# MachinaIO/mxx

Measured on AMD Instinct MI355X. Metric: dcrt_ring_ops_per_s, higher is better.
Workload: dtype u32

## Files before the change

include/gpupoly.h:

```cpp
#ifndef GPUPOLY_H
#define GPUPOLY_H

#include <stddef.h>
#include <stdint.h>

#ifdef __cplusplus
extern "C" {
#endif

typedef struct GpuContext GpuContext;
typedef struct GpuMatrix GpuMatrix;
typedef struct GpuEventSet GpuEventSet;
typedef struct GpuP1CovarianceCache GpuP1CovarianceCache;
typedef struct GpuComm GpuComm;

typedef struct GpuRngSeed {
    uint64_t words[4];
} GpuRngSeed;

#define GPU_POLY_FORMAT_COEFF 0
#define GPU_POLY_FORMAT_EVAL 1
#define GPU_MATRIX_DIST_UNIFORM 0
#define GPU_MATRIX_DIST_GAUSS 1
#define GPU_MATRIX_DIST_BIT 2
// ... 98 lines not shown
    const GpuMatrix *lhs;
    const GpuMatrix *rhs;
} GpuBatchOp;
int gpupoly_batch(const GpuBatchOp *ops, size_t count, uint32_t base_bits);
int gpupoly_matrix_mul_decompose_small(GpuMatrix *out, const GpuMatrix *lhs, const GpuMatrix *rhs, uint32_t base_bits);
int gpupoly_matrix_mul_tensor_identity(GpuMatrix *out, const GpuMatrix *lhs, const GpuMatrix *rhs, size_t identity_size);
int gpupoly_matrix_mul_tensor_identity_decompose(GpuMatrix *out, const GpuMatrix *lhs, const GpuMatrix *rhs,
                                                 size_t identity_size, uint32_t base_bits);
int gpupoly_matrix_mul_scalar_intt(GpuMatrix *out, const GpuMatrix *lhs, const GpuMatrix *scalar_1x1);
int gpupoly_matrix_transpose(GpuMatrix *out, const GpuMatrix *src);
int gpupoly_matrix_tensor(GpuMatrix *out, const GpuMatrix *lhs, const GpuMatrix *rhs);
int gpupoly_matrix_add_rows(GpuMatrix *out, size_t dst_row, const GpuMatrix *lhs, const GpuMatrix *rhs);
int gpupoly_matrix_ntt_add_rows(GpuMatrix *out, size_t dst_row, GpuMatrix *coeff, const GpuMatrix *addend,
                                int consume_coeff);
int gpupoly_matrix_row_view(GpuMatrix *m, size_t row, size_t rows, GpuMatrix **out_view);
int gpupoly_matrix_reshape_view(GpuMatrix *m, size_t rows, size_t cols, GpuMatrix **out_view);
int gpupoly_matrix_neg(GpuMatrix *out, const GpuMatrix *src);
int gpupoly_matrix_fill_zero(GpuMatrix *out);
int gpupoly_matrix_fill_identity(GpuMatrix *out, const GpuMatrix *scalar_1x1);
int gpupoly_matrix_sample_decomposed(GpuMatrix *out, int dist_type, double sigma, GpuRngSeed seed, uint32_t base_bits,
                                     int small);
int gpupoly_matrix_decompose_rows(const GpuMatrix *src, uint32_t base_bits, int small, size_t row_start, GpuMatrix *out);
int gpupoly_matrix_sample_decomposed_window(GpuMatrix *out, int dist_type, double sigma, GpuRngSeed seed,
                                            uint32_t base_bits, int small, size_t src_rows, size_t full_ncol,
                                            size_t col_offset, size_t row_start);
int gpupoly_timer_start(GpuContext *ctx);
int gpupoly_timer_stop(GpuContext *ctx, float *out_ms);
int gpupoly_timer_mark(GpuContext *ctx, uint32_t slot);
int gpupoly_timer_elapsed(GpuContext *ctx, uint32_t slot_begin, uint32_t slot_end, float *out_ms);
int gpupoly_matrix_device_ptr(const GpuMatrix *mat, void **out_ptr, size_t *out_bytes);
int gpupoly_matrix_layout(const GpuMatrix *mat, int *out);
int gpupoly_matrix_copy_to_context(GpuContext *dst_ctx, const GpuMatrix *src, GpuMatrix **out);
int gpupoly_context_device(const GpuContext *ctx, int *out_device);
int gpupoly_context_word_bytes(const GpuContext *ctx, int *out_bytes);
const char *gpupoly_context_last_kernel(const GpuContext *ctx);
int gpupoly_context_stream(const GpuContext *ctx, void **out_stream);
int gpupoly_comm_create(GpuContext *const *ctxs, size_t n, GpuComm **out_comm);
void gpupoly_comm_destroy(GpuComm *comm);
int gpupoly_comm_size(const GpuComm *comm, int *out_size);
const char *gpupoly_comm_backend(const GpuComm *comm);
int gpupoly_matrix_all_gather_columns(GpuComm *comm, const GpuMatrix *const *local_blocks, GpuMatrix *const *full);
int gpupoly_matrix_sample_distribution_segments(GpuMatrix *out, int dist_type, double sigma, const GpuRngSeed *seeds,
                                                const size_t *seg_cols, size_t nseg);
int gpupoly_matrix_sample_p1_full_cached_segments(const GpuP1CovarianceCache *cache, const GpuMatrix *tp2,
                                                  const GpuRngSeed *seeds, const size_t *seg_cols, size_t nseg,
                                                  GpuMatrix *out);
int gpupoly_matrix_gauss_samp_gq_arb_base_segments(GpuMatrix *src, uint32_t base_bits, double c, double dgg_stddev,
                                                   const GpuRngSeed *seeds, const size_t *seg_cols, size_t nseg,
                                                   GpuMatrix *out);
#define GPUPOLY_BLOCKS_STACKED 0
#define GPUPOLY_BLOCKS_COLUMNS 1
int gpupoly_matrix_sample_distribution_blocks(GpuMatrix *out, int dist_type, const GpuRngSeed *seeds, size_t nblk,
                                              int layout, const size_t *seg_cols);
#define GPUPOLY_HASH_KECCAK256 0
#define GPUPOLY_HASH_SHA3_256 1
#define GPUPOLY_TAGS_TABLE 0
#define GPUPOLY_TAGS_INDEXED_LE64 1
#define GPUPOLY_TAGS_INDEXED_DECIMAL 2
typedef struct GpuHashTags {
    int hash;
    int form;
    uint8_t key[32];
    const uint8_t *tags;
    const size_t *tag_offsets;
    size_t prefix_len;
    uint64_t first_index;
} GpuHashTags;
int gpupoly_hash_seeds(GpuContext *ctx, const GpuHashTags *tags, size_t ntags, GpuRngSeed *seeds_out);
int gpupoly_matrix_sample_hash_blocks(GpuMatrix *out, int dist_type, const GpuHashTags *tags, size_t nblk, int layout,
                                      const size_t *seg_cols);
int gpupoly_matrix_sample_gauss_blocks(GpuMatrix *out, double sigma, const GpuRngSeed *seeds, size_t nblk, int layout,
                                       const size_t *seg_cols);
int gpupoly_matrix_sample_hash_gauss_blocks(GpuMatrix *out, double sigma, const GpuHashTags *tags, size_t nblk, int layout,
                                            const size_t *seg_cols);
int gpupoly_matrix_concat_columns(GpuMatrix *out, const GpuMatrix *const *blocks, size_t n);
int gpupoly_matrix_split_columns(const GpuMatrix *src, GpuMatrix *const *blocks, size_t n);
int gpupoly_trapdoor_preimage_many(const GpuMatrix *re, const GpuP1CovarianceCache *cache, const GpuMatrix *public_matrix,
                                   uint32_t base_bits, const GpuMatrix *const *targets, size_t n, const GpuRngSeed *seeds,
                                   GpuMatrix *const *outs);
int gpupoly_trapdoor_preimage_keyed(const GpuMatrix *const *res, const GpuP1CovarianceCache *const *caches,
                                    const GpuMatrix *const *public_matrices, size_t nkeys, uint32_t base_bits,
                                    const uint32_t *key_of, const GpuMatrix *const *targets, size_t n,
                                    const GpuRngSeed *seeds, GpuMatrix *const *outs);
int gpupoly_matrix_sample_decomposed_blocks(GpuMatrix *out, int dist_type, const GpuRngSeed *seeds, size_t nblk,
                                            uint32_t base_bits, int small, size_t src_rows, size_t full_ncol,
                                            size_t col_offset);
int gpupoly_matrix_sample_hash_decomposed_blocks(GpuMatrix *out, int dist_type, const GpuHashTags *tags, size_t nblk,
                                                 uint32_t base_bits, int small, size_t src_rows, size_t full_ncol,
                                                 size_t col_offset);
int gpupoly_matrix_lut_targets(GpuMatrix *const *outs, size_t nrows_T, const GpuMatrix *w_identity, const GpuMatrix *w_gy,
                               const GpuMatrix *w_v, const GpuMatrix *w_vx, size_t col_start, uint32_t base_bits,
                               const uint64_t *y_words, size_t words_per_y, const uint64_t *idx, const GpuHashTags *tags);
int gpupoly_matrix_lut_targets_combine(GpuMatrix *const *outs, size_t nrows_T, const GpuMatrix *w_identity,
                                       const GpuMatrix *w_gy, const GpuMatrix *product, size_t col_start, uint32_t base_bits,
                                       const uint64_t *y_words, size_t words_per_y, const uint64_t *idx);
int gpupoly_matrix_scale_round(GpuMatrix *out, const GpuMatrix *in, uint64_t t, int round_half);
int gpupoly_matrix_crt_recompose_rounded(GpuMatrix *out, const GpuMatrix *const *terms, const int *signs,
                                         size_t terms_per_level, size_t num_slots);
int gpupoly_matrix_store_coeff_words(const GpuMatrix *mat, uint64_t *out, size_t words_per_coeff);
int gpupoly_matrix_load_coeff_words(GpuMatrix *mat, const uint64_t *words, size_t words_per_coeff, size_t coeffs_per_poly,
                                    int out_format);
int gpupoly_matrix_centered_max_abs(const GpuMatrix *mat, uint64_t *out, size_t words_per_value);
int gpupoly_matrix_extract_bits(const GpuMatrix *mat, const uint64_t *lo, const uint64_t *hi, size_t words_per_bound,
                                uint8_t *out, size_t bytes_per_poly);
int gpupoly_matrix_store_coeff_ints(const GpuMatrix *mat, void *out, int elem_bytes, int centred, size_t coeffs_per_poly,
                                    uint64_t *out_misfit_count, uint64_t *out_first_misfit);
int gpupoly_matrix_store_compact_bytes_many(GpuMatrix *const *mats, size_t n, uint8_t *payload_out, size_t payload_capacity,
                                            uint16_t *out_max_coeff_bits, uint16_t *out_bytes_per_coeff,
                                            size_t *out_payload_offsets, size_t *out_payload_lens, size_t *out_total_len);
int gpupoly_matrix_load_compact_bytes_many(GpuMatrix *const *mats, size_t n, const uint8_t *const *payloads,
                                           const size_t *payload_lens, const uint16_t *max_coeff_bits);
int gpupoly_matrix_fill_monomial(GpuMatrix *out, uint64_t shift, int format);
int gpupoly_matrix_mul_monomial(GpuMatrix *out, const GpuMatrix *in, uint64_t shift);
int gpupoly_matrix_monomial_sum(GpuMatrix *out, const GpuMatrix *addend, const GpuMatrix *const *mats,
                                const uint64_t *shifts, size_t n, int negate);
int gpupoly_matrix_mul_sum(GpuMatrix *out, size_t dst_col, size_t cols, const GpuMatrix *addend,
                           const GpuMatrix *const *lhss, const GpuMatrix *const *rhss, size_t n, int negate);
int gpupoly_matrix_mul_acc(GpuMatrix *out, const GpuMatrix *lhs, const GpuMatrix *rhs, int negate);
int gpupoly_matrix_mul_gadget(GpuMatrix *out, size_t dst_col, const GpuMatrix *lhs, const GpuMatrix *scalar_1x1,
                              size_t gadget_col, size_t cols, const GpuMatrix *addend, int negate, uint32_t base_bits,
                              int small);
int gpupoly_matrix_gadget_mul(GpuMatrix *out, const GpuMatrix *rhs, const GpuMatrix *addend, int negate,
                              uint32_t base_bits, int small);
int gpupoly_matrix_mul_decompose_gadget_scalar_many(GpuMatrix *const *outs, const GpuMatrix *const *lhss,
                                                    const GpuMatrix *const *addends, size_t n, const GpuMatrix *scalar_1x1,
                                                    int negate, uint32_t base_bits);
int gpupoly_matrix_mul_decompose_gadget_const_many(GpuMatrix *const *outs, const GpuMatrix *const *lhss,
                                                   const GpuMatrix *const *addends, size_t n, const uint64_t *const_words,
                                                   size_t words_per_const, int negate, uint32_t base_bits);
uint64_t gpupoly_launch_count(void);
int gpupoly_detmath_eval(GpuContext *ctx, int fn, const double *host_in, double *host_out, size_t n);
int gpupoly_device_can_access_peer(int device, int peer, int *out_can);
int gpupoly_marker_launch(GpuContext *ctx, uint32_t id);
int gpupoly_trace_begin(void);
const char *gpupoly_trace_end(void);
const char *gpupoly_version(void);
int gpupoly_reload_env(void);

#ifdef __cplusplus
}
#endif
#endif
```

mxx_amd/_ffi.py:

```python
from __future__ import annotations

import ctypes as C
import os

_HERE = os.path.dirname(os.path.abspath(__file__))
LIB_PATH = os.environ.get("MXX_GPUPOLY_LIB") or os.path.join(_HERE, "libgpupoly.so")

GPU_POLY_FORMAT_COEFF = 0
GPU_POLY_FORMAT_EVAL = 1
GPU_MATRIX_DIST_UNIFORM = 0
GPU_MATRIX_DIST_GAUSS = 1
GPU_MATRIX_DIST_BIT = 2
GPU_MATRIX_DIST_TERNARY = 3
GPUPOLY_BLOCKS_STACKED = 0
GPUPOLY_BLOCKS_COLUMNS = 1
GPUPOLY_HASH_KECCAK256 = 0
GPUPOLY_HASH_SHA3_256 = 1
GPUPOLY_TAGS_TABLE = 0
GPUPOLY_TAGS_INDEXED_LE64 = 1
GPUPOLY_TAGS_INDEXED_DECIMAL = 2


class GpuPolyError(RuntimeError):
    """Raised where the reference's Rust wrapper panics (`check_status`, gpu.rs:259-263)."""
# ... 54 lines not shown
    "gpu_matrix_add": (C.c_int, [_vp, _vp, _vp]),
    "gpu_matrix_sub": (C.c_int, [_vp, _vp, _vp]),
    "gpu_matrix_add_block": (C.c_int, [_vp, _vp, _sz, _sz, _sz, _sz, _sz, _sz]),
    "gpu_matrix_mul": (C.c_int, [_vp, _vp, _vp]),
    "gpu_matrix_mul_scalar": (C.c_int, [_vp, _vp, _vp]),
    "gpu_matrix_equal": (C.c_int, [_vp, _vp, C.POINTER(C.c_int)]),
    "gpu_matrix_ntt_all": (C.c_int, [_vp]),
    "gpu_matrix_intt_all": (C.c_int, [_vp]),
    "gpu_matrix_fill_gadget": (C.c_int, [_vp, C.c_uint32]),
    "gpu_matrix_fill_small_gadget": (C.c_int, [_vp, C.c_uint32]),
    "gpu_matrix_fill_small_decomposed_identity_chunk": (C.c_int, [_vp, _vp, _sz]),
    "gpu_matrix_decompose_base": (C.c_int, [_vp, C.c_uint32, _vp]),
    "gpu_matrix_decompose_base_small": (C.c_int, [_vp, C.c_uint32, _vp]),
    "gpu_matrix_sample_distribution": (C.c_int, [_vp, C.c_int, C.c_double, GpuRngSeed]),
    "gpu_matrix_sample_distribution_columns": (C.c_int, [_vp, C.c_int, C.c_double, GpuRngSeed, _sz, _sz]),
    "gpu_matrix_gauss_samp_gq_arb_base": (C.c_int, [_vp, C.c_uint32, C.c_double, C.c_double, GpuRngSeed, _vp]),
    "gpu_matrix_sample_p1_full": (C.c_int, [_vp, _vp, _vp, _vp, C.c_double, C.c_double, C.c_double, GpuRngSeed, _vp]),
    "gpu_matrix_create_p1_covariance_cache": (C.c_int, [_vp, _vp, _vp, C.c_double, C.c_double, C.c_double, C.POINTER(_vp)]),
    "gpu_matrix_destroy_p1_covariance_cache": (None, [_vp]),
    "gpu_matrix_sample_p1_full_cached": (C.c_int, [_vp, _vp, GpuRngSeed, _vp]),
    "gpu_matrix_load_rns_batch": (C.c_int, [_vp, _vp, _sz, C.c_int, C.POINTER(_vp)]),
    "gpu_matrix_store_rns_batch": (C.c_int, [_vp, _vp, _sz, C.c_int, C.POINTER(_vp)]),
    "gpu_matrix_store_const_coeff_batch": (C.c_int, [_vp, _vp, _sz, C.POINTER(_vp)]),
    "gpu_matrix_store_compact_bytes": (C.c_int, [_vp, _vp, _sz, C.POINTER(C.c_uint16), C.POINTER(C.c_uint16), C.POINTER(_sz)]),
    "gpu_matrix_load_compact_bytes": (C.c_int, [_vp, _vp, _sz, C.c_uint16]),
    "gpu_poly_store_compact_bytes": (C.c_int, [_vp, _vp, _sz, C.POINTER(C.c_uint16), C.POINTER(C.c_uint16), C.POINTER(_sz)]),
    "gpu_poly_load_compact_bytes": (C.c_int, [_vp, _vp, _sz, C.c_uint16]),
    "gpupoly_matrix_mul_decompose": (C.c_int, [_vp, _vp, _vp, C.c_uint32]),
    "gpupoly_matrix_mul_decompose_many": (C.c_int, [C.POINTER(C.c_void_p), C.POINTER(C.c_void_p), C.POINTER(C.c_void_p), C.POINTER(C.c_void_p), C.c_size_t, _vp, C.c_uint32]),
    "gpupoly_matrix_mul_decompose_pairs": (C.c_int, [C.POINTER(C.c_void_p), C.POINTER(C.c_void_p), C.POINTER(C.c_void_p), C.POINTER(C.c_void_p), C.POINTER(C.c_void_p), _sz, _sz, C.c_uint32, C.c_int]),
    "gpupoly_matrix_mul_batch":(C.c_int, [C.POINTER(C.c_void_p), C.POINTER(C.c_void_p), C.POINTER(C.c_void_p), C.c_size_t]),
    "gpupoly_batch": (C.c_int, [C.POINTER(GpuBatchOp), C.c_size_t, C.c_uint32]),
    "gpupoly_matrix_mul_decompose_small": (C.c_int, [_vp, _vp, _vp, C.c_uint32]),
    "gpupoly_matrix_mul_tensor_identity": (C.c_int, [_vp, _vp, _vp, C.c_size_t]),
    "gpupoly_matrix_mul_tensor_identity_decompose": (C.c_int, [_vp, _vp, _vp, C.c_size_t, C.c_uint32]),
    "gpupoly_matrix_mul_scalar_intt": (C.c_int, [_vp, _vp, _vp]),
    "gpupoly_matrix_transpose": (C.c_int, [_vp, _vp]),
    "gpupoly_matrix_tensor": (C.c_int, [_vp, _vp, _vp]),
    "gpupoly_matrix_add_rows": (C.c_int, [_vp, C.c_size_t, _vp, _vp]),
    "gpupoly_matrix_ntt_add_rows": (C.c_int, [_vp, C.c_size_t, _vp, _vp, C.c_int]),
    "gpupoly_matrix_row_view": (C.c_int, [_vp, C.c_size_t, C.c_size_t, C.POINTER(C.c_void_p)]),
    "gpupoly_matrix_reshape_view": (C.c_int, [_vp, C.c_size_t, C.c_size_t, C.POINTER(C.c_void_p)]),
    "gpupoly_matrix_neg": (C.c_int, [_vp, _vp]),
    "gpupoly_matrix_fill_zero": (C.c_int, [_vp]),
    "gpupoly_matrix_fill_identity": (C.c_int, [_vp, _vp]),
    "gpupoly_matrix_sample_decomposed": (C.c_int, [_vp, C.c_int, C.c_double, GpuRngSeed, C.c_uint32, C.c_int]),
    "gpupoly_matrix_decompose_rows": (C.c_int, [_vp, C.c_uint32, C.c_int, _sz, _vp]),
    "gpupoly_matrix_sample_decomposed_window": (C.c_int, [_vp, C.c_int, C.c_double, GpuRngSeed, C.c_uint32, C.c_int, _sz, _sz, _sz, _sz]),
    "gpupoly_timer_start": (C.c_int, [_vp]),
    "gpupoly_timer_stop": (C.c_int, [_vp, C.POINTER(C.c_float)]),
    "gpupoly_timer_mark": (C.c_int, [_vp, C.c_uint32]),
    "gpupoly_timer_elapsed": (C.c_int, [_vp, C.c_uint32, C.c_uint32, C.POINTER(C.c_float)]),
    "gpupoly_matrix_device_ptr": (C.c_int, [_vp, C.POINTER(_vp), C.POINTER(_sz)]),
    "gpupoly_matrix_layout": (C.c_int, [_vp, C.POINTER(C.c_int)]),
    "gpupoly_matrix_copy_to_context": (C.c_int, [_vp, _vp, C.POINTER(_vp)]),
    "gpupoly_context_device": (C.c_int, [_vp, C.POINTER(C.c_int)]),
    "gpupoly_context_word_bytes": (C.c_int, [_vp, C.POINTER(C.c_int)]),
    "gpupoly_context_last_kernel": (C.c_char_p, [_vp]),
    "gpupoly_context_stream": (C.c_int, [_vp, C.POINTER(C.c_void_p)]),
    "gpupoly_comm_create": (C.c_int, [C.POINTER(C.c_void_p), C.c_size_t, C.POINTER(_vp)]),
    "gpupoly_comm_destroy": (None, [_vp]),
    "gpupoly_comm_size": (C.c_int, [_vp, C.POINTER(C.c_int)]),
    "gpupoly_comm_backend": (C.c_char_p, [_vp]),
    "gpupoly_matrix_all_gather_columns": (C.c_int, [_vp, C.POINTER(C.c_void_p), C.POINTER(C.c_void_p)]),
    "gpupoly_matrix_sample_distribution_segments": (C.c_int, [_vp, C.c_int, C.c_double, C.POINTER(GpuRngSeed), C.POINTER(_sz), _sz]),
    "gpupoly_matrix_sample_distribution_blocks": (C.c_int, [_vp, C.c_int, C.POINTER(GpuRngSeed), _sz, C.c_int, C.POINTER(_sz)]),
    "gpupoly_hash_seeds": (C.c_int, [_vp, C.POINTER(GpuHashTags), _sz, C.POINTER(GpuRngSeed)]),
    "gpupoly_matrix_sample_hash_blocks": (C.c_int, [_vp, C.c_int, C.POINTER(GpuHashTags), _sz, C.c_int, C.POINTER(_sz)]),
    "gpupoly_matrix_sample_gauss_blocks": (C.c_int, [_vp, C.c_double, C.POINTER(GpuRngSeed), _sz, C.c_int, C.POINTER(_sz)]),
    "gpupoly_matrix_sample_hash_gauss_blocks": (C.c_int, [_vp, C.c_double, C.POINTER(GpuHashTags), _sz, C.c_int, C.POINTER(_sz)]),
    "gpupoly_matrix_sample_decomposed_blocks": (C.c_int, [_vp, C.c_int, C.POINTER(GpuRngSeed), _sz, C.c_uint32, C.c_int, _sz, _sz, _sz]),
    "gpupoly_matrix_sample_hash_decomposed_blocks": (C.c_int, [_vp, C.c_int, C.POINTER(GpuHashTags), _sz, C.c_uint32, C.c_int, _sz, _sz, _sz]),
    "gpupoly_matrix_lut_targets": (C.c_int, [C.POINTER(C.c_void_p), _sz, _vp, _vp, _vp, _vp, _sz, C.c_uint32, C.POINTER(C.c_uint64), _sz,
                                   C.POINTER(C.c_uint64), C.POINTER(GpuHashTags)]),
    "gpupoly_matrix_lut_targets_combine": (C.c_int, [C.POINTER(C.c_void_p), _sz, _vp, _vp, _vp, _sz, C.c_uint32, C.POINTER(C.c_uint64), _sz,
                                           C.POINTER(C.c_uint64)]),
    "gpupoly_matrix_sample_p1_full_cached_segments":(C.c_int, [_vp, _vp, C.POINTER(GpuRngSeed), C.POINTER(_sz), _sz, _vp]),
    "gpupoly_matrix_gauss_samp_gq_arb_base_segments": (C.c_int, [_vp, C.c_uint32, C.c_double, C.c_double, C.POINTER(GpuRngSeed), C.POINTER(_sz), _sz, _vp]),
    "gpupoly_matrix_concat_columns": (C.c_int, [_vp, C.POINTER(C.c_void_p), _sz]),
    "gpupoly_matrix_split_columns": (C.c_int, [_vp, C.POINTER(C.c_void_p), _sz]),
    "gpupoly_trapdoor_preimage_many": (C.c_int, [_vp, _vp, _vp, C.c_uint32, C.POINTER(C.c_void_p), _sz, C.POINTER(GpuRngSeed), C.POINTER(C.c_void_p)]),
    "gpupoly_trapdoor_preimage_keyed": (C.c_int, [C.POINTER(C.c_void_p), C.POINTER(C.c_void_p), C.POINTER(C.c_void_p), _sz, C.c_uint32,
                                        C.POINTER(C.c_uint32), C.POINTER(C.c_void_p), _sz, C.POINTER(GpuRngSeed), C.POINTER(C.c_void_p)]),
    "gpupoly_launch_count": (C.c_uint64, []),
    "gpupoly_matrix_scale_round": (C.c_int, [_vp, _vp, C.c_uint64, C.c_int]),
    "gpupoly_matrix_crt_recompose_rounded": (C.c_int, [_vp, C.POINTER(C.c_void_p), C.POINTER(C.c_int), _sz, _sz]),
    "gpupoly_matrix_store_coeff_words": (C.c_int, [_vp, C.POINTER(C.c_uint64), _sz]),
    "gpupoly_matrix_load_coeff_words": (C.c_int, [_vp, C.POINTER(C.c_uint64), _sz, _sz, C.c_int]),
    "gpupoly_matrix_centered_max_abs": (C.c_int, [_vp, C.POINTER(C.c_uint64), _sz]),
    "gpupoly_matrix_extract_bits": (C.c_int, [_vp, C.POINTER(C.c_uint64), C.POINTER(C.c_uint64), _sz, _u8p, _sz]),
    "gpupoly_matrix_store_coeff_ints": (C.c_int, [_vp, _vp, C.c_int, C.c_int, _sz, C.POINTER(C.c_uint64), C.POINTER(C.c_uint64)]),
    "gpupoly_matrix_fill_monomial": (C.c_int, [_vp, C.c_uint64, C.c_int]),
    "gpupoly_matrix_mul_monomial": (C.c_int, [_vp, _vp, C.c_uint64]),
    "gpupoly_matrix_monomial_sum": (C.c_int, [_vp, _vp, C.POINTER(C.c_void_p), C.POINTER(C.c_uint64), _sz, C.c_int]),
    "gpupoly_matrix_mul_sum": (C.c_int, [_vp, _sz, _sz, _vp, C.POINTER(C.c_void_p), C.POINTER(C.c_void_p), _sz, C.c_int]),
    "gpupoly_matrix_mul_acc": (C.c_int, [_vp, _vp, _vp, C.c_int]),
    "gpupoly_matrix_mul_gadget": (C.c_int, [_vp, _sz, _vp, _vp, _sz, _sz, _vp, C.c_int, C.c_uint32, C.c_int]),
    "gpupoly_matrix_gadget_mul": (C.c_int, [_vp, _vp, _vp, C.c_int, C.c_uint32, C.c_int]),
    "gpupoly_matrix_mul_decompose_gadget_scalar_many": (C.c_int, [C.POINTER(C.c_void_p), C.POINTER(C.c_void_p), C.POINTER(C.c_void_p), _sz, _vp, C.c_int, C.c_uint32]),
    "gpupoly_matrix_mul_decompose_gadget_const_many": (C.c_int, [C.POINTER(C.c_void_p), C.POINTER(C.c_void_p), C.POINTER(C.c_void_p), _sz, C.POINTER(C.c_uint64), _sz, C.c_int, C.c_uint32]),
    "gpupoly_matrix_store_compact_bytes_many": (C.c_int, [C.POINTER(C.c_void_p), _sz, _vp, _sz, C.POINTER(C.c_uint16), C.POINTER(C.c_uint16), C.POINTER(_sz), C.POINTER(_sz), C.POINTER(_sz)]),
    "gpupoly_matrix_load_compact_bytes_many": (C.c_int, [C.POINTER(C.c_void_p), _sz, C.POINTER(C.c_void_p), C.POINTER(_sz), C.POINTER(C.c_uint16)]),
    "gpupoly_detmath_eval": (C.c_int, [_vp, C.c_int, C.POINTER(C.c_double), C.POINTER(C.c_double), _sz]),
    "gpupoly_device_can_access_peer": (C.c_int, [C.c_int, C.c_int, C.POINTER(C.c_int)]),
    "gpupoly_marker_launch": (C.c_int, [_vp, C.c_uint32]),
    "gpupoly_trace_begin": (C.c_int, []),
    "gpupoly_trace_end": (C.c_char_p, []),
    "gpupoly_version": (C.c_char_p, []),
    "gpupoly_reload_env": (C.c_int, []),
}

_lib = None


def lib() -> C.CDLL:
    global _lib
    if _lib is None:
        if not os.path.exists(LIB_PATH):
            raise GpuPolyError(
                f"{LIB_PATH} is missing: build it with `python -c 'import __graft_entry__ as g; g.build()'` "
                "(or `make -C mxx_amd/csrc`). mxx_amd has no CPU fallback."
            )
        handle = C.CDLL(LIB_PATH)
        for name, (res, args) in SIGNATURES.items():
            fn = getattr(handle, name)
            fn.restype = res
            fn.argtypes = args
        _lib = handle
    return _lib


def last_error_string() -> str:
    msg = lib().gpu_last_error()
    return msg.decode("utf-8", "replace") if msg else "unknown GPU error"


def check_status(code: int, context: str) -> None:
    if code != 0:
        raise GpuPolyError(f"{context} failed: {last_error_string()}")


def reload_env() -> None:
    check_status(lib().gpupoly_reload_env(), "gpupoly_reload_env")


def trace_begin() -> None:
    check_status(lib().gpupoly_trace_begin(), "gpupoly_trace_begin")


def trace_end() -> list[dict]:
    text = lib().gpupoly_trace_end()
    if text is None:
        raise GpuPolyError(f"gpupoly_trace_end failed: {last_error_string()}")
    out = []
    for ln in text.decode().splitlines():
        name, blocks, threads, nbytes, ms = ln.split("\t")
        out.append({"kernel": name.strip("()"), "blocks": int(blocks), "threads": int(threads), "bytes": float(nbytes), "ms": float(ms)})
    return out


def gpu_device_sync() -> None:
    check_status(lib().gpu_device_synchronize(), "gpu_device_synchronize")


def detected_gpu_device_ids() -> list[int]:
    n = C.c_int(0)
# ... 28 lines not shown
```

mxx_amd/csrc/common.h:

```cpp
#pragma once

#include <hip/hip_runtime.h>

#include <atomic>
#include <cstddef>
#include <cstdint>
#include <cstdio>
#include <exception>
#include <map>
#include <unordered_map>
#include <mutex>
#include <string>
#include <vector>

#include "../../include/gpupoly.h"

constexpr size_t GPUPOLY_MAX_LIMBS = 64;

struct LimbConst {
    uint64_t q;
    uint64_t mu;
    uint64_t mu64;
    uint64_t n_inv;
    uint64_t n_inv_sh;
    uint64_t mu32;
    uint64_t inv_last_w;
    uint64_t inv_last_w_sh;
    uint32_t kbits;
    uint32_t lazy_terms;
};

struct EnvSwitches {
    int ntt_path = 0;
    int ntt14 = 0;
    bool decompose_fused = true;
    char matmul_path = 0;
    int matmul_tile = 0;
    bool gsamp_simple = false;
    bool gsamp_no_uni = false;
    bool p1_simple = false;
    int sampler_per_lane = 0;
    int sampler_fill_every = 0;
    bool ntt64_int = false;
    int ntt_phase = 0;
    bool serde_general = false;
    bool rng_compat = false;
    bool pack24 = true;
    int skinny24 = 0;
    int skinny24_shape = 0;
    size_t mul_decompose_many_budget = 0;
    size_t mul_decompose_pairs_budget = 0;
    size_t gadget_scalar_budget = 0;
    char mul_sum_path = 0;
    size_t crt_recompose_chunk_bytes = size_t(256) << 20;
    void load();
};

struct GpuContext {
    EnvSwitches env;
    int device = 0;
    std::vector<int> gpu_ids;
    uint32_t logN = 0;
    int N = 0;
    int level = 0;
    uint32_t dnum = 0;
    int limb_count = 0;
    bool wide = false;
    int word_bytes = 4;
    uint32_t crt_bits = 0;
    std::vector<uint64_t> moduli;
    hipStream_t stream = nullptr;
    LimbConst *d_limbs = nullptr;
    LimbConst *d_limbs_r = nullptr;
    void *d_tw_fwd = nullptr;
    void *d_tw_fwd_sh = nullptr;
    void *d_tw_inv = nullptr;
    void *d_tw_inv_sh = nullptr;
    void *d_tw2_fwd = nullptr;
    void *d_tw2_inv = nullptr;
    bool lazy_ok = false;
    bool tight_ok = false;
    void *d_tw2s_inv = nullptr;
    bool signed_ok = false;
    void *d_twf_fwd = nullptr, *d_twf_inv = nullptr;
    void *d_flimbs = nullptr;
    bool f64_ok = false;
    uint64_t *d_garner = nullptr;
    std::vector<uint64_t> garner_inv;
    std::vector<LimbConst> limbs;
    hipEvent_t timer_start = nullptr, timer_stop = nullptr;
    std::vector<hipEvent_t> marks;
    std::mutex mutex;
    bool pool_ok = false;
    std::mutex alloc_mutex;
    std::multimap<size_t, void *> free_blocks;
    std::unordered_map<void *, size_t> live_blocks;
    size_t cached_bytes = 0, cache_limit = 0;
    std::atomic<const char *> last_kernel{""};
    bool pack24_ok = false;
    std::mutex layout_mutex;
    std::map<uint32_t, void *> gadget_weights;
    std::map<std::vector<uint64_t>, void *> gadget_const_tables;
};

struct LayoutTag {
    std::atomic<int> v{GPU_MATRIX_LAYOUT_WORDS};
    LayoutTag() = default;
    LayoutTag(const LayoutTag &o) : v(o.v.load(std::memory_order_acquire)) {}
    LayoutTag &operator=(const LayoutTag &o) {
        v.store(o.v.load(std::memory_order_acquire), std::memory_order_release);
        return *this;
    }
};

struct GpuMatrix {
    GpuContext *ctx = nullptr;
    int level = 0;
    size_t rows = 0, cols = 0;
    int format = GPU_POLY_FORMAT_EVAL;
    void *storage = nullptr;
    size_t bytes = 0;
    LayoutTag layout;
    bool borrowed = false;
    GpuMatrix *parent = nullptr;
    int views = 0;
};

struct GpuEventSet {
    std::vector<hipEvent_t> events;
    int device = 0;
    void *staging = nullptr;
    GpuContext *ctx = nullptr;
    void *dev_staging = nullptr;
};

struct GpuP1CovarianceCache {
    GpuContext *ctx = nullptr;
    int level = 0;
    size_t d = 0, m = 0, n = 0;
    double sigma = 0, s = 0, dgg_stddev = 0;
    double *sqrt_var = nullptr;
    double *update_coeff = nullptr;
    void *karney_div = nullptr;
};

struct P1KeyEntry {
    const double *sqrt_var;
    const double *update_coeff;
    const void *karney_div;
};

static inline dim3 item_grid(size_t items, unsigned threads) {
    const size_t blocks = (items + threads - 1) / threads;
    const size_t max_x = (static_cast<size_t>(1) << 31) / threads;
// ... 79 lines not shown

inline size_t matrix_polys(const GpuMatrix *m) { return m->rows * m->cols; }
inline size_t matrix_limbs(const GpuMatrix *m) { return static_cast<size_t>(m->level) + 1; }
inline size_t matrix_words(const GpuMatrix *m) { return matrix_polys(m) * matrix_limbs(m) * static_cast<size_t>(m->ctx->N); }

void *words_ptr(const GpuMatrix *m);
const void *packed24_ptr(const GpuMatrix *m, bool *packed);
inline size_t packed24_bytes(const GpuMatrix *m) { return m->bytes / 4 * 3; }
inline bool storage_overlaps(const GpuMatrix *x, const GpuMatrix *y) {
    if (x == y) return true;
    if (!x->storage || !y->storage || x->bytes == 0 || y->bytes == 0) return false;
    const size_t xb = x->layout.v.load(std::memory_order_acquire) == GPU_MATRIX_LAYOUT_PACKED24 ? packed24_bytes(x) : x->bytes;
    const size_t yb = y->layout.v.load(std::memory_order_acquire) == GPU_MATRIX_LAYOUT_PACKED24 ? packed24_bytes(y) : y->bytes;
    const char *xs = static_cast<const char *>(x->storage), *ys = static_cast<const char *>(y->storage);
    return xs < ys + yb && ys < xs + xb;
}
inline bool same_block(const GpuMatrix *x, const GpuMatrix *y) {
    return x == y || (x->storage == y->storage && x->bytes == y->bytes);
}
inline bool partial_overlap(const GpuMatrix *out, const GpuMatrix *operand) {
    return storage_overlaps(out, operand) && !same_block(out, operand);
}
inline bool row_block_overlaps(const GpuMatrix *m, size_t row, size_t rows, const GpuMatrix *y) {
    if (m->layout.v.load(std::memory_order_acquire) == GPU_MATRIX_LAYOUT_PACKED24) return rows && m->cols && storage_overlaps(m, y);
    if (!m->storage) return false;
    const size_t poly_bytes = matrix_limbs(m) * static_cast<size_t>(m->ctx->N) * m->ctx->word_bytes;
    GpuMatrix block;
    block.storage = static_cast<char *>(m->storage) + row * m->cols * poly_bytes;
    block.bytes = rows * m->cols * poly_bytes;
    return storage_overlaps(&block, y);
}
bool pack24_eligible(const GpuMatrix *m);
int pack24_store(GpuMatrix *m, bool ntt);

int sample_impl(GpuMatrix *out, int dist, double sigma, GpuRngSeed seed, size_t full_ncol, size_t col_offset, bool keep_coeff,
                size_t row_offset = 0, uint32_t tower_first = 0, uint32_t tower_count = 0);

struct RngBlockWindow {
    size_t cols, full_ncol, col_offset;
};
int sample_blocks_impl(const char *entry, bool hashed, GpuMatrix *out, int dist_type, const GpuRngSeed *seeds, const GpuHashTags *tags,
                       size_t nblk, int layout, const size_t *seg_cols, const RngBlockWindow *win, const double *sigma = nullptr);
int sample_decomposed_blocks_impl(const char *entry, bool hashed, GpuMatrix *out, int dist_type, const GpuRngSeed *seeds,
                                  const GpuHashTags *tags, size_t nblk, uint32_t base_bits, int small, size_t src_rows, size_t full_ncol,
                                  size_t col_offset);

int hash_tags_check(const char *entry, const GpuHashTags *tags, size_t ntags, size_t *table_bytes);
size_t hash_tags_staged_words(const GpuHashTags *tags, size_t ntags, size_t table_bytes);
void hash_tags_stage(const GpuHashTags *tags, size_t ntags, size_t table_bytes, uint64_t *staging);
int launch_hash_seeds(GpuContext *ctx, GpuRngSeed *d_seeds, const GpuHashTags *tags, size_t ntags, const uint64_t *d_staged);

int ctx_activate(const GpuContext *ctx);
bool ctx_is_registered(const GpuContext *ctx);
int ctx_alloc(GpuContext *ctx, size_t bytes, void **out);
void ctx_free(GpuContext *ctx, void *ptr);
struct CtxBlock {
    GpuContext *ctx;
    void *ptr = nullptr;
    explicit CtxBlock(GpuContext *c) : ctx(c) {}
    CtxBlock(const CtxBlock &) = delete;
    CtxBlock &operator=(const CtxBlock &) = delete;
    ~CtxBlock() {
        if (ptr) ctx_free(ctx, ptr);
    }
    int alloc(size_t bytes) { return ctx_alloc(ctx, bytes, &ptr); }
    void *release() {
        void *p = ptr;
        ptr = nullptr;
        return p;
    }
};
int matrix_check_same_shape(const GpuMatrix *a, const GpuMatrix *b, const char *who);
int coeff_domain_source(const GpuMatrix *mat, CtxBlock &scratch, const void **src);

int launch_ntt(GpuContext *ctx, void *data, size_t vectors, int limbs_per_poly, bool inverse);
int launch_ntt_lds_u32(GpuContext *ctx, uint32_t *data, size_t vectors, uint32_t L, bool inverse);
int launch_ntt_digits_u32(GpuContext *ctx, uint32_t *out, const uint32_t *coeff, size_t out_vectors, uint32_t L,
                          uint32_t src_cols, uint32_t towers, uint32_t dpt, uint32_t base_bits, size_t k, uint32_t td0 = 0);
int launch_ntt_lds_u64(GpuContext *ctx, uint64_t *data, size_t vectors, uint32_t L, bool inverse);
int launch_ntt_digits_u64(GpuContext *ctx, uint64_t *out, const uint64_t *coeff, size_t out_vectors, uint32_t L,
                          uint32_t src_cols, uint32_t towers, uint32_t dpt, uint32_t base_bits, size_t k, uint32_t td0 = 0);
int launch_intt_oop_u32(GpuContext *ctx, uint32_t *out, const uint32_t *in, size_t vectors, uint32_t L);
int launch_ntt_add_u32(GpuContext *ctx, uint32_t *out, const uint32_t *src, const uint32_t *add, size_t vectors, uint32_t L);
int launch_mul_intt_u32(GpuContext *ctx, uint32_t *out, const uint32_t *in, const uint32_t *w, size_t vectors, uint32_t L);
int launch_matmul(GpuMatrix *out, const GpuMatrix *lhs, const GpuMatrix *rhs);
int launch_ntt_fwd_pack24_u32(GpuContext *ctx, uint32_t *out, const uint32_t *in, size_t vectors, uint32_t L);
int launch_matmul_skinny24(GpuMatrix *out, const GpuMatrix *lhs, const GpuMatrix *rhs, bool small_grid);
int skinny24_parse_shape(const char *s);
int launch_matmul_dma_u32(GpuMatrix *out, const GpuMatrix *lhs, const GpuMatrix *rhs);
int launch_matmul_dma32_u32(GpuMatrix *out, const GpuMatrix *lhs, const GpuMatrix *rhs);
int launch_matmul_mfma_u32(GpuMatrix *out, const GpuMatrix *lhs, const GpuMatrix *rhs);
int launch_copy_block(GpuMatrix *out, const GpuMatrix *src, size_t dst_row, size_t dst_col, size_t src_row,
                      size_t src_col, size_t rows, size_t cols, bool add);
int sample_p1_keyed_segments(const GpuP1CovarianceCache *cache, const P1KeyEntry *d_keys, const GpuMatrix *tp2,
                             const GpuRngSeed *seeds, const size_t *seg_cols, size_t nseg, GpuMatrix *out);
int launch_scatter_i64(GpuMatrix *out, const int64_t *vals);
```

mxx_amd/csrc/ntt14.h:

```cpp
#pragma once

#include "ntt_lds.h"

namespace ntt14 {
constexpr int LOGN = 14;
constexpr uint32_t N = 1u << LOGN;
constexpr uint32_t T = 512;
constexpr int R0 = 32;
constexpr uint32_t BLK = 512;
constexpr uint32_t BLK_PAD = BLK + 64;
constexpr uint32_t GROUP_WORDS = 8 * BLK_PAD;

__device__ __forceinline__ uint32_t pad64(uint32_t pos) { return pos + ((pos >> 5) << 2); }

__device__ __forceinline__ void wave_sync() {
    __builtin_amdgcn_fence(__ATOMIC_ACQ_REL, "wavefront");
    __builtin_amdgcn_wave_barrier();
}

#ifdef GPUPOLY_PHASE_TIMING
#define NTT14_PHASE(bit) ((phase & (bit)) != 0)
#else
#define NTT14_PHASE(bit) false
#endif
// ... 115 lines not shown
                        if (t[0] == static_cast<W>(0xdeadbeefu) && t[VN - 1] == static_cast<W>(0x12345u)) dstc[0] = t[0];
                    } else if constexpr (NTS) __builtin_nontemporal_store(t, reinterpret_cast<wx *>(dstc));
                    else *reinterpret_cast<wx *>(dstc) = t;
                }
                continue;
            }
            W *dst = g + B * BLK + 8 * lane;
#pragma unroll
            for (int m = 0; m < 8; m += VN) {
                typedef W wx __attribute__((ext_vector_type(VN)));
                wx t;
#pragma unroll
                for (int e = 0; e < VN; ++e) t[e] = v[m + e];
                if constexpr (PK) {
                    store_packed4<NTS>(reinterpret_cast<uint32_t *>(g), B * BLK + 8 * lane + m, t[0], t[1], t[2], t[3]);
                    continue;
                }
                if constexpr (ADD) {
                    const wx a = __builtin_nontemporal_load(reinterpret_cast<const wx *>(addv + B * BLK + 8 * lane + m));
#pragma unroll
                    for (int e = 0; e < VN; ++e) t[e] = csub<W>(t[e] + a[e], q);
                }
                if (NTT14_PHASE(4)) {
                    if (t[0] == static_cast<W>(0xdeadbeefu) && t[VN - 1] == static_cast<W>(0x12345u)) dst[m] = t[0];
                } else if constexpr (NTS) __builtin_nontemporal_store(t, reinterpret_cast<wx *>(dst + m));
                else *reinterpret_cast<wx *>(dst + m) = t;
            }
        }
    }
}

template <typename W, bool NT = false>
struct LoadVector {
    const W *g;
    __device__ __forceinline__ W operator()(uint32_t e) const { return nt_load<NT, W>(g + e); }
};

template <typename W, bool TIGHT = false, bool NT = false>
__global__ void __launch_bounds__(512, 8 / (sizeof(W) / 4))
    fwd_kernel(W *__restrict__ data, const TwPair<W> *__restrict__ tw_all, const LimbConst *__restrict__ limbs,
               uint32_t L, uint32_t phase = 0) {
    const uint32_t limb = blockIdx.x;
    const size_t vec = (static_cast<size_t>(blockIdx.z) * gridDim.y + blockIdx.y) * L + limb;
    const LimbConst lc = limbs[limb];
    W *g = data + vec * N;
#ifdef GPUPOLY_PHASE_TIMING
    if (phase & 64) {
        fwd_body<W, TIGHT, NT, LoadVector<W, NT>, false, NT, true>(g, LoadVector<W, NT>{g}, tw_all, lc, limb, nullptr, phase);
    } else if (phase & 8) {
        if (phase & 16) fwd_body<W, TIGHT, false, LoadVector<W, NT>, false, true>(g, LoadVector<W, NT>{g}, tw_all, lc, limb, nullptr, phase);
        else fwd_body<W, TIGHT, NT, LoadVector<W, NT>, false, true>(g, LoadVector<W, NT>{g}, tw_all, lc, limb, nullptr, phase);
    } else if (phase & 16) {
        fwd_body<W, TIGHT, false>(g, LoadVector<W, NT>{g}, tw_all, lc, limb, nullptr, phase);
    } else {
        fwd_body<W, TIGHT, NT>(g, LoadVector<W, NT>{g}, tw_all, lc, limb, nullptr, phase);
    }
#else
    (void)phase;
    fwd_body<W, TIGHT, NT, LoadVector<W, NT>, false, NT>(g, LoadVector<W, NT>{g}, tw_all, lc, limb);
#endif
}

template <bool NT = false>
__global__ void __launch_bounds__(512, 8)
    fwd_pack24_kernel(uint32_t *__restrict__ out, const uint32_t *__restrict__ in, const TwPair<uint32_t> *__restrict__ tw_all,
                      const LimbConst *__restrict__ limbs, uint32_t L) {
    const uint32_t limb = blockIdx.x;
    const size_t vec = (static_cast<size_t>(blockIdx.z) * gridDim.y + blockIdx.y) * L + limb;
    const LimbConst lc = limbs[limb];
    fwd_body<uint32_t, false, NT, LoadVector<uint32_t, NT>, false, NT, false, true>(
        out + vec * (N / 4 * 3), LoadVector<uint32_t, NT>{in + vec * N}, tw_all, lc, limb);
}

template <typename W, bool TIGHT = false>
__global__ void __launch_bounds__(512, 8 / (sizeof(W) / 4))
    fwd_add_kernel(W *__restrict__ out, const W *__restrict__ src, const W *__restrict__ add,
                   const TwPair<W> *__restrict__ tw_all, const LimbConst *__restrict__ limbs, uint32_t L) {
    const uint32_t limb = blockIdx.x;
    const size_t vec = (static_cast<size_t>(blockIdx.z) * gridDim.y + blockIdx.y) * L + limb;
    const LimbConst lc = limbs[limb];
    fwd_body<W, TIGHT, true, LoadVector<W, true>, true, true>(out + vec * N, LoadVector<W, true>{src + vec * N}, tw_all, lc, limb, add + vec * N);
}

template <typename W, bool REDUCE>
struct LoadDigit {
    const W *src;
    uint32_t shift;
    W mask, q;
    __device__ __forceinline__ W operator()(uint32_t e) const {
        const W digit = (src[e] >> shift) & mask;
        if constexpr (REDUCE) return digit >= q ? digit % q : digit;
        else return digit;
    }
};

template <typename W, bool REDUCE, bool TIGHT = false, bool NTS = false>
__global__ void __launch_bounds__(512, 8 / (sizeof(W) / 4))
    fwd_digits_kernel(W *__restrict__ out, const W *__restrict__ coeff, const TwPair<W> *__restrict__ tw_all,
                      const LimbConst *__restrict__ limbs, uint32_t L, uint32_t src_cols, uint32_t towers, uint32_t dpt,
                      uint32_t base_bits, uint32_t k, uint32_t td0) {
    const uint32_t rest = blockIdx.x >> 3, col_hi = rest / L, limb = rest - col_hi * L;
    const uint32_t col = col_hi * 8u + (blockIdx.x & 7u);
    if (col >= src_cols) return;
    const uint32_t td = blockIdx.y + td0;
    const size_t r = blockIdx.z;
    const uint32_t t = td / dpt, d = td - t * dpt;
    const size_t vec = ((r * k + blockIdx.y) * src_cols + col) * L + limb;
    const LimbConst lc = limbs[limb];
    const uint32_t src_bits = limbs[t].kbits, shift = d * base_bits;
    LoadDigit<W, REDUCE> load;
    load.src = coeff + ((r * src_cols + col) * L + t) * N;
    load.shift = shift < 8 * sizeof(W) ? shift : 0;
    load.mask = 0;
    if (shift < src_bits && shift < 8 * sizeof(W)) {
        const uint32_t rem = src_bits - shift;
        const uint32_t db = base_bits < rem ? base_bits : rem;
        load.mask = db >= 8 * sizeof(W) ? static_cast<W>(~static_cast<W>(0)) : static_cast<W>((static_cast<W>(1) << db) - 1);
    }
    load.q = static_cast<W>(lc.q);
    (void)towers;
    fwd_body<W, TIGHT, NTS, LoadDigit<W, REDUCE>, false, NTS>(out + vec * N, load, tw_all, lc, limb);
}

template <typename W, bool SGN, bool MULW = false, int CAP = 31, int WPS = ((SGN && !MULW) ? 8 : 6), bool NT = false>
__global__ void __launch_bounds__(512, WPS / (sizeof(W) / 4))
    inv_kernel(W *__restrict__ data, const TwPair<W> *__restrict__ tw_all, const LimbConst *__restrict__ limbs,
               uint32_t L, const W *in = nullptr, const W *__restrict__ mulw = nullptr) {
    extern __shared__ __attribute__((aligned(16))) unsigned char smem[];
    W *xs = reinterpret_cast<W *>(smem);
    typedef typename std::conditional<sizeof(W) == 4, uint4, ulonglong2>::type V16;
    constexpr int VN = 16 / sizeof(W);
    const uint32_t tid = threadIdx.x, lane = tid & 63u;
    const uint32_t wave = __builtin_amdgcn_readfirstlane(tid >> 6);
    const uint32_t limb = blockIdx.x;
    const size_t vec = (static_cast<size_t>(blockIdx.z) * gridDim.y + blockIdx.y) * L + limb;
    const LimbConst lc = limbs[limb];
    const W q = static_cast<W>(lc.q);
    const W muw = static_cast<W>(sizeof(W) == 4 ? lc.mu32 : lc.mu64);
    const TwPair<W> *tw = tw_all + static_cast<size_t>(limb) * N;
    W *g = data + vec * N;
    const W *gin = (!MULW && in) ? in + vec * N : g;

    V16 dnext[8 / VN], wnext[8 / VN];
    const W *src0 = (MULW ? in + vec * N : g) + wave * BLK + 8 * lane;
    const W *wsrc0 = MULW ? mulw + static_cast<size_t>(limb) * N + wave * BLK + 8 * lane : nullptr;
    if constexpr (MULW) {
#pragma unroll
        for (int m = 0; m < 8 / VN; ++m) {
            dnext[m] = *reinterpret_cast<const V16 *>(src0 + m * VN);
            wnext[m] = *reinterpret_cast<const V16 *>(wsrc0 + m * VN);
        }
    }

    W h[R0];
#pragma unroll
    for (int grp = 0; grp < 4; ++grp) {
        W *x = xs + (grp & 1) * GROUP_WORDS;
        W *xb = x + wave * BLK_PAD;
        const uint32_t B = 8u * grp + wave;
        W v[8];
        {
            if constexpr (MULW) {
                static_assert(sizeof(W) == 4, "the fused product is a 32-bit Montgomery product");
                W wv[8];
#pragma unroll
                for (int m = 0; m < 8 / VN; ++m) {
// ... 73 lines not shown
```

mxx_amd/csrc/ntt_lds_u32.hip:

```cpp
#include "ntt_rings.h"

using W = uint32_t;

int launch_ntt_lds_u32(GpuContext *ctx, uint32_t *data, size_t vectors, uint32_t L, bool inverse) {
    return launch_ntt_lds<W>(ctx, data, vectors, L, inverse);
}

template __global__ void ntt14::inv_kernel<W, true, false, 31, 8, true>(W *, const TwPair<W> *, const LimbConst *, uint32_t, const W *,
                                                                        const W *);

template <typename R, bool TIGHT>
static int launch_lazy_mulw(GpuContext *ctx, W *out, const W *in, const W *w, size_t vectors, uint32_t L) {
    const size_t lds = R::template lds<W>();
    if (lds > kLdsLimitBytes) return -1;
    if (int rc = lds_opt_in<ntt_inv_lazy_kernel<W, R::LOGN, R::LOGR, R::WPE, 0, TIGHT, false, true>>(ctx, lds)) return rc;
    MXX_LAUNCH((ntt_inv_lazy_kernel<W, R::LOGN, R::LOGR, R::WPE, 0, TIGHT, false, true>), dim3(static_cast<unsigned>(vectors)), R::block(),
               lds, ctx->stream, out, tw_inv<W>(ctx), ctx->d_limbs_r, L, in, w);
    HIP_TRY(hipGetLastError());
    return 0;
}

template <typename R, bool TIGHT>
static int launch_split_mulw(GpuContext *ctx, W *out, const W *in, const W *w, size_t vectors, uint32_t L) {
    const size_t lds = R::template lds<W>();
    if (lds > kLdsLimitBytes || !R::fits(vectors)) return -1;
    if (int rc = lds_opt_in<ntt_inv_lazy_kernel<W, R::LOGN, R::LOGR, R::WPE, R::PRE, TIGHT, false, true>>(ctx, lds)) return rc;
    const uint32_t logN = R::RING;
    MXX_LAUNCH((ntt_inv_lazy_kernel<W, R::LOGN, R::LOGR, R::WPE, R::PRE, TIGHT, false, true>), R::sub_grid(vectors), R::block(), lds,
               ctx->stream, out, tw_inv<W>(ctx), ctx->d_limbs, L, in, w);
    MXX_LAUNCH((ntt_inv_tail_kernel<W, R::PRE, TIGHT>), dim3(static_cast<unsigned>(vectors * R::set_blocks)), dim3(256), 0, ctx->stream, out,
               tw_inv<W>(ctx), ctx->d_limbs_r, L, logN);
    HIP_TRY(hipGetLastError());
    return 0;
}

int launch_mul_intt_u32(GpuContext *ctx, uint32_t *out, const uint32_t *in, const uint32_t *w, size_t vectors, uint32_t L) {
    if (!(ctx->lazy_ok || ctx->tight_ok) || !ctx->d_limbs_r || ctx->env.ntt_path > 1 || vectors > 0x7fffffffull) return -1;
    MXX_TRACE_BYTES(2.0 * vectors * ctx->N * sizeof(W));
    dim3 grid;
    if (ntt14_grouped(ctx, vectors, L, false, true, grid)) {
        const dim3 block(ntt14::T);
        const size_t lds = ntt14::lds_bytes(sizeof(W));
        if (ntt14_signed(ctx))
            MXX_LAUNCH((ntt14::inv_kernel<W, true, true>), grid, block, lds, ctx->stream, out,
                       static_cast<const TwPair<W> *>(ctx->d_tw2s_inv), ctx->d_limbs_r, L, in, w);
        else
            MXX_LAUNCH((ntt14::inv_kernel<W, false, true>), grid, block, lds, ctx->stream, out, tw_inv<W>(ctx), ctx->d_limbs_r, L, in, w);
        HIP_TRY(hipGetLastError());
        return 0;
    }
    return by_width_class<W>(ctx, [&](auto tight) {
        constexpr bool TIGHT = decltype(tight)::value;
        return visit_ring<W>(ctx->logN, [&](auto ring) {
            using R = decltype(ring);
            if constexpr (R::PRE > 0) return launch_split_mulw<R, TIGHT>(ctx, out, in, w, vectors, L);
            else return launch_lazy_mulw<R, TIGHT>(ctx, out, in, w, vectors, L);
        });
    });
}

int launch_intt_oop_u32(GpuContext *ctx, uint32_t *out, const uint32_t *in, size_t vectors, uint32_t L) {
    dim3 grid;
    if (vectors == 0 || !ntt14_grouped(ctx, vectors, L, true, true, grid)) return -1;
    MXX_TRACE_BYTES(2.0 * vectors * ntt14::N * sizeof(W));
    return launch_ntt_lds<W>(ctx, out, vectors, L, true, in);
}

int launch_ntt_fwd_pack24_u32(GpuContext *ctx, uint32_t *out, const uint32_t *in, size_t vectors, uint32_t L) {
    dim3 grid;
    if (vectors == 0 || !ntt14_grouped(ctx, vectors, L, false, false, grid)) return -1;
    const bool nt = (vectors << 14) * sizeof(W) >= (size_t(1) << 30);
    MXX_TRACE_BYTES(1.75 * vectors * ntt14::N * sizeof(W));
    return bool_dispatch(nt, [&](auto NT) {
        MXX_LAUNCH((ntt14::fwd_pack24_kernel<NT()>), grid, dim3(ntt14::T), ntt14::lds_bytes(sizeof(W)), ctx->stream, out, in, tw_fwd<W>(ctx),
                   ctx->d_limbs, L);
        HIP_TRY(hipGetLastError());
        return 0;
    });
}

int launch_ntt_add_u32(GpuContext *ctx, uint32_t *out, const uint32_t *src, const uint32_t *add, size_t vectors, uint32_t L) {
    dim3 grid;
    if (!ntt14_grouped(ctx, vectors, L, true, true, grid)) return -1;
    MXX_TRACE_BYTES(3.0 * vectors * ntt14::N * sizeof(W));
    return bool_dispatch(!ctx->lazy_ok, [&](auto TIGHT) {
        MXX_LAUNCH((ntt14::fwd_add_kernel<W, TIGHT()>), grid, dim3(ntt14::T), ntt14::lds_bytes(sizeof(W)), ctx->stream, out, src, add,
                   tw_fwd<W>(ctx), ctx->d_limbs, L);
        HIP_TRY(hipGetLastError());
        return 0;
    });
}

int launch_ntt_digits_u32(GpuContext *ctx, uint32_t *out, const uint32_t *coeff, size_t out_vectors, uint32_t L,
                          uint32_t src_cols, uint32_t towers, uint32_t dpt, uint32_t base_bits, size_t k, uint32_t td0) {
    DigitLaunch<W> d{out, coeff, L, src_cols, towers, dpt, base_bits, 0, td0};
    if (!ntt14_switches(ctx, true, true) || !d.plan(ctx, out_vectors, k)) return -1;
    MXX_TRACE_BYTES((static_cast<double>(d.src_rows) * src_cols * L + static_cast<double>(out_vectors)) * ctx->N * sizeof(W));
    if (ctx->logN != 14) return launch_ntt_digits<W>(ctx, d);
    const dim3 grid(8u * L * ((src_cols + 7u) / 8u), d.k, static_cast<unsigned>(d.src_rows));
    return bool_dispatch(d.reduce, !ctx->lazy_ok, d.nts, [&](auto RED, auto TIGHT, auto NTS) {
        MXX_LAUNCH((ntt14::fwd_digits_kernel<W, RED(), TIGHT(), NTS()>), grid, dim3(ntt14::T), ntt14::lds_bytes(sizeof(W)), ctx->stream, out,
                   coeff, tw_fwd<W>(ctx), ctx->d_limbs, L, src_cols, towers, dpt, base_bits, d.k, td0);
        HIP_TRY(hipGetLastError());
        return 0;
    });
}
```

mxx_amd/csrc/preimage.hip:

```cpp
#include "matmul_tile.h"
#include "rng.h"

#include <algorithm>
#include <cmath>
#include <string>
#include <vector>

namespace {

constexpr size_t kGroupMax = RNG_MAX_SEGMENTS;
constexpr size_t kGroupBytes = size_t(1) << 30;

struct RequestTable {
    uint32_t count;
    uint32_t start[kGroupMax + 1];
    uint32_t pad_start[kGroupMax];
    void *ptr[kGroupMax];
};

__device__ __forceinline__ uint32_t request_of(const RequestTable &t, uint32_t col) {
    uint32_t lo = 0, hi = t.count;
    while (hi - lo > 1) {
        const uint32_t mid = (lo + hi) >> 1;
        if (col >= t.start[mid]) lo = mid;
// ... 125 lines not shown
    const uint32_t ct = blockIdx.y / row_tiles, rt = blockIdx.y - ct * row_tiles;
    const uint32_t i = (blockIdx.x * blockDim.x + threadIdx.x) * SV;
    if (i >= N) return;
    uint32_t lo = 0, hi = keys.count;
    while (hi - lo > 1) {
        const uint32_t mid = (lo + hi) >> 1;
        if (ct >= keys.tile_start[mid]) lo = mid;
        else hi = mid;
    }
    const uint32_t r0 = rt * TR, c0 = keys.col_start[lo] + (ct - keys.tile_start[lo]) * TC, cend = keys.col_start[lo + 1];
    const LimbConst lc = limbs[limb];
    const W q = static_cast<W>(lc.q);
    typedef typename TileTypes<W, SV>::VT VT;
    typedef typename TileTypes<W, SV>::wxs wxs;
    typedef typename TileTypes<W, SV>::D D;

    const size_t poly = static_cast<size_t>(L) * N;
    const size_t in_poly = static_cast<size_t>(limb) * N + i;
    const W *a_ptr[TR];
#pragma unroll
    for (int r = 0; r < TR; ++r)
        a_ptr[r] = static_cast<const W *>(keys.lhs[lo]) + static_cast<size_t>(min(r0 + r, rows - 1)) * inner * poly + in_poly;
    size_t b_off[TC];
#pragma unroll
    for (int c = 0; c < TC; ++c) b_off[c] = static_cast<size_t>(min(c0 + c, cend - 1)) * poly + in_poly;
    const size_t strideBk = static_cast<size_t>(cols) * poly;

    D acc[TR][TC][SV];
    MXX_TILE_CLEAR(acc);
    const uint32_t lazy = lc.lazy_terms;
    uint32_t pending = 0;
#define MXX_TILE_A(r, k) (a_ptr[r] + (k) * poly)
#define MXX_TILE_B(c, k) (B + b_off[c] + (k) * strideBk)
#include "matmul_tile_loop.inc"
#pragma unroll
    for (int r = 0; r < TR; ++r) {
        if (r0 + r >= rows) continue;
#pragma unroll
        for (int c = 0; c < TC; ++c) {
            if (c0 + c >= cend) continue;
            W o[SV];
#pragma unroll
            for (int s = 0; s < SV; ++s) o[s] = tile_reduce<W>(acc[r][c][s], q, lc);
            *reinterpret_cast<VT *>(C + (static_cast<size_t>(r0 + r) * cols + c0 + c) * poly + in_poly) = *reinterpret_cast<const VT *>(o);
        }
    }
}

struct KeyRuns {
    size_t count = 0;
    uint32_t start[kGroupMax + 1];
    uint32_t pad_start[kGroupMax + 1];
    const GpuMatrix *re[kGroupMax], *a[kGroupMax];
};

static uint64_t keyed_col_tiles(const uint32_t *col_start, size_t runs, uint32_t tc) {
    uint64_t tiles = 0;
    for (size_t k = 0; k < runs; ++k) tiles += (col_start[k + 1] - col_start[k] + tc - 1) / tc;
    return tiles;
}

static bool keyed_grid_fits(const GpuContext *ctx, size_t rows, const uint32_t *col_start, size_t runs, size_t L) {
    const TileShape t = stacked_tile(ctx, rows, col_start[runs], L);
    return (rows + t.tr - 1) / t.tr * keyed_col_tiles(col_start, runs, t.tc) <= 65535;
}

template <typename W, int TR, int TC, int SV>
static int launch_keyed_cfg(GpuContext *ctx, GpuMatrix *out, const GpuMatrix *const *lhs, const uint32_t *col_start, size_t runs,
                            const GpuMatrix *rhs) {
    const uint32_t rows = static_cast<uint32_t>(out->rows), inner = static_cast<uint32_t>(rhs->rows),
                   cols = static_cast<uint32_t>(rhs->cols), L = static_cast<uint32_t>(matrix_limbs(out));
    KeyedLhs keys{};
    keys.count = static_cast<uint32_t>(runs);
    uint32_t tiles = 0;
    double lhs_bytes = 0.0;
    for (size_t k = 0; k < runs; ++k) {
        keys.col_start[k] = col_start[k];
        keys.tile_start[k] = tiles;
        keys.lhs[k] = words_ptr(lhs[k]);
        tiles += (col_start[k + 1] - col_start[k] + TC - 1) / TC;
        lhs_bytes += static_cast<double>(lhs[k]->bytes);
    }
    for (size_t k = runs; k <= kGroupMax; ++k) {
        keys.col_start[k] = cols;
        keys.tile_start[k] = tiles;
    }
    TileGrid g = tile_grid<TR, TC, SV>(ctx, rows, cols, L, rhs->bytes);
    g.grid.y = g.row_tiles * tiles;
    if (g.grid.y > 65535) return set_error("gpupoly_trapdoor_preimage_keyed: matrix too large");
    static const std::string name = std::string("matmul_keyed_kernel<") + (sizeof(W) == 4 ? "u32," : "u64,") + std::to_string(TR) + "," +
                                    std::to_string(TC) + "," + std::to_string(SV) + "> (a left operand per column run, few rows)";
    ctx->last_kernel = name.c_str();
    MXX_TRACE_BYTES(lhs_bytes + static_cast<double>(rhs->bytes) + static_cast<double>(out->bytes));
    MXX_LAUNCH((matmul_keyed_kernel<W, TR, TC, SV>), g.grid, dim3(g.threads), 0, ctx->stream, keys, static_cast<W *>(words_ptr(out)),
               static_cast<const W *>(words_ptr(rhs)), ctx->d_limbs, rows, inner, cols, L, static_cast<uint32_t>(ctx->N), g.row_tiles);
    HIP_TRY(hipGetLastError());
    return 0;
}

static int launch_matmul_keyed(GpuContext *ctx, GpuMatrix *out, const GpuMatrix *const *lhs, const uint32_t *col_start, size_t runs,
                               const GpuMatrix *rhs) {
    const int rc = dispatch_stacked_tile(ctx, stacked_tile(ctx, out->rows, rhs->cols, matrix_limbs(out)), [&](auto cfg) {
        typedef decltype(cfg) T;
        return launch_keyed_cfg<typename T::W, T::TR, T::TC, T::SV>(ctx, out, lhs, col_start, runs, rhs);
    });
    if (rc == 0) out->format = GPU_POLY_FORMAT_EVAL;
    return rc;
}

struct TempMatrix {
    GpuMatrix *m = nullptr;
    TempMatrix() = default;
    TempMatrix(const TempMatrix &) = delete;
    TempMatrix &operator=(const TempMatrix &) = delete;
    ~TempMatrix() { release(); }
    int make(GpuContext *ctx, int level, size_t rows, size_t cols) {
        return gpu_matrix_create(ctx, level, rows, cols, GPU_POLY_FORMAT_EVAL, &m);
    }
    void release() {
        gpu_matrix_destroy(m);
        m = nullptr;
    }
};

static GpuMatrix row_block(const GpuMatrix *m, size_t row, size_t rows) {
    const size_t poly_bytes = matrix_limbs(m) * static_cast<size_t>(m->ctx->N) * m->ctx->word_bytes;
    char *base = static_cast<char *>(words_ptr(m));
    GpuMatrix v = *m;
    v.rows = rows;
    v.storage = rows && m->cols ? base + row * m->cols * poly_bytes : nullptr;
    v.bytes = rows * m->cols * poly_bytes;
    v.borrowed = true;
    return v;
}

static bool words_overlap(const GpuMatrix *a, const GpuMatrix *b) { return a->bytes && b->bytes && storage_overlaps(a, b); }

static int fail(const std::string &msg) { return set_error("gpupoly_trapdoor_preimage_many: " + msg); }

struct PreimageCall {
    GpuContext *ctx;
    const GpuMatrix *re, *a;
    const GpuP1CovarianceCache *cache;
    uint32_t base_bits;
    double sigma_large;
    size_t d, dk;
    const char *entry = "gpupoly_trapdoor_preimage_many";
};

struct KeyedGroup {
    KeyRuns runs;
    const P1KeyEntry *d_keys;
};

static int preimage_group(const PreimageCall &call, const GpuMatrix *const *targets, const GpuRngSeed *seeds,
                          GpuMatrix *const *outs, const std::vector<size_t> &group, const KeyedGroup *keyed = nullptr) {
    GpuContext *ctx = call.ctx;
    const int level = call.re->level;
    const size_t top = 2 * call.d, ng = group.size();
    std::vector<size_t> cols(ng), pads(ng);
    std::vector<GpuRngSeed> seed_p2(ng), seed_p1(ng), seed_z(ng);
    RequestTable gather{}, scatter{};
    gather.count = scatter.count = static_cast<uint32_t>(ng);
    size_t at = 0, pad_at = 0;
    for (size_t g = 0; g < ng; ++g) {
        const size_t j = group[g];
        cols[g] = targets[j]->cols;
        pads[g] = (cols[g] + call.d - 1) / call.d * call.d;
        seed_p2[g] = seeds[3 * j];
        seed_p1[g] = seeds[3 * j + 1];
        seed_z[g] = seeds[3 * j + 2];
        gather.start[g] = scatter.start[g] = static_cast<uint32_t>(at);
        gather.pad_start[g] = scatter.pad_start[g] = static_cast<uint32_t>(pad_at);
        gather.ptr[g] = words_ptr(targets[j]);
        scatter.ptr[g] = words_ptr(outs[j]);
        at += cols[g];
        pad_at += pads[g];
    }
    if (pad_at >> 32) return set_error(std::string(call.entry) + ": a group of requests wider than 2^32 columns");
    for (size_t g = ng; g <= kGroupMax; ++g) gather.start[g] = scatter.start[g] = static_cast<uint32_t>(at);
    for (size_t g = ng; g < kGroupMax; ++g) {
        gather.pad_start[g] = scatter.pad_start[g] = static_cast<uint32_t>(pad_at);
        gather.ptr[g] = scatter.ptr[g] = nullptr;
    }
    TempMatrix p, tp2, ap, perturbed, z, rez;
    int rc = p.make(ctx, level, top + call.dk, pad_at);
    if (rc) return rc;
    GpuMatrix p1 = row_block(p.m, 0, top), p2 = row_block(p.m, top, call.dk);
    rc = gpupoly_matrix_sample_distribution_segments(&p2, GPU_MATRIX_DIST_GAUSS, call.sigma_large, seed_p2.data(), pads.data(), ng);
    if (rc) return rc;
    if ((rc = tp2.make(ctx, level, top, pad_at))) return rc;
    rc = keyed ? launch_matmul_keyed(ctx, tp2.m, keyed->runs.re, keyed->runs.pad_start, keyed->runs.count, &p2)
               : gpu_matrix_mul(tp2.m, call.re, &p2);
    if (rc || (rc = gpu_matrix_intt_all(tp2.m))) return rc;
    rc = keyed ? sample_p1_keyed_segments(call.cache, keyed->d_keys, tp2.m, seed_p1.data(), pads.data(), ng, &p1)
               : gpupoly_matrix_sample_p1_full_cached_segments(call.cache, tp2.m, seed_p1.data(), pads.data(), ng, &p1);
    if (rc) return rc;
    tp2.release();
    p.m->format = GPU_POLY_FORMAT_EVAL;
    if ((rc = ap.make(ctx, level, call.d, pad_at))) return rc;
    rc = keyed ? launch_matmul_keyed(ctx, ap.m, keyed->runs.a, keyed->runs.pad_start, keyed->runs.count, p.m) : gpu_matrix_mul(ap.m, call.a, p.m);
    if (rc) return rc;
    if ((rc = perturbed.make(ctx, level, call.d, at))) return rc;
    rc = ctx->wide ? launch_gather_sub<uint64_t>(ctx, perturbed.m, ap.m, gather) : launch_gather_sub<uint32_t>(ctx, perturbed.m, ap.m, gather);
    if (rc) return rc;
    ap.release();
    if ((rc = z.make(ctx, level, call.dk, at))) return rc;
    rc = gpupoly_matrix_gauss_samp_gq_arb_base_segments(perturbed.m, call.base_bits, call.cache->sigma, call.cache->dgg_stddev,
                                                        seed_z.data(), cols.data(), ng, z.m);
    if (rc) return rc;
    perturbed.release();
    if ((rc = rez.make(ctx, level, top, at))) return rc;
    rc = keyed ? launch_matmul_keyed(ctx, rez.m, keyed->runs.re, keyed->runs.start, keyed->runs.count, z.m) : gpu_matrix_mul(rez.m, call.re, z.m);
    if (rc) return rc;
    return ctx->wide ? launch_scatter<uint64_t>(ctx, scatter, p.m, rez.m, z.m) : launch_scatter<uint32_t>(ctx, scatter, p.m, rez.m, z.m);
}

}

extern "C" int gpupoly_trapdoor_preimage_many(const GpuMatrix *re, const GpuP1CovarianceCache *cache,
                                              const GpuMatrix *public_matrix, uint32_t base_bits,
                                              const GpuMatrix *const *targets, size_t n, const GpuRngSeed *seeds,
                                              GpuMatrix *const *outs) {
    ABI_GUARD_BEGIN
    if (!re || !cache || !public_matrix) return fail("null trapdoor, covariance cache or public matrix");
    if (n == 0) return 0;
    if (!targets || !seeds || !outs) return fail("null targets, seeds or outputs");
    GpuContext *ctx = re->ctx;
    const int level = re->level;
    if (cache->ctx != ctx || public_matrix->ctx != ctx) return fail("context mismatch");
    if (cache->level != level || public_matrix->level != level) return fail("level mismatch");
    if (base_bits == 0 || base_bits >= 63) return fail("invalid base_bits");
    const size_t d = public_matrix->rows, L = matrix_limbs(re);
    const uint32_t dpt = (ctx->crt_bits + base_bits - 1) / base_bits;
    const size_t top = 2 * d, dk = d * dpt * L;
    if (d == 0 || re->rows != top || re->cols != dk || public_matrix->cols != top + dk || cache->d != d || cache->m != top)
        return fail("shape mismatch: needs [R; E] 2d x dk, A d x (2d + dk) and a covariance cache of dimension d");
    if (re->format != GPU_POLY_FORMAT_EVAL || public_matrix->format != GPU_POLY_FORMAT_EVAL)
        return fail("[R; E] and the public matrix must be in EVAL form");
    for (size_t j = 0; j < n; ++j) {
        const GpuMatrix *t = targets[j], *o = outs[j];
        if (!t || !o) return fail("null target or output " + std::to_string(j));
        if (t->ctx != ctx || o->ctx != ctx) return fail("context mismatch in request " + std::to_string(j));
        if (t->level != level || o->level != level) return fail("level mismatch in request " + std::to_string(j));
        if (t->rows != d) return fail("target " + std::to_string(j) + " must have d rows");
        if (o->rows != top + dk || o->cols != t->cols)
            return fail("output " + std::to_string(j) + " must be (2d + dk) x its target's columns");
        if (t->format != GPU_POLY_FORMAT_EVAL) return fail("target " + std::to_string(j) + " must be in EVAL form");
        if (t->cols >> 31) return fail("target " + std::to_string(j) + " too wide");
    }
    for (size_t j = 0; j < n; ++j) {
        const GpuMatrix *o = outs[j];
        bool alias = words_overlap(o, re) || words_overlap(o, public_matrix);
        for (size_t i = 0; i < n && !alias; ++i) alias = words_overlap(o, targets[i]) || (i != j && words_overlap(o, outs[i]));
        if (alias) return fail("output " + std::to_string(j) + " aliases an input or another output");
    }
    if ((static_cast<size_t>(ctx->N) >> 1) % SAMPLER_THREADS)
        return fail("unsupported: ring dimension not a multiple of 128 (segmented samplers)");
    if (cache->m > 8) return fail("unsupported: trapdoor dimension above 4 (no p1 lane kernel)");
    if (ctx->env.p1_simple) return fail("unsupported under MXX_HIP_P1=simple (the p1 lane kernel is switched off)");
    if (dpt > 4) return fail("unsupported: more than four digits per tower (G-sampler lane kernel)");
    if (ctx->env.rng_compat) return fail("unsupported under MXX_HIP_RNG_COMPAT=reference");
    const double sigma_large = std::sqrt(cache->s * cache->s - cache->sigma * cache->sigma);
    if (!(sigma_large > 0.0) || !(cache->sigma > 0.0)) return fail("invalid Gaussian widths in the covariance cache");
    if (ctx_activate(ctx)) return 1;
    const PreimageCall call{ctx, re, public_matrix, cache, base_bits, sigma_large, d, dk};
    const size_t poly_bytes = L * static_cast<size_t>(ctx->N) * ctx->word_bytes;
    std::vector<size_t> group;
    size_t group_bytes = 0;
    for (size_t j = 0; j < n; ++j) {
        if (targets[j]->cols == 0) continue;
        const size_t bytes = dk * ((targets[j]->cols + d - 1) / d * d) * poly_bytes;
        if (!group.empty() && (group.size() == kGroupMax || group_bytes + bytes > kGroupBytes)) {
            const int rc = preimage_group(call, targets, seeds, outs, group);
            if (rc) return rc;
            group.clear();
            group_bytes = 0;
        }
        group.push_back(j);
        group_bytes += bytes;
    }
    if (!group.empty()) {
        const int rc = preimage_group(call, targets, seeds, outs, group);
        if (rc) return rc;
    }
    for (size_t j = 0; j < n; ++j) outs[j]->format = GPU_POLY_FORMAT_EVAL;
    return 0;
    ABI_GUARD_END
}

extern "C" int gpupoly_trapdoor_preimage_keyed(const GpuMatrix *const *res, const GpuP1CovarianceCache *const *caches,
                                               const GpuMatrix *const *public_matrices, size_t nkeys, uint32_t base_bits,
                                               const uint32_t *key_of, const GpuMatrix *const *targets, size_t n,
                                               const GpuRngSeed *seeds, GpuMatrix *const *outs) {
    ABI_GUARD_BEGIN
    static const char *const who = "gpupoly_trapdoor_preimage_keyed";
    auto refuse = [&](const std::string &what) { return set_error(std::string(who) + ": " + what); };
    if (nkeys > 0 && (!res || !caches || !public_matrices)) return refuse("null array of trapdoors, covariance caches or public matrices");
    if (n > 0 && (!key_of || !targets || !seeds || !outs)) return refuse("null key_of, targets, seeds or outputs");
    if (nkeys == 0 && n > 0) return refuse("requests without keys");
    if (base_bits == 0 || base_bits >= 63) return refuse("invalid base_bits");
    for (size_t k = 0; k < nkeys; ++k)
        if (!res[k] || !caches[k] || !public_matrices[k])
            return refuse("null trapdoor, covariance cache or public matrix in key " + std::to_string(k));
    if (nkeys == 0) return 0;
    GpuContext *ctx = res[0]->ctx;
    const int level = res[0]->level;
    const size_t d = public_matrices[0]->rows, L = matrix_limbs(res[0]);
    const uint32_t dpt = (ctx->crt_bits + base_bits - 1) / base_bits;
    const size_t top = 2 * d, dk = d * dpt * L;
    for (size_t k = 0; k < nkeys; ++k) {
        const GpuMatrix *re = res[k], *a = public_matrices[k];
        const GpuP1CovarianceCache *cache = caches[k];
        const std::string at = " in key " + std::to_string(k);
        if (re->ctx != ctx || cache->ctx != ctx || a->ctx != ctx) return refuse("context mismatch" + at);
        if (re->level != level || cache->level != level || a->level != level) return refuse("level mismatch" + at);
        if (a->rows != d) return refuse("keys of different trapdoor dimension d" + at);
        if (d == 0 || re->rows != top || re->cols != dk || a->cols != top + dk || cache->d != d || cache->m != top)
            return refuse("shape mismatch" + at + ": needs [R; E] 2d x dk, A d x (2d + dk) and a covariance cache of dimension d");
        if (re->format != GPU_POLY_FORMAT_EVAL || a->format != GPU_POLY_FORMAT_EVAL)
            return refuse("[R; E] and the public matrix must be in EVAL form" + at);
    }
    for (size_t j = 0; j < n; ++j) {
        const GpuMatrix *t = targets[j], *o = outs[j];
        const std::string js = std::to_string(j);
        if (key_of[j] >= nkeys) return refuse("key_of[" + js + "] out of range");
        if (!t || !o) return refuse("null target or output " + js);
        if (t->ctx != ctx || o->ctx != ctx) return refuse("context mismatch in request " + js);
        if (t->level != level || o->level != level) return refuse("level mismatch in request " + js);
    }
    for (size_t j = 0; j < n; ++j) {
        const GpuMatrix *o = outs[j];
        bool alias = false;
        for (size_t k = 0; k < nkeys && !alias; ++k) alias = words_overlap(o, res[k]) || words_overlap(o, public_matrices[k]);
        for (size_t i = 0; i < n && !alias; ++i) alias = words_overlap(o, targets[i]) || (i != j && words_overlap(o, outs[i]));
        if (alias) return refuse("output " + std::to_string(j) + " aliases a key's [R; E] or A, a target or another output");
    }
    for (size_t j = 0; j < n; ++j) {
        const GpuMatrix *t = targets[j], *o = outs[j];
        const std::string js = std::to_string(j);
        if (t->rows != d) return refuse("target " + js + " must have d rows");
        if (o->rows != top + dk || o->cols != t->cols) return refuse("output " + js + " must be (2d + dk) x its target's columns");
        if (t->format != GPU_POLY_FORMAT_EVAL) return refuse("target " + js + " must be in EVAL form");
        if (t->cols >> 31) return refuse("target " + js + " too wide");
    }
    if ((static_cast<size_t>(ctx->N) >> 1) % SAMPLER_THREADS)
        return refuse("unsupported: ring dimension not a multiple of 128 (segmented samplers)");
    if (top > 8) return refuse("unsupported: trapdoor dimension above 4 (no p1 lane kernel)");
    if (ctx->env.p1_simple) return refuse("unsupported under MXX_HIP_P1=simple (the p1 lane kernel is switched off)");
    if (dpt > 4) return refuse("unsupported: more than four digits per tower (G-sampler lane kernel)");
    if (ctx->env.rng_compat) return refuse("unsupported under MXX_HIP_RNG_COMPAT=reference");
    for (size_t k = 1; k < nkeys; ++k)
        if (caches[k]->sigma != caches[0]->sigma || caches[k]->s != caches[0]->s || caches[k]->dgg_stddev != caches[0]->dgg_stddev)
            return refuse("unsupported: the covariance caches of key 0 and key " + std::to_string(k) + " carry different widths");
    const GpuP1CovarianceCache *cache0 = caches[0];
    const double sigma_large = std::sqrt(cache0->s * cache0->s - cache0->sigma * cache0->sigma);
    if (!(sigma_large > 0.0) || !(cache0->sigma > 0.0)) return refuse("invalid Gaussian widths in the covariance caches");
    std::vector<size_t> order;
    for (size_t j = 0; j < n; ++j)
        if (targets[j]->cols) order.push_back(j);
    std::stable_sort(order.begin(), order.end(), [&](size_t x, size_t y) { return key_of[x] < key_of[y]; });
    const size_t poly_bytes = L * static_cast<size_t>(ctx->N) * ctx->word_bytes;
    std::vector<std::vector<size_t>> groups;
    size_t group_bytes = 0;
    for (size_t j : order) {
        const size_t bytes = dk * ((targets[j]->cols + d - 1) / d * d) * poly_bytes;
        if (groups.empty() || groups.back().size() == kGroupMax || group_bytes + bytes > kGroupBytes) {
            groups.emplace_back();
            group_bytes = 0;
// ... 51 lines not shown
```

mxx_amd/csrc/rng.h:

```cpp
#pragma once

#include <hip/hip_runtime.h>
#include <stdint.h>
#include <type_traits>
#include <cstdlib>

#include "detmath.h"

struct ChaChaRng {
    uint32_t state[16];
    uint32_t *ring;
    uint32_t ring_stride;
    uint32_t head;
    uint32_t tail;
};

#define RNG_RING_SLOTS 32
#ifndef RNG_DRAW_BITS
#define RNG_DRAW_BITS 16
#endif
#define RNG_DRAW_LOG (RNG_DRAW_BITS == 16 ? 1 : 2)
#define RNG_DRAW_MASK ((1u << RNG_DRAW_BITS) - 1u)
#define RNG_BLOCK_DRAWS (512u / RNG_DRAW_BITS)
#define RNG_U64_DRAWS (64 / RNG_DRAW_BITS)
// ... 436 lines not shown
    return (hi == 0 && lo == 0) ? 1 : lo;
}

template <typename RNG>
__device__ __forceinline__ void karney_heavy(KarneyFsm &f, RNG &rng) {
    if (f.st == KS_SIGN && rng_avail(rng) >= 1 + RNG_U64_DRAWS) {
        uint32_t w1;
        uint64_t w2;
        rng_next16_u64(rng, w1, w2);
        const bool neg = (w1 & 1u) == 0;
        const double di0 = f.stddev * static_cast<double>(f.k) + (neg ? -f.mean : f.mean);
        const double ci0 = ceil(di0);
        const double x0 = (ci0 - di0) / f.stddev;
        uint64_t j = w2 - __umul64hi(w2, f.magic) * f.cs;
        while (j >= f.cs) j -= f.cs;
        const double x = x0 + static_cast<double>(static_cast<int64_t>(j)) / f.stddev;
        if (!(x < 1.0) || (x == 0.0 && neg && f.k == 0)) {
            const int32_t it = f.iter + 1;
            f.iter = it;
            f.k = 0;
            f.in_p = false;
            karney_open_h(f);
            if (it >= (1 << 16)) f.st = KS_FALLBACK;
        } else {
            f.b_left = f.k + 1;
            f.x = x;
            f.xt_hi = karney_ticks_hi(x);
            f.bt_hi = karney_ticks_hi(karney_b1_threshold(f.k, x));
            f.T_hi = f.xt_hi;
            f.cnt = 0;
            f.T_own_cnt = f.zz_own_cnt = KARNEY_NO_OWN;
            const int64_t mag = static_cast<int64_t>(ci0) + static_cast<int64_t>(j);
            f.result = neg ? -mag : mag;
            f.st = KS_B;
        }
    } else if (f.st == KS_TIE && rng_avail(rng) >= 2 * ((KARNEY_LO_BITS + RNG_DRAW_BITS - 1) / RNG_DRAW_BITS)) {
        const bool is_b = f.tie_st == KS_B, odd = (f.cnt & 1u) != 0;
        uint64_t tlo;
        if (!is_b) {
            if (f.cnt == 0) tlo = 0;
            else if (f.T_own_cnt == f.cnt) tlo = f.T_lo;
            else tlo = karney_draw_lo(rng, f.T_hi);
        } else if (odd) {
            tlo = karney_ticks(karney_b1_threshold(f.k, f.x)) & KARNEY_LO_MASK;
        } else {
            if (f.cnt == 0) tlo = karney_ticks(f.x) & KARNEY_LO_MASK;
            else if (f.zz_own_cnt == f.cnt - 2) tlo = f.zz_lo;
            else tlo = karney_draw_lo(rng, f.T_hi);
        }
        const uint64_t ulo = karney_draw_lo(rng, f.tie_h);
        f.st = static_cast<int32_t>(f.tie_st);
        karney_advance<true>(f, ulo < tlo, f.tie_h, ulo);
    } else if (f.st == KS_FALLBACK && rng_avail(rng) >= 2 * RNG_U64_DRAWS) {
        f.result = static_cast<int64_t>(llround(f.mean + f.stddev * rng_standard_normal(rng)));
        f.st = KS_DONE;
    }
}

static __device__ int64_t sample_integer_karney(ChaChaRng &rng, double mean, double stddev) {
    KarneyFsm f;
    karney_reset(f);
    karney_begin(f, mean, stddev, karney_divisor(stddev));
    for (uint32_t step = 0; f.st != KS_DONE; ++step) {
        if ((step & 7) == 0) rng_fill_lane(rng);
        karney_heavy(f, rng);
        karney_light(f, rng);
    }
    return f.result;
}

#ifndef SAMPLER_PER_LANE_CAP
#define SAMPLER_PER_LANE_CAP 8
#endif
constexpr uint32_t kSamplerPerLaneCap = SAMPLER_PER_LANE_CAP;
#ifndef GAUSS_GROUP_LOG
#define GAUSS_GROUP_LOG 1
#endif
#ifndef SAMPLER_THREADS
#define SAMPLER_THREADS 64
#endif
#define RNG_MAX_SEGMENTS 64
struct RngSegments {
    uint32_t count;
    uint32_t start[RNG_MAX_SEGMENTS + 1];
    ChaChaKey key[RNG_MAX_SEGMENTS];
};
struct NoSegments {};
template <bool SEG>
using SegArg = typename std::conditional<SEG, RngSegments, NoSegments>::type;

#if defined(__HIPCC__)
__device__ __forceinline__ uint32_t rng_segment_of(const RngSegments &s, uint32_t col) {
    uint32_t lo = 0, hi = s.count;
    while (hi - lo > 1) {
        const uint32_t mid = (lo + hi) >> 1;
        if (col >= s.start[mid]) lo = mid;
        else hi = mid;
    }
    return lo;
}
#endif

static inline bool rng_segments_build(RngSegments &out, const GpuRngSeed *seeds, const size_t *seg_cols, size_t nseg,
                                      uint64_t domain_tag, size_t total_cols) {
    if (nseg == 0 || nseg > RNG_MAX_SEGMENTS || !seeds || !seg_cols) return false;
    size_t at = 0;
    out.count = static_cast<uint32_t>(nseg);
    for (size_t j = 0; j < nseg; ++j) {
        if (seg_cols[j] == 0 || at + seg_cols[j] > 0xffffffffull) return false;
        out.start[j] = static_cast<uint32_t>(at);
        out.key[j] = chacha_subkey(seeds[j], 0, domain_tag);
        at += seg_cols[j];
    }
    for (size_t j = nseg; j <= RNG_MAX_SEGMENTS; ++j) out.start[j] = static_cast<uint32_t>(at);
    for (size_t j = nseg; j < RNG_MAX_SEGMENTS; ++j) out.key[j] = ChaChaKey{};
    return at == total_cols;
}

struct RngBlockTable {
    const ChaChaKey *keys;
    const uint64_t *starts;
    uint64_t cols;
    uint32_t nblk, keys_per_block;
    uint64_t win_cols = 0, full_ncol = 0, col_offset = 0;
};
struct RngBlockRef {
    uint32_t blk;
    uint64_t local;
};

#if defined(__HIPCC__)
__device__ __forceinline__ RngBlockRef rng_block_of(const RngBlockTable &t, uint64_t p) {
    const uint64_t row = p / t.cols, col = p - row * t.cols;
    RngBlockRef r;
    if (t.win_cols) {
        const uint64_t blk = col / t.win_cols;
        r.blk = static_cast<uint32_t>(blk);
        r.local = row * t.full_ncol + t.col_offset + (col - blk * t.win_cols);
        return r;
    }
    if (!t.starts) {
        r.blk = static_cast<uint32_t>(row);
        r.local = col;
        return r;
    }
    uint32_t lo = 0, hi = t.nblk;
    while (hi - lo > 1) {
        const uint32_t mid = (lo + hi) >> 1;
        if (col >= t.starts[mid]) lo = mid;
        else hi = mid;
    }
    const uint64_t first = t.starts[lo];
    r.blk = lo;
    r.local = row * (t.starts[lo + 1] - first) + (col - first);
    return r;
}
#endif

struct GpuContext;
void launch_gauss_blocks(GpuContext *ctx, int64_t *stage, size_t polys, const RngBlockTable &table, double sigma);

static inline uint32_t sampler_per_lane(size_t total, const void *kernel, int device, int forced) {
    if (forced >= 1) return static_cast<uint32_t>(forced);
    int blocks_per_cu = 0, cus = 0;
    if (hipOccupancyMaxActiveBlocksPerMultiprocessor(&blocks_per_cu, kernel, SAMPLER_THREADS, 0) != hipSuccess || blocks_per_cu < 1)
        blocks_per_cu = 2;
    if (hipDeviceGetAttribute(&cus, hipDeviceAttributeMultiprocessorCount, device) != hipSuccess || cus < 1) cus = 256;
    const size_t lanes = static_cast<size_t>(blocks_per_cu) * cus * SAMPLER_THREADS;
    const size_t per = (total + lanes - 1) / lanes;
    return static_cast<uint32_t>(per < 1 ? 1 : (per > kSamplerPerLaneCap ? kSamplerPerLaneCap : per));
}
```

mxx_amd/csrc/runtime.hip:

```cpp
#include "common.h"

#include <algorithm>
#include <cstdlib>
#include <iterator>
#include <map>
#include <cstring>
#include <dlfcn.h>

typedef unsigned __int128 u128h;

static thread_local std::string g_last_error;

int set_error(const char *msg) {
    g_last_error = msg ? msg : "unknown error";
    return 1;
}
int set_error(const std::string &msg) {
    g_last_error = msg;
    return 1;
}
int set_error(hipError_t err, const char *what) {
    g_last_error = std::string(what ? what : "hip call") + ": " + hipGetErrorString(err);
    (void)hipGetLastError();
    return 1;
// ... 217 lines not shown
void EnvSwitches::load() {
    *this = EnvSwitches();
    if (const char *e = std::getenv("MXX_HIP_NTT_PATH")) {
        if (e[0] == 'l') ntt_path = 1;
        else if (e[0] == 'g' && e[1] == 'e') ntt_path = 2;
        else if (e[0] == 'g' && e[1] == 'l') ntt_path = 3;
    }
    if (const char *e = std::getenv("MXX_HIP_NTT14")) ntt14 = e[0] == 'w' ? 1 : (e[0] == 'u' ? 2 : 0);
    if (const char *e = std::getenv("MXX_HIP_DECOMPOSE_FUSED")) decompose_fused = e[0] != '0';
    if (const char *e = std::getenv("MXX_HIP_MATMUL_PATH")) matmul_path = e[0];
    if (const char *e = std::getenv("MXX_HIP_MATMUL_TILE")) {
        if (e[0] && e[1] && e[2]) matmul_tile = ((e[0] - '0') * 100 + (e[1] - '0') * 10 + (e[2] - '0')) * 2 + (e[3] == 'p');
    }
    if (const char *e = std::getenv("MXX_HIP_GSAMP")) {
        gsamp_simple = e[0] == 's';
        gsamp_no_uni = e[0] == 'n';
    }
    if (const char *e = std::getenv("MXX_HIP_P1")) p1_simple = e[0] == 's';
    if (const char *e = std::getenv("MXX_HIP_NTT64")) ntt64_int = e[0] == 'i';
    if (const char *e = std::getenv("MXX_HIP_RNG_COMPAT")) rng_compat = e[0] == 'r';
    if (const char *e = std::getenv("MXX_HIP_SERDE")) serde_general = e[0] == 'g';
    if (const char *e = std::getenv("MXX_HIP_PACK24")) pack24 = !(std::strcmp(e, "0") == 0 || std::strcmp(e, "off") == 0);
    if (const char *e = std::getenv("MXX_HIP_SKINNY24")) {
        if (std::strcmp(e, "0") == 0) skinny24 = 1;
        else if (std::strncmp(e, "force", 5) == 0 && (e[5] == 0 || e[5] == ':')) {
            skinny24 = 2;
            if (e[5] == ':') skinny24_shape = skinny24_parse_shape(e + 6) ? skinny24_parse_shape(e + 6) : -1;
        }
    }
    if (const char *e = std::getenv("MXX_HIP_MUL_DECOMPOSE_MANY_BUDGET")) mul_decompose_many_budget = static_cast<size_t>(std::strtoull(e, nullptr, 10));
    if (const char *e = std::getenv("MXX_HIP_MUL_DECOMPOSE_PAIRS_BUDGET")) mul_decompose_pairs_budget = static_cast<size_t>(std::strtoull(e, nullptr, 10));
    if (const char *e = std::getenv("MXX_HIP_GADGET_SCALAR_BUDGET")) gadget_scalar_budget = static_cast<size_t>(std::strtoull(e, nullptr, 10));
    if (const char *e = std::getenv("MXX_HIP_CRT_RECOMPOSE_CHUNK_BYTES")) {
        const size_t v = static_cast<size_t>(std::strtoull(e, nullptr, 10));
        if (v >= 1) crt_recompose_chunk_bytes = v;
    }
    if (const char *e = std::getenv("MXX_HIP_MUL_SUM_PATH")) mul_sum_path = (e[0] == 't' || e[0] == 's') ? e[0] : 0;
    if (const char *e = std::getenv("MXX_HIP_SAMPLER_PER_LANE")) {
        const int v = std::atoi(e);
        if (v >= 1 && v <= 4096) sampler_per_lane = v;
    }
    if (const char *e = std::getenv("MXX_HIP_NTT_PHASE")) {
        const int v = std::atoi(e);
        if (v >= 0 && v <= 127) ntt_phase = v;
    }
    if (const char *e = std::getenv("MXX_HIP_SAMPLER_FILL_EVERY")) {
        const int v = std::atoi(e);
        if (v >= 1 && v <= 8) sampler_fill_every = v;
    }
}

static std::mutex g_registry_mutex;
static std::vector<GpuContext *> g_contexts;
bool ctx_is_registered(const GpuContext *ctx) {
    std::lock_guard<std::mutex> lk(g_registry_mutex);
    return std::find(g_contexts.begin(), g_contexts.end(), ctx) != g_contexts.end();
}

extern "C" int gpupoly_reload_env(void) {
    std::lock_guard<std::mutex> lk(g_registry_mutex);
    for (GpuContext *c : g_contexts) c->env.load();
    return 0;
}

int ctx_activate(const GpuContext *ctx) {
    HIP_TRY(hipSetDevice(ctx->device));
    return 0;
}

static size_t round_block(size_t bytes) {
    const size_t gran = bytes >= (size_t(1) << 20) ? (size_t(1) << 20) : 4096;
    return (bytes + gran - 1) / gran * gran;
}

static void cache_trim(GpuContext *ctx, size_t limit) {
    while (ctx->cached_bytes > limit && !ctx->free_blocks.empty()) {
        auto it = std::prev(ctx->free_blocks.end());
        (void)hipFree(it->second);
        ctx->cached_bytes -= it->first;
        ctx->free_blocks.erase(it);
    }
}

int ctx_alloc(GpuContext *ctx, size_t bytes, void **out) {
    *out = nullptr;
    if (bytes == 0) return 0;
    const size_t want = round_block(bytes);
    std::lock_guard<std::mutex> lk(ctx->alloc_mutex);
    auto it = ctx->free_blocks.lower_bound(want);
    if (it != ctx->free_blocks.end() && it->first <= want + want / 4) {
        *out = it->second;
        ctx->live_blocks[*out] = it->first;
        ctx->cached_bytes -= it->first;
        ctx->free_blocks.erase(it);
        return 0;
    }
    hipError_t e = hipMalloc(out, want);
    if (e != hipSuccess) {
        (void)hipGetLastError();
        cache_trim(ctx, 0);
        e = hipMalloc(out, want);
    }
    if (e != hipSuccess) {
        (void)hipGetLastError();
        {
            std::lock_guard<std::mutex> reg(g_registry_mutex);
            for (GpuContext *other : g_contexts) {
                if (other == ctx || other->device != ctx->device) continue;
                if (!other->alloc_mutex.try_lock()) continue;
                cache_trim(other, 0);
                other->alloc_mutex.unlock();
            }
        }
        e = hipMalloc(out, want);
        if (e != hipSuccess) {
            *out = nullptr;
            return set_error(e, "hipMalloc");
        }
    }
    ctx->live_blocks[*out] = want;
    return 0;
}

void ctx_free(GpuContext *ctx, void *ptr) {
    if (!ptr) return;
    std::lock_guard<std::mutex> lk(ctx->alloc_mutex);
    auto it = ctx->live_blocks.find(ptr);
    if (it == ctx->live_blocks.end()) {
        (void)hipFree(ptr);
        return;
    }
    const size_t size = it->second;
    ctx->live_blocks.erase(it);
    if (!ctx->pool_ok) {
        (void)hipFree(ptr);
        return;
    }
    ctx->free_blocks.emplace(size, ptr);
    ctx->cached_bytes += size;
    cache_trim(ctx, ctx->cache_limit);
}

template <typename W>
static int upload_tables(GpuContext *ctx, const std::vector<std::vector<uint64_t>> &fwd,
                         const std::vector<std::vector<uint64_t>> &inv) {
    const size_t N = ctx->N, L = ctx->limb_count;
    const unsigned shift = sizeof(W) * 8;
    std::vector<W> h_f(L * N), h_fs(L * N), h_i(L * N), h_is(L * N);
    for (size_t l = 0; l < L; ++l) {
        uint64_t q = ctx->moduli[l];
        for (size_t j = 0; j < N; ++j) {
            h_f[l * N + j] = (W)fwd[l][j];
            h_fs[l * N + j] = (W)(((u128h)fwd[l][j] << shift) / q);
            h_i[l * N + j] = (W)inv[l][j];
            h_is[l * N + j] = (W)(((u128h)inv[l][j] << shift) / q);
        }
    }
    size_t bytes = L * N * sizeof(W);
    HIP_TRY(hipMalloc(&ctx->d_tw_fwd, bytes));
    HIP_TRY(hipMalloc(&ctx->d_tw_fwd_sh, bytes));
    HIP_TRY(hipMalloc(&ctx->d_tw_inv, bytes));
    HIP_TRY(hipMalloc(&ctx->d_tw_inv_sh, bytes));
    HIP_TRY(hipMemcpy(ctx->d_tw_fwd, h_f.data(), bytes, hipMemcpyHostToDevice));
    HIP_TRY(hipMemcpy(ctx->d_tw_fwd_sh, h_fs.data(), bytes, hipMemcpyHostToDevice));
    HIP_TRY(hipMemcpy(ctx->d_tw_inv, h_i.data(), bytes, hipMemcpyHostToDevice));
    HIP_TRY(hipMemcpy(ctx->d_tw_inv_sh, h_is.data(), bytes, hipMemcpyHostToDevice));
    std::vector<W> h_pf(2 * L * N), h_pi(2 * L * N);
    for (size_t i = 0; i < L * N; ++i) {
        h_pf[2 * i] = static_cast<W>(0) - h_f[i];
        h_pf[2 * i + 1] = h_fs[i];
        h_pi[2 * i] = h_i[i];
        h_pi[2 * i + 1] = h_is[i];
    }
    HIP_TRY(hipMalloc(&ctx->d_tw2_fwd, 2 * bytes));
    HIP_TRY(hipMalloc(&ctx->d_tw2_inv, 2 * bytes));
    HIP_TRY(hipMemcpy(ctx->d_tw2_fwd, h_pf.data(), 2 * bytes, hipMemcpyHostToDevice));
    HIP_TRY(hipMemcpy(ctx->d_tw2_inv, h_pi.data(), 2 * bytes, hipMemcpyHostToDevice));
    if (sizeof(W) == 8 && ctx->crt_bits <= 51 && N >= 2) {
        struct HostTwF { double w, wi; };
        struct HostF64Limb { double q, qinv; HostTwF n_inv, last_w; };
        std::vector<HostTwF> tf(L * N), ti(L * N);
        std::vector<HostF64Limb> fl(L);
        for (size_t l = 0; l < L; ++l) {
            const double qd = static_cast<double>(ctx->moduli[l]);
            for (size_t j = 0; j < N; ++j) {
                tf[l * N + j] = {static_cast<double>(fwd[l][j]), static_cast<double>(fwd[l][j]) / qd};
                ti[l * N + j] = {static_cast<double>(inv[l][j]), static_cast<double>(inv[l][j]) / qd};
            }
            const LimbConst &lc = ctx->limbs[l];
            fl[l] = {qd, 1.0 / qd, {static_cast<double>(lc.n_inv), static_cast<double>(lc.n_inv) / qd},
                     {static_cast<double>(lc.inv_last_w), static_cast<double>(lc.inv_last_w) / qd}};
        }
        HIP_TRY(hipMalloc(&ctx->d_twf_fwd, sizeof(HostTwF) * L * N));
        HIP_TRY(hipMalloc(&ctx->d_twf_inv, sizeof(HostTwF) * L * N));
        HIP_TRY(hipMalloc(&ctx->d_flimbs, sizeof(HostF64Limb) * L));
        HIP_TRY(hipMemcpy(ctx->d_twf_fwd, tf.data(), sizeof(HostTwF) * L * N, hipMemcpyHostToDevice));
        HIP_TRY(hipMemcpy(ctx->d_twf_inv, ti.data(), sizeof(HostTwF) * L * N, hipMemcpyHostToDevice));
        HIP_TRY(hipMemcpy(ctx->d_flimbs, fl.data(), sizeof(HostF64Limb) * L, hipMemcpyHostToDevice));
        ctx->f64_ok = true;
    }
    if (ctx->signed_ok && sizeof(W) == 4) {
        auto signed_pair = [](uint64_t w, uint64_t q, W *dst) {
            const int64_t c = w > q / 2 ? static_cast<int64_t>(w) - static_cast<int64_t>(q) : static_cast<int64_t>(w);
            __int128 num = static_cast<__int128>(c) << 32;
            __int128 fl = num / static_cast<__int128>(q);
            if (num % static_cast<__int128>(q) < 0) fl -= 1;
            dst[0] = static_cast<W>(static_cast<uint32_t>(static_cast<int32_t>(c)));
            dst[1] = static_cast<W>(static_cast<uint32_t>(static_cast<int32_t>(fl)));
        };
        for (size_t l = 0; l < L; ++l)
            for (size_t j = 0; j < N; ++j) signed_pair(inv[l][j], ctx->moduli[l], &h_pi[2 * (l * N + j)]);
        HIP_TRY(hipMalloc(&ctx->d_tw2s_inv, 2 * bytes));
        HIP_TRY(hipMemcpy(ctx->d_tw2s_inv, h_pi.data(), 2 * bytes, hipMemcpyHostToDevice));
    }
    return 0;
}

static void context_release(GpuContext *ctx) {
    if (!ctx) return;
    {
        std::lock_guard<std::mutex> reg(g_registry_mutex);
        g_contexts.erase(std::remove(g_contexts.begin(), g_contexts.end(), ctx), g_contexts.end());
    }
    (void)hipSetDevice(ctx->device);
    if (ctx->stream) (void)hipStreamSynchronize(ctx->stream);
    for (auto &kv : ctx->free_blocks) (void)hipFree(kv.second);
    for (auto &kv : ctx->live_blocks) (void)hipFree(kv.first);
    if (ctx->d_limbs) (void)hipFree(ctx->d_limbs);
    if (ctx->d_limbs_r) (void)hipFree(ctx->d_limbs_r);
    if (ctx->d_twf_fwd) (void)hipFree(ctx->d_twf_fwd);
    if (ctx->d_twf_inv) (void)hipFree(ctx->d_twf_inv);
    if (ctx->d_flimbs) (void)hipFree(ctx->d_flimbs);
    if (ctx->d_tw_fwd) (void)hipFree(ctx->d_tw_fwd);
    if (ctx->d_tw_fwd_sh) (void)hipFree(ctx->d_tw_fwd_sh);
    if (ctx->d_tw_inv) (void)hipFree(ctx->d_tw_inv);
    if (ctx->d_tw_inv_sh) (void)hipFree(ctx->d_tw_inv_sh);
    if (ctx->d_garner) (void)hipFree(ctx->d_garner);
    if (ctx->d_tw2_fwd) (void)hipFree(ctx->d_tw2_fwd);
    if (ctx->d_tw2_inv) (void)hipFree(ctx->d_tw2_inv);
    if (ctx->d_tw2s_inv) (void)hipFree(ctx->d_tw2s_inv);
    for (auto &kv : ctx->gadget_weights) (void)hipFree(kv.second);
    for (auto &kv : ctx->gadget_const_tables) (void)hipFree(kv.second);
    if (ctx->timer_start) (void)hipEventDestroy(ctx->timer_start);
    if (ctx->timer_stop) (void)hipEventDestroy(ctx->timer_stop);
    for (hipEvent_t ev : ctx->marks)
        if (ev) (void)hipEventDestroy(ev);
    if (ctx->stream) (void)hipStreamDestroy(ctx->stream);
    delete ctx;
}

extern "C" int gpu_context_create(uint32_t logN, uint32_t L, uint32_t dnum, const uint64_t *moduli,
                                  size_t moduli_len, const int *gpu_ids, size_t gpu_ids_len, GpuContext **out_ctx) {
    ABI_GUARD_BEGIN
    if (!out_ctx) return set_error("gpu_context_create: null out_ctx");
    *out_ctx = nullptr;
    if (!moduli || moduli_len == 0) return set_error("gpu_context_create: empty moduli");
    if (moduli_len != static_cast<size_t>(L) + 1) return set_error("gpu_context_create: moduli_len must equal L+1");
    if (moduli_len > GPUPOLY_MAX_LIMBS) return set_error("gpu_context_create: too many limbs");
    if (!gpu_ids || gpu_ids_len == 0) return set_error("gpu_context_create: empty gpu_ids");
    if (logN < 1 || logN > 17) return set_error("gpu_context_create: logN out of range [1,17]");
    int dev_count = 0;
    HIP_TRY(hipGetDeviceCount(&dev_count));
    for (size_t i = 0; i < gpu_ids_len; ++i) {
        if (gpu_ids[i] < 0 || gpu_ids[i] >= dev_count) return set_error("gpu_context_create: invalid gpu id");
        for (size_t j = 0; j < i; ++j)
            if (gpu_ids[j] == gpu_ids[i]) return set_error("gpu_context_create: duplicate gpu id");
    }
    const uint64_t N = 1ull << logN;
    bool wide = false;
    for (size_t i = 0; i < moduli_len; ++i) {
        uint64_t q = moduli[i];
        if (q < 3 || (q - 1) % (2 * N) != 0) return set_error("gpu_context_create: modulus must be = 1 (mod 2N)");
        if (!h_is_prime(q)) return set_error("gpu_context_create: modulus is not prime");
        if (q >> 62) return set_error("gpu_context_create: modulus must be < 2^62");
        if (q >> 31) wide = true;
        for (size_t j = 0; j < i; ++j)
            if (moduli[j] == q) return set_error("gpu_context_create: duplicate modulus");
    }

    GpuContext *ctx = new GpuContext();
    ctx->device = gpu_ids[0];
    ctx->gpu_ids.assign(gpu_ids, gpu_ids + gpu_ids_len);
    ctx->logN = logN;
    ctx->N = static_cast<int>(N);
    ctx->level = static_cast<int>(L);
    ctx->dnum = dnum;
    ctx->limb_count = static_cast<int>(moduli_len);
    ctx->wide = wide;
    ctx->word_bytes = wide ? 8 : 4;
    ctx->moduli.assign(moduli, moduli + moduli_len);

    hipError_t e = hipSetDevice(ctx->device);
    if (e != hipSuccess) { delete ctx; return set_error(e, "hipSetDevice"); }
    e = hipStreamCreateWithFlags(&ctx->stream, hipStreamNonBlocking);
    if (e != hipSuccess) { delete ctx; return set_error(e, "hipStreamCreate"); }

    ctx->env.load();
    {
        ctx->pool_ok = true;
        size_t free_b = 0, total_b = 0;
        ctx->cache_limit = size_t(64) << 30;
        if (hipMemGetInfo(&free_b, &total_b) == hipSuccess && free_b) ctx->cache_limit = free_b / 2;
        else (void)hipGetLastError();
        const char *env = std::getenv("MXX_HIP_MEMPOOL_RELEASE_THRESHOLD_BYTES");
        if (!env) env = std::getenv("MXX_CUDA_MEMPOOL_RELEASE_THRESHOLD_BYTES");
        if (env && *env) ctx->cache_limit = std::strtoull(env, nullptr, 10);
        const char *nopool = std::getenv("MXX_HIP_DISABLE_MEMPOOL");
        if (nopool && *nopool == '1') ctx->pool_ok = false;
    }

    std::vector<std::vector<uint64_t>> fwd(moduli_len), inv(moduli_len);
    ctx->limbs.resize(moduli_len);
    uint32_t crt_bits = 0;
    for (size_t l = 0; l < moduli_len; ++l) {
        uint64_t q = moduli[l];
        uint64_t psi = h_min_primitive_root(q, 2 * N);
        uint64_t ipsi = h_invmod_prime(psi, q);
        fwd[l].resize(N);
        inv[l].resize(N);
        uint64_t p = 1, ip = 1;
        for (uint64_t i = 0; i < N; ++i) {
            uint32_t r = h_bitrev(static_cast<uint32_t>(i), logN);
            fwd[l][r] = p;
            inv[l][r] = ip;
            p = h_mulmod(p, psi, q);
            ip = h_mulmod(ip, ipsi, q);
        }
        LimbConst &lc = ctx->limbs[l];
        lc.q = q;
        lc.kbits = h_bits(q);
        crt_bits = std::max(crt_bits, lc.kbits);
        lc.mu = static_cast<uint64_t>((((u128h)1) << (2 * lc.kbits)) / q);
        lc.mu64 = static_cast<uint64_t>((((u128h)1) << 64) / q);
        lc.n_inv = h_invmod_prime(N % q, q);
        lc.n_inv_sh = static_cast<uint64_t>(((u128h)lc.n_inv << (wide ? 64 : 32)) / q);
        lc.mu32 = (((uint64_t)1) << 32) / q;
        lc.inv_last_w = h_mulmod(inv[l][1 % N], lc.n_inv, q);
        lc.inv_last_w_sh = static_cast<uint64_t>(((u128h)lc.inv_last_w << (wide ? 64 : 32)) / q);
        if (!wide) {
            u128h q2 = (u128h)(q - 1) * (q - 1);
            u128h terms = ((((u128h)1) << 64) - q) / q2;
            lc.lazy_terms = terms > (1u << 20) ? (1u << 20) : static_cast<uint32_t>(terms);
        } else {
            u128h q2 = (u128h)(q - 1) * (q - 1);
            u128h terms = (~(u128h)0 - q) / q2;
            lc.lazy_terms = terms > (1u << 20) ? (1u << 20) : static_cast<uint32_t>(terms);
        }
    }
    ctx->crt_bits = crt_bits;
    ctx->lazy_ok = crt_bits + 7 <= (wide ? 64u : 32u);
    ctx->tight_ok = !wide && !ctx->lazy_ok && crt_bits + 4 <= 32u;
    ctx->signed_ok = !wide && crt_bits <= 24;
    ctx->pack24_ok = !wide && crt_bits <= 24 && ctx->N % 4 == 0;

    ctx->garner_inv.assign(moduli_len * moduli_len, 0);
    for (size_t i = 0; i < moduli_len; ++i)
        for (size_t j = 0; j < i; ++j)
            ctx->garner_inv[i * moduli_len + j] = h_invmod_prime(moduli[j] % moduli[i], moduli[i]);

    int rc = 0;
    e = hipMalloc(&ctx->d_limbs, sizeof(LimbConst) * moduli_len);
    if (e == hipSuccess)
        e = hipMemcpy(ctx->d_limbs, ctx->limbs.data(), sizeof(LimbConst) * moduli_len, hipMemcpyHostToDevice);
    if (e == hipSuccess) e = hipMalloc(&ctx->d_garner, sizeof(uint64_t) * moduli_len * moduli_len);
    if (e == hipSuccess)
        e = hipMemcpy(ctx->d_garner, ctx->garner_inv.data(), sizeof(uint64_t) * moduli_len * moduli_len,
                      hipMemcpyHostToDevice);
    if (e == hipSuccess && !wide) {
        std::vector<LimbConst> lr = ctx->limbs;
        for (LimbConst &c : lr) {
            const uint64_t r = (1ull << 32) % c.q;
            c.n_inv = h_mulmod(c.n_inv, r, c.q);
            c.n_inv_sh = static_cast<uint64_t>(((u128h)c.n_inv << 32) / c.q);
            c.inv_last_w = h_mulmod(c.inv_last_w, r, c.q);
            c.inv_last_w_sh = static_cast<uint64_t>(((u128h)c.inv_last_w << 32) / c.q);
        }
        e = hipMalloc(&ctx->d_limbs_r, sizeof(LimbConst) * moduli_len);
        if (e == hipSuccess) e = hipMemcpy(ctx->d_limbs_r, lr.data(), sizeof(LimbConst) * moduli_len, hipMemcpyHostToDevice);
    }
    if (e != hipSuccess) rc = set_error(e, "context constant upload");
    if (!rc) rc = wide ? upload_tables<uint64_t>(ctx, fwd, inv) : upload_tables<uint32_t>(ctx, fwd, inv);
    if (!rc) {
        e = hipEventCreate(&ctx->timer_start);
        if (e == hipSuccess) e = hipEventCreate(&ctx->timer_stop);
        if (e != hipSuccess) rc = set_error(e, "hipEventCreate");
    }
    if (rc) {
        std::string keep = g_last_error;
        context_release(ctx);
        g_last_error = keep;
        return rc;
    }
    {
        std::lock_guard<std::mutex> reg(g_registry_mutex);
        g_contexts.push_back(ctx);
    }
    *out_ctx = ctx;
    return 0;
    ABI_GUARD_END
}

extern "C" void gpu_context_destroy(GpuContext *ctx) { context_release(ctx); }

extern "C" int gpu_context_get_N(const GpuContext *ctx, int *out_N) {
    if (!ctx || !out_N) return set_error("gpu_context_get_N: null argument");
    *out_N = ctx->N;
    return 0;
}

extern "C" int gpupoly_context_device(const GpuContext *ctx, int *out_device) {
    if (!ctx || !out_device) return set_error("gpupoly_context_device: null argument");
    *out_device = ctx->device;
    return 0;
}

extern "C" int gpupoly_context_stream(const GpuContext *ctx, void **out_stream) {
    if (!ctx || !out_stream) return set_error("gpupoly_context_stream: null argument");
    *out_stream = static_cast<void *>(ctx->stream);
    return 0;
}

extern "C" const char *gpupoly_context_last_kernel(const GpuContext *ctx) { return ctx ? ctx->last_kernel.load() : ""; }

extern "C" int gpupoly_context_word_bytes(const GpuContext *ctx, int *out_bytes) {
    if (!ctx || !out_bytes) return set_error("gpupoly_context_word_bytes: null argument");
    *out_bytes = ctx->word_bytes;
    return 0;
}

extern "C" int gpu_event_set_wait(GpuEventSet *events) {
    ABI_GUARD_BEGIN
    if (!events) return 0;
    HIP_TRY(hipSetDevice(events->device));
    for (hipEvent_t ev : events->events) HIP_TRY(hipEventSynchronize(ev));
    return 0;
    ABI_GUARD_END
}

extern "C" void gpu_event_set_destroy(GpuEventSet *events) {
    if (!events) return;
    (void)hipSetDevice(events->device);
    for (hipEvent_t ev : events->events) {
        (void)hipEventSynchronize(ev);
        (void)hipEventDestroy(ev);
    }
    if (events->staging) (void)hipHostFree(events->staging);
    if (events->dev_staging && events->ctx) ctx_free(events->ctx, events->dev_staging);
    delete events;
}

extern "C" int gpu_device_count(int *out_count) {
    ABI_GUARD_BEGIN
    if (!out_count) return set_error("gpu_device_count: null out_count");
    int n = 0;
    hipError_t e = hipGetDeviceCount(&n);
    if (e != hipSuccess) {
        *out_count = 0;
        return set_error(e, "hipGetDeviceCount");
    }
    *out_count = n;
    return 0;
    ABI_GUARD_END
}

extern "C" int gpu_device_mem_info(int device, size_t *out_free, size_t *out_total) {
    ABI_GUARD_BEGIN
    if (!out_free || !out_total) return set_error("gpu_device_mem_info: null output");
    int prev = 0;
    HIP_TRY(hipGetDevice(&prev));
    HIP_TRY(hipSetDevice(device));
    hipError_t e = hipMemGetInfo(out_free, out_total);
    (void)hipSetDevice(prev);
    if (e != hipSuccess) return set_error(e, "hipMemGetInfo");
    return 0;
    ABI_GUARD_END
}

extern "C" int gpupoly_device_can_access_peer(int device, int peer, int *out_can) {
    ABI_GUARD_BEGIN
    if (!out_can) return set_error("gpupoly_device_can_access_peer: null output");
    *out_can = 0;
    if (device == peer) {
        *out_can = 1;
        return 0;
    }
    HIP_TRY(hipDeviceCanAccessPeer(out_can, device, peer));
    return 0;
    ABI_GUARD_END
}

extern "C" int gpu_device_synchronize(void) {
    ABI_GUARD_BEGIN
    int n = 0;
    HIP_TRY(hipGetDeviceCount(&n));
    int prev = 0;
    HIP_TRY(hipGetDevice(&prev));
    for (int d = 0; d < n; ++d) {
        HIP_TRY(hipSetDevice(d));
        HIP_TRY(hipDeviceSynchronize());
    }
    HIP_TRY(hipSetDevice(prev));
// ... 74 lines not shown
```

mxx_amd/csrc/trapdoor.hip:

```cpp
#include "common.h"
#include "modarith.h"
#include "rng.h"

#include <algorithm>
#include <cstdlib>

static constexpr uint64_t kTagGadget = 0x6761646765746731ull;
static constexpr uint64_t kTagP1 = 0x7065727475726231ull;
static constexpr int kGaussMaxDigits = 64;

__host__ __device__ __forceinline__ uint64_t gadget_stream0(uint32_t i, uint32_t t) {
    return ((static_cast<uint64_t>(i) + 1) << 8) | (static_cast<uint64_t>(t) + 1);
}

template <typename W, int MAXD>
__global__ void __launch_bounds__(128) gauss_samp_gq_kernel(W *__restrict__ out, const W *__restrict__ src,
                                     const LimbConst *__restrict__ limbs, size_t src_polys, uint32_t src_cols,
                                     uint32_t L, uint32_t N, uint32_t dpt, uint32_t base_bits, double c, size_t k,
                                     GpuRngSeed seed) {
    __shared__ uint32_t ring[128 * RNG_RING_SLOTS];
    const size_t idx = item_index();
    const size_t total = src_polys * L * N;
    if (idx >= total) return;
    const uint32_t i = static_cast<uint32_t>(idx % N);
// ... 80 lines not shown
    for (int d = 0; d < MAXD; ++d) {
        if (d < last) z[d] = sample_integer_karney(rng, -a[d], sigma);
        else z[d] = z_last;
    }

    const size_t r = p / src_cols, col = p - r * src_cols;
    int64_t z_prev = 0;
#pragma unroll
    for (int d = 0; d < MAXD; ++d) {
        if (d < (int)dpt) {
            int64_t digit;
            if (dpt == 1) digit = static_cast<int64_t>(base) * z[0] + m_digits[0] * z[0] + v_digits[0];
            else if (d == 0) digit = static_cast<int64_t>(base) * z[0] + m_digits[0] * z_last + v_digits[0];
            else if (d < last) digit = static_cast<int64_t>(base) * z[d] - z_prev + m_digits[d] * z_last + v_digits[d];
            else digit = m_digits[d] * z_last - z_prev + v_digits[d];
            z_prev = z[d];
            const size_t orow = r * k + static_cast<size_t>(t) * dpt + d;
            const size_t opoly = orow * src_cols + col;
            for (uint32_t l = 0; l < L; ++l)
                out[(opoly * L + l) * N + i] = signed_to_residue_mu<W>(digit, limbs[l].q, limbs[l].mu64);
        }
    }
}

struct GqTower {
    double c_last, sd;
    KarneyDivisor div;
    double cvec[4];
};

__global__ void gq_tower_kernel(GqTower *__restrict__ towers, const LimbConst *__restrict__ limbs, uint32_t L,
                                uint32_t dpt, uint32_t base_bits, double c) {
    const uint32_t t = blockIdx.x * blockDim.x + threadIdx.x;
    if (t >= L) return;
    const uint64_t base = 1ull << base_bits;
    const double base_f = static_cast<double>(base);
    const double sigma = c / (base_f + 1.0);
    const uint64_t qt = limbs[t].q;
    double c_last = 0.0;
    GqTower g;
    for (uint32_t d = 0; d < 4; ++d) g.cvec[d] = 0.0;
    for (uint32_t d = 0; d < dpt; ++d) {
        c_last = (c_last + static_cast<double>(static_cast<int64_t>((qt >> (base_bits * d)) & (base - 1)))) / base_f;
        if (d < 4) g.cvec[d] = c_last;
    }
    g.c_last = c_last;
    g.sd = sigma / c_last;
    g.div = karney_divisor(g.sd);
    towers[t] = g;
}

struct GqPertConsts {
    double ld[4], hn[4];
};

static inline GqPertConsts gq_pert_consts(uint32_t dpt, uint32_t base_bits) {
    GqPertConsts k{};
    const double base_f = static_cast<double>(1ull << base_bits), kf = static_cast<double>(dpt);
    for (uint32_t d = 0; d < 4 && d < dpt; ++d) {
        k.ld[d] = d == 0 ? sqrt(base_f * (1.0 + 1.0 / kf) + 1.0) : sqrt(base_f * (1.0 + 1.0 / (kf - static_cast<double>(d))));
        k.hn[d] = sqrt(base_f * (1.0 - 1.0 / (kf - static_cast<double>(d))));
    }
    return k;
}

template <typename W, int MAXD, bool SEG = false>
__global__ void __launch_bounds__(256) gauss_samp_prep_kernel(double *__restrict__ a_out, uint64_t *__restrict__ left_out,
                                       const W *__restrict__ src, const LimbConst *__restrict__ limbs,
                                       ChaChaKey key, size_t total, uint32_t L, uint32_t logN,
                                       uint32_t dpt, uint32_t base_bits, double c, GqPertConsts pc,
                                       uint32_t src_cols, SegArg<SEG> segs) {
    static_assert(MAXD <= 4, "GqPertConsts holds four digits");
    const size_t idx = item_index();
    if (idx >= total) return;
    const uint32_t i = static_cast<uint32_t>(idx & ((1u << logN) - 1));
    const uint32_t pt = static_cast<uint32_t>(idx >> logN);
    uint32_t p = pt / L;
    const uint32_t t = pt - p * L;
    if constexpr (SEG) {
        const uint32_t p_u = static_cast<uint32_t>(__builtin_amdgcn_readfirstlane(p));
        const uint32_t row = p_u / src_cols, col = p_u - row * src_cols;
        const uint32_t j = rng_segment_of(segs, col);
        key = segs.key[j];
        p = row * (segs.start[j + 1] - segs.start[j]) + (col - segs.start[j]);
    }
    const uint64_t qt = limbs[t].q;
    uint64_t value = static_cast<uint64_t>(src[idx]);
    if (value >= qt) value %= qt;
    const uint64_t base = 1ull << base_bits;
    const double base_f = static_cast<double>(base);
    const double sigma = c / (base_f + 1.0);

    uint64_t w[8];
    chacha_block_words(key, gadget_stream0(i, t), static_cast<uint64_t>(p) + 1, 0, w);
    double zf[MAXD];
#pragma unroll
    for (int d = 0; d < MAXD; ++d)
        zf[d] = d < (int)dpt ? sigma * (sqrt(-2.0 * det_log(u64_to_open01(w[2 * d]))) * det_cos2pi(u64_to_open01(w[2 * d + 1]))) : 0.0;
#pragma unroll
    for (int j = 0; j < 8; ++j)
        if (j >= 2 * (int)dpt) left_out[static_cast<size_t>(j - 2 * (int)dpt) * total + idx] = w[j];
    double prev_a = 0.0;
#pragma unroll
    for (int d = 0; d < MAXD; ++d) {
        if (d < (int)dpt) {
            double pd;
            if (d + 1 < (int)dpt) pd = pc.ld[d] * zf[d] + pc.hn[d] * zf[d + 1 < MAXD ? d + 1 : d];
            else pd = (d == 0 ? 0.0 : pc.hn[d - 1 < 0 ? 0 : d - 1]) * zf[d];
            const double vd = static_cast<double>(static_cast<int64_t>((value >> (base_bits * d)) & (base - 1)));
            const double ad = (prev_a + vd - pd) / base_f;
            prev_a = ad;
            a_out[static_cast<size_t>(d) * total + idx] = ad;
        }
    }
}

template <typename W, int MAXD, int SV, bool UNI = false, bool SEG = false>
__global__ void __launch_bounds__(SAMPLER_THREADS, 4) gauss_samp_lanes_kernel(int64_t *__restrict__ stage,
                                        const LimbConst *__restrict__ limbs, ChaChaKey key,
                                        const GqTower *__restrict__ towers, const double *__restrict__ a_in,
                                        const uint64_t *__restrict__ left_in, size_t total, uint32_t src_cols,
                                        uint32_t L, uint32_t logN, uint32_t dpt, uint32_t base_bits, double c,
                                        KarneyDivisor div_sigma, uint32_t per_lane, uint32_t fill_every,
                                        SegArg<SEG> segs) {
    static_assert(!SEG || UNI, "segments need a wave's chunk inside one polynomial");
    __shared__ uint32_t ring[SAMPLER_THREADS * RNG_RING_SLOTS];
    const uint64_t base = 1ull << base_bits;
    const double base_f = static_cast<double>(base);
    const double sigma = c / (base_f + 1.0);
    const int last = static_cast<int>(dpt) - 1;
    const uint32_t nleft = 8 - 2 * dpt;
    WaveChunk chunk = wave_chunk(total, per_lane);
    const uint32_t pt_u = static_cast<uint32_t>(__builtin_amdgcn_readfirstlane(static_cast<uint32_t>(chunk.base >> logN)));
    uint32_t p_u = pt_u / L;
    const uint32_t t_u = pt_u - p_u * L;
    const GqTower tw_u = towers[UNI ? t_u : 0];
    if constexpr (SEG) {
        const uint32_t row = p_u / src_cols, col = p_u - row * src_cols;
        const uint32_t j = rng_segment_of(segs, col);
        key = segs.key[j];
        p_u = row * (segs.start[j + 1] - segs.start[j]) + (col - segs.start[j]);
    }

    ChaChaRng rng;
    rng_init_keyed(rng, ring, key, 0, 0, SAMPLER_THREADS);
    KarneyFsm f;
    karney_reset(f);
    bool fin = true, have = false;
    uint32_t ph = 0;
    size_t idx = 0;
    uint32_t tower = 0;
    double a[MAXD];
    int64_t z[MAXD];
    int64_t z_last = 0;
#pragma unroll
    for (int d = 0; d < MAXD; ++d) { a[d] = 0.0; z[d] = 0; }

    auto integer_ready = [&]() {
        if (f.st == KS_DONE && !fin) {
            if (ph == 0) {
                z_last = f.result;
                const double zl = static_cast<double>(z_last);
#pragma unroll
                for (int d = 0; d < MAXD; ++d)
                    if (d < (int)dpt) a[d] += zl * (UNI ? tw_u.cvec[d] : towers[tower].cvec[d]);
            } else {
#pragma unroll
                for (int d = 0; d < MAXD; ++d)
                    if (d == (int)ph - 1) z[d] = f.result;
            }
            ++ph;
            if (ph == dpt) {
                fin = true;
            } else {
                double an = 0.0;
#pragma unroll
                for (int d = 0; d < MAXD; ++d)
                    if (d == (int)ph - 1) an = a[d];
                karney_begin(f, -an, sigma, div_sigma);
            }
        }
    };
    auto element_done = [&]() {
        const bool take = f.st == KS_DONE && fin;
        if (take && have) {
#pragma unroll
            for (int d = 0; d < MAXD; ++d) {
                if (d < (int)dpt) {
                    stage[idx * dpt + d] = d < last ? z[d] : z_last;
                }
            }
        }
        const uint32_t e = wave_take(chunk, take);
        if (take) {
            have = e < chunk.len;
            if (have) {
                idx = chunk.base + e;
                const uint32_t i = static_cast<uint32_t>(idx & ((1u << logN) - 1));
                uint32_t p, t;
                if constexpr (UNI) {
                    p = p_u;
                    t = t_u;
                } else {
                    const uint32_t pt = static_cast<uint32_t>(idx >> logN);
                    p = pt / L;
                    t = pt - p * L;
                }
                tower = t;
                rng_reopen(rng, gadget_stream0(i, t), static_cast<uint64_t>(p) + 1, 1);
                const uint32_t slot0 = (rng.tail >> RNG_DRAW_LOG) & (RNG_RING_SLOTS - 1);
                for (uint32_t w = 0; w < nleft; ++w) {
                    const uint64_t lw = left_in[static_cast<size_t>(w) * total + idx];
                    rng.ring[(slot0 + 4 * dpt + 2 * w) * rng.ring_stride] = static_cast<uint32_t>(lw);
                    rng.ring[(slot0 + 4 * dpt + 2 * w + 1) * rng.ring_stride] = static_cast<uint32_t>(lw >> 32);
                }
                rng.head = rng.tail + 2 * RNG_U64_DRAWS * dpt;
                rng.tail += RNG_BLOCK_DRAWS;
                double a_last = 0.0;
#pragma unroll
                for (int d = 0; d < MAXD; ++d) {
                    if (d < (int)dpt) {
                        a[d] = a_in[static_cast<size_t>(d) * total + idx];
                        a_last = a[d];
                    }
// ... 145 lines not shown
    MXX_TRACE_BYTES(static_cast<double>(total) * (sizeof(W) + static_cast<double>(dpt) * L * sizeof(W)));
#define LAUNCH_GS(MAXD)                                                                                        \
    MXX_LAUNCH((gauss_samp_gq_kernel<W, MAXD>), dim3(blocks), dim3(128), 0, ctx->stream, out, src,      \
                       ctx->d_limbs, polys, src_cols, L, N, dpt, base_bits, c, k, seed)
    if (dpt <= 2) LAUNCH_GS(2);
    else if (dpt <= 4) LAUNCH_GS(4);
    else if (dpt <= 8) LAUNCH_GS(8);
    else if (dpt <= 20) LAUNCH_GS(20);
    else LAUNCH_GS(64);
#undef LAUNCH_GS
    HIP_TRY(hipGetLastError());
    return 0;
}

static int gauss_samp_impl(GpuMatrix *src, uint32_t base_bits, double c, GpuRngSeed seed, GpuMatrix *out, const RngSegments *segs);

extern "C" int gpu_matrix_gauss_samp_gq_arb_base(GpuMatrix *src, uint32_t base_bits, double c, double dgg_stddev,
                                                 GpuRngSeed seed, GpuMatrix *out) {
    ABI_GUARD_BEGIN
    (void)dgg_stddev;
    return gauss_samp_impl(src, base_bits, c, seed, out, nullptr);
    ABI_GUARD_END
}

extern "C" int gpupoly_matrix_gauss_samp_gq_arb_base_segments(GpuMatrix *src, uint32_t base_bits, double c, double dgg_stddev,
                                                              const GpuRngSeed *seeds, const size_t *seg_cols, size_t nseg,
                                                              GpuMatrix *out) {
    ABI_GUARD_BEGIN
    (void)dgg_stddev;
    if (!src || !out) return set_error("invalid gpupoly_matrix_gauss_samp_gq_arb_base_segments arguments");
    if (static_cast<size_t>(src->ctx->N) % SAMPLER_THREADS)
        return set_error("gpupoly_matrix_gauss_samp_gq_arb_base_segments: unsupported: ring too small for a wave per polynomial chunk");
    RngSegments segs;
    if (!rng_segments_build(segs, seeds, seg_cols, nseg, kTagGadget, src->cols))
        return set_error("gpupoly_matrix_gauss_samp_gq_arb_base_segments: segments must be 1..64, non-empty and cover the source's columns");
    return gauss_samp_impl(src, base_bits, c, GpuRngSeed{}, out, &segs);
    ABI_GUARD_END
}

static int gauss_samp_impl(GpuMatrix *src, uint32_t base_bits, double c, GpuRngSeed seed, GpuMatrix *out, const RngSegments *segs) {
    {
    if (!src || !out) return set_error("invalid gpu_matrix_gauss_samp_gq_arb_base arguments");
    if (base_bits == 0 || base_bits >= 63) return set_error("invalid base_bits in gpu_matrix_gauss_samp_gq_arb_base");
    if (!(c > 0.0)) return set_error("c must be positive in gpu_matrix_gauss_samp_gq_arb_base");
    if (src->ctx != out->ctx || src->level != out->level)
        return set_error("context mismatch in gpu_matrix_gauss_samp_gq_arb_base");
    GpuContext *ctx = src->ctx;
    const int requested = out->format;
    const size_t L = matrix_limbs(src);
    const uint32_t dpt = (ctx->crt_bits + base_bits - 1) / base_bits;
    if (dpt == 0 || dpt > kGaussMaxDigits)
        return set_error("invalid digits_per_tower in gpu_matrix_gauss_samp_gq_arb_base");
    const size_t k = static_cast<size_t>(dpt) * L;
    if (out->rows != src->rows * k || out->cols != src->cols)
        return set_error("output size mismatch in gpu_matrix_gauss_samp_gq_arb_base");
    if (storage_overlaps(src, out)) return set_error("gpu_matrix_gauss_samp_gq_arb_base: output must not alias the source");
    const size_t polys = matrix_polys(src);
    if (polys == 0) {
        out->format = GPU_POLY_FORMAT_EVAL;
        return 0;
    }
    if (ctx_activate(ctx)) return 1;
    if (src->format == GPU_POLY_FORMAT_EVAL) {
        int rc = gpu_matrix_intt_all(src);
        if (rc) return rc;
    }
    int rc = ctx->wide ? launch_gauss_samp<uint64_t>(ctx, static_cast<uint64_t *>(words_ptr(out)),
                                                     static_cast<const uint64_t *>(words_ptr(src)), polys,
                                                     (uint32_t)src->cols, (uint32_t)L, dpt, base_bits, c, k, seed, segs)
                       : launch_gauss_samp<uint32_t>(ctx, static_cast<uint32_t *>(words_ptr(out)),
                                                     static_cast<const uint32_t *>(words_ptr(src)), polys,
                                                     (uint32_t)src->cols, (uint32_t)L, dpt, base_bits, c, k, seed, segs);
    if (rc) return rc;
    out->format = GPU_POLY_FORMAT_COEFF;
    if (requested == GPU_POLY_FORMAT_EVAL) {
        rc = launch_ntt(ctx, words_ptr(out), matrix_polys(out) * L, static_cast<int>(L), false);
        if (rc) return rc;
        out->format = GPU_POLY_FORMAT_EVAL;
    }
    return 0;
    }
}

struct P1KeyedSegments {
    RngSegments segs;
    const P1KeyEntry *keys;
};
template <typename W>
__global__ void p1_covariance_kernel(const W *__restrict__ a_mat, const W *__restrict__ b_mat,
                                     const W *__restrict__ d_mat, uint32_t d, uint32_t L, uint32_t N, uint64_t q0,
                                     double sigma, double s, double dgg_stddev, double *__restrict__ cov_ws,
                                     double *__restrict__ sqrt_var_out, double *__restrict__ update_out) {
    const uint32_t i = blockIdx.x * blockDim.x + threadIdx.x;
    if (i >= N) return;
    const uint32_t m = 2 * d;
    double *cov = cov_ws + static_cast<size_t>(i) * m * m;
    double *sqrt_var = sqrt_var_out + static_cast<size_t>(i) * m;
    double *upd = update_out + static_cast<size_t>(i) * m * m;
    const double sigma2 = sigma * sigma, s2 = s * s, fallback = dgg_stddev * dgg_stddev, eps = 1e-9;
    for (uint32_t r = 0; r < d; ++r)
        for (uint32_t c = 0; c < d; ++c) {
            const size_t rc = (static_cast<size_t>(r) * d + c) * L * N + i;
            const size_t cr = (static_cast<size_t>(c) * d + r) * L * N + i;
            const double a_rc = static_cast<double>(centered_residue(a_mat[rc], q0));
            const double d_rc = static_cast<double>(centered_residue(d_mat[rc], q0));
            const double b_rc = static_cast<double>(centered_residue(b_mat[rc], q0));
            const double b_cr = static_cast<double>(centered_residue(b_mat[cr], q0));
            cov[r * m + c] = -sigma2 * a_rc + (r == c ? s2 : 0.0);
            cov[(r + d) * m + (c + d)] = -sigma2 * d_rc + (r == c ? s2 : 0.0);
            cov[r * m + (c + d)] = -sigma2 * b_rc;
            cov[(r + d) * m + c] = -sigma2 * b_cr;
        }
    for (int t = static_cast<int>(m) - 1; t >= 0; --t) {
        double var = cov[t * m + t];
        if (!(var > eps)) var = fallback;
        sqrt_var[t] = sqrt(var);
        for (int r = 0; r < t; ++r) upd[t * m + r] = cov[r * m + t] / var;
        if (t == 0) break;
        for (int r = 0; r < t; ++r) {
            const double cr = upd[t * m + r];
            for (int c = 0; c <= r; ++c) {
                const double colc = upd[t * m + c] * var;
                const double v = cov[r * m + c] - cr * colc;
                cov[r * m + c] = v;
                cov[c * m + r] = v;
            }
        }
    }
}

template <typename W, int MAXM>
__global__ void __launch_bounds__(128) p1_sample_kernel(W *__restrict__ out, const W *__restrict__ tp2,
                                 const LimbConst *__restrict__ limbs, const double *__restrict__ sqrt_var_base,
                                 const double *__restrict__ update_base, uint32_t m, uint32_t cols, uint32_t L,
                                 uint32_t N, uint64_t q0, double c_scale, GpuRngSeed seed,
                                 double *__restrict__ mean_ws) {
    __shared__ uint32_t ring[128 * RNG_RING_SLOTS];
    const size_t idx = item_index();
    if (idx >= static_cast<size_t>(cols) * N) return;
    const uint32_t col = static_cast<uint32_t>(idx / N);
    const uint32_t i = static_cast<uint32_t>(idx - static_cast<size_t>(col) * N);
    const double *sqrt_var = sqrt_var_base + static_cast<size_t>(i) * m;
    const double *upd = update_base + static_cast<size_t>(i) * m * m;
    ChaChaRng rng;
    rng_init(rng, ring, seed, static_cast<uint64_t>(col) + 1, static_cast<uint64_t>(i) + 1, 0, kTagP1);

    if constexpr (MAXM > 0) {
        double mean[MAXM];
#pragma unroll
        for (int r = 0; r < MAXM; ++r)
            mean[r] = r < (int)m ? c_scale * static_cast<double>(centered_residue(
                                                 tp2[((static_cast<size_t>(r) * cols + col) * L) * N + i], q0))
                                 : 0.0;
#pragma unroll
        for (int t = MAXM - 1; t >= 0; --t) {
            if (t >= (int)m) continue;
            const double mu = mean[t];
            const int64_t z = sample_integer_karney(rng, mu, sqrt_var[t]);
            for (uint32_t l = 0; l < L; ++l)
                out[((static_cast<size_t>(t) * cols + col) * L + l) * N + i] =
                    signed_to_residue_mu<W>(z, limbs[l].q, limbs[l].mu64);
            const double delta = static_cast<double>(z) - mu;
#pragma unroll
            for (int r = 0; r < MAXM; ++r)
                if (r < t) mean[r] += upd[t * m + r] * delta;
        }
    } else {
        double *mean = mean_ws + idx * m;
        for (uint32_t r = 0; r < m; ++r)
            mean[r] = c_scale * static_cast<double>(centered_residue(
                                    tp2[((static_cast<size_t>(r) * cols + col) * L) * N + i], q0));
        for (int t = static_cast<int>(m) - 1; t >= 0; --t) {
            const double mu = mean[t];
            const int64_t z = sample_integer_karney(rng, mu, sqrt_var[t]);
            for (uint32_t l = 0; l < L; ++l)
                out[((static_cast<size_t>(t) * cols + col) * L + l) * N + i] =
                    signed_to_residue_mu<W>(z, limbs[l].q, limbs[l].mu64);
            const double delta = static_cast<double>(z) - mu;
            for (int r = 0; r < t; ++r) mean[r] += upd[t * m + r] * delta;
        }
    }
}

__global__ void p1_divisor_kernel(KarneyDivisor *__restrict__ div, const double *__restrict__ sqrt_var, size_t count) {
    const size_t idx = item_index();
    if (idx < count) div[idx] = karney_divisor(sqrt_var[idx]);
}

template <bool SEG, bool KEYED>
using P1SegArg = typename std::conditional<KEYED, P1KeyedSegments, SegArg<SEG>>::type;
template <typename T>
__device__ __forceinline__ const T *wave_uniform_ptr(const void *p) {
    const uint64_t v = reinterpret_cast<uint64_t>(p);
    const uint32_t lo = __builtin_amdgcn_readfirstlane(static_cast<uint32_t>(v));
    const uint32_t hi = __builtin_amdgcn_readfirstlane(static_cast<uint32_t>(v >> 32));
    return reinterpret_cast<const T *>((static_cast<uint64_t>(hi) << 32) | lo);
}
template <typename W, int MAXM, int SV, bool SEG = false, bool KEYED = false>
__global__ void __launch_bounds__(SAMPLER_THREADS) p1_sample_lanes_kernel(int64_t *__restrict__ stage, const W *__restrict__ tp2,
                                       const double *__restrict__ sqrt_var_base, const double *__restrict__ update_base,
                                       const KarneyDivisor *__restrict__ div_base, uint32_t m, uint32_t cols, uint32_t L,
                                       uint32_t logN, uint64_t q0, double c_scale, ChaChaKey key, size_t total,
                                       uint32_t per_lane, uint32_t fill_every, P1SegArg<SEG, KEYED> segs) {
    static_assert(SEG || !KEYED, "the keyed form is a form of the segment path");
    __shared__ uint32_t ring[SAMPLER_THREADS * RNG_RING_SLOTS];
    WaveChunk chunk = wave_chunk(total, per_lane);
    uint32_t seg_col0 = 0;
    if constexpr (KEYED) {
        const uint32_t col_u = static_cast<uint32_t>(__builtin_amdgcn_readfirstlane(static_cast<uint32_t>(chunk.base >> logN)));
        const uint32_t j = rng_segment_of(segs.segs, col_u < cols ? col_u : cols - 1);
        key = segs.segs.key[j];
        seg_col0 = segs.segs.start[j];
        const P1KeyEntry e = segs.keys[j];
        sqrt_var_base = wave_uniform_ptr<double>(e.sqrt_var);
        update_base = wave_uniform_ptr<double>(e.update_coeff);
        div_base = wave_uniform_ptr<KarneyDivisor>(e.karney_div);
    } else if constexpr (SEG) {
        const uint32_t col_u = static_cast<uint32_t>(__builtin_amdgcn_readfirstlane(static_cast<uint32_t>(chunk.base >> logN)));
        const uint32_t j = rng_segment_of(segs, col_u < cols ? col_u : cols - 1);
        key = segs.key[j];
        seg_col0 = segs.start[j];
    }
    ChaChaRng rng;
    rng_init_keyed(rng, ring, key, 0, 0, SAMPLER_THREADS);
    KarneyFsm f;
    karney_reset(f);
    bool fin = true, have = false;
    uint32_t t = 0, col = 0, i = 0;
    double mean[MAXM], mu = 0.0;
#pragma unroll
    for (int r = 0; r < MAXM; ++r) mean[r] = 0.0;

    auto integer_ready = [&]() {
        if (f.st == KS_DONE && !fin) {
            const int64_t z = f.result;
            stage[((static_cast<size_t>(t) * cols + col) << logN) + i] = z;
            const double delta = static_cast<double>(z) - mu;
            const double *upd = update_base + (static_cast<size_t>(i) * m + t) * m;
#pragma unroll
            for (int r = 0; r < MAXM; ++r)
                if (r < (int)t) mean[r] += upd[r] * delta;
            if (t == 0) {
                fin = true;
            } else {
                --t;
#pragma unroll
                for (int r = 0; r < MAXM; ++r)
                    if (r == (int)t) mu = mean[r];
                const size_t sv = static_cast<size_t>(i) * m + t;
                karney_begin(f, mu, sqrt_var_base[sv], div_base[sv]);
            }
        }
    };
    auto element_done = [&]() {
        const bool take = f.st == KS_DONE && fin;
        const uint32_t e = wave_take(chunk, take);
        if (take) {
            have = e < chunk.len;
            if (have) {
                const size_t idx = chunk.base + e;
                col = static_cast<uint32_t>(idx >> logN);
                i = static_cast<uint32_t>(idx & ((1u << logN) - 1));
                const W *row = tp2 + ((static_cast<size_t>(col) * L) << logN) + i;
#pragma unroll
                for (int r = 0; r < MAXM; ++r)
                    if (r < (int)m) {
                        mean[r] = c_scale * static_cast<double>(centered_residue(*row, q0));
                        row += (static_cast<size_t>(cols) * L) << logN;
                    }
                rng_reopen(rng, static_cast<uint64_t>(col - seg_col0) + 1, static_cast<uint64_t>(i) + 1);
                t = m - 1;
#pragma unroll
                for (int r = 0; r < MAXM; ++r)
                    if (r == (int)t) mu = mean[r];
                fin = false;
                const size_t sv = static_cast<size_t>(i) * m + t;
                karney_begin(f, mu, sqrt_var_base[sv], div_base[sv]);
            } else {
                f.st = KS_IDLE;
            }
        }
    };
    for (uint32_t step = 0;; ++step) {
        integer_ready();
        element_done();
        if (__all(f.st == KS_IDLE)) break;
        rng_fill_wave(rng, f.st != KS_IDLE, step % fill_every == 0, 16, karney_urgent(SV));
        karney_heavy(f, rng);
#pragma unroll
        for (int s4 = 0; s4 < KARNEY_SUPERSTEP / SV; ++s4) karney_light(f, rng);
#pragma unroll
        for (int sv = 1; sv < SV; ++sv) {
            integer_ready();
            karney_heavy(f, rng);
#pragma unroll
            for (int s4 = 0; s4 < KARNEY_SUPERSTEP / SV; ++s4) karney_light(f, rng);
        }
    }
}

static int check_p1_inputs(const GpuMatrix *a, const GpuMatrix *b, const GpuMatrix *d, double sigma, double s,
                           double dgg_stddev, const char *who) {
    if (!a || !b || !d) return set_error(std::string("invalid ") + who + " arguments");
    if (!(sigma > 0.0) || !(s > sigma)) return set_error(std::string("invalid sigma/s in ") + who);
// ... 167 lines not shown
    MXX_LAUNCH((p1_sample_lanes_kernel<WT, MAXM, SV, SEG>), dim3(lblocks), dim3(SAMPLER_THREADS), 0, ctx->stream, \
               static_cast<int64_t *>(stage), static_cast<const WT *>(words_ptr(tp2)), cache->sqrt_var,                \
               cache->update_coeff, static_cast<const KarneyDivisor *>(cache->karney_div), (uint32_t)m,           \
               (uint32_t)cols, L, ctx->logN, ctx->moduli[0], c_scale, key, total, per_lane,                       \
               static_cast<uint32_t>(ctx->env.sampler_fill_every ? ctx->env.sampler_fill_every : 2), SEGARG)
#define LAUNCH_P1KEYED(WT, MAXM, SV)  \
    MXX_LAUNCH((p1_sample_lanes_kernel<WT, MAXM, SV, true, true>), dim3(lblocks), dim3(SAMPLER_THREADS), 0, ctx->stream, \
               static_cast<int64_t *>(stage), static_cast<const WT *>(words_ptr(tp2)), static_cast<const double *>(nullptr), \
               static_cast<const double *>(nullptr), static_cast<const KarneyDivisor *>(nullptr), (uint32_t)m,   \
               (uint32_t)cols, L, ctx->logN, ctx->moduli[0], c_scale, key, total, per_lane,                       \
               static_cast<uint32_t>(ctx->env.sampler_fill_every ? ctx->env.sampler_fill_every : 2), keyed_segs)
#define LAUNCH_P1L(WT, MAXM)                                                                                      \
    do {                                                                                                          \
        uint32_t per_lane =                                                                                       \
            sampler_per_lane(total, reinterpret_cast<const void *>(p1_sample_lanes_kernel<WT, MAXM, KARNEY_SERVICES>), ctx->device, ctx->env.sampler_per_lane); \
        if (segs)         \
            while ((static_cast<size_t>(N) / SAMPLER_THREADS) % per_lane) --per_lane;                             \
        const unsigned lblocks = static_cast<unsigned>((total + SAMPLER_THREADS * per_lane - 1) / (SAMPLER_THREADS * per_lane)); \
        if (segs && d_keys) {                                                                                     \
            const P1KeyedSegments keyed_segs{*segs, d_keys};                                                      \
            if (per_lane == 1) LAUNCH_P1KEYED(WT, MAXM, 1);                                                       \
            else LAUNCH_P1KEYED(WT, MAXM, KARNEY_SERVICES);                                                       \
        } else if (segs) {                                                                                        \
            if (per_lane == 1) LAUNCH_P1K(WT, MAXM, 1, true, *segs);                                              \
            else LAUNCH_P1K(WT, MAXM, KARNEY_SERVICES, true, *segs);                                              \
        } else if (per_lane == 1) {                                                                               \
            LAUNCH_P1K(WT, MAXM, 1, false, NoSegments{});                                                         \
        } else {                                                                                                  \
            LAUNCH_P1K(WT, MAXM, KARNEY_SERVICES, false, NoSegments{});                                           \
        }                                                                                                         \
    } while (0)
        if (ctx->wide) {
            if (m <= 2) LAUNCH_P1L(uint64_t, 2);
            else if (m <= 4) LAUNCH_P1L(uint64_t, 4);
            else LAUNCH_P1L(uint64_t, 8);
        } else {
            if (m <= 2) LAUNCH_P1L(uint32_t, 2);
            else if (m <= 4) LAUNCH_P1L(uint32_t, 4);
            else LAUNCH_P1L(uint32_t, 8);
        }
#undef LAUNCH_P1L
#undef LAUNCH_P1KEYED
#undef LAUNCH_P1K
        const hipError_t le = hipGetLastError();
        int lrc = le == hipSuccess ? launch_scatter_i64(out, static_cast<const int64_t *>(stage)) : 0;
        ctx_free(ctx, stage);
        if (le != hipSuccess) return set_error(le, "p1_sample_lanes_kernel");
        if (lrc) return lrc;
        lrc = launch_ntt(ctx, words_ptr(out), matrix_polys(out) * L, static_cast<int>(L), false);
        if (lrc) return lrc;
        out->format = GPU_POLY_FORMAT_EVAL;
        return 0;
    }
    const dim3 blocks = item_grid(total, 128);
    void *mean_ws = nullptr;
    if (m > 8 && ctx_alloc(ctx, total * m * sizeof(double), &mean_ws)) return 1;
#define LAUNCH_P1(WT, MAXM)                                                                                       \
    MXX_LAUNCH((p1_sample_kernel<WT, MAXM>), dim3(blocks), dim3(128), 0, ctx->stream,                      \
                       static_cast<WT *>(words_ptr(out)), static_cast<const WT *>(words_ptr(tp2)), ctx->d_limbs,             \
                       cache->sqrt_var, cache->update_coeff, (uint32_t)m, (uint32_t)cols, L, N, ctx->moduli[0],    \
                       c_scale, seed, static_cast<double *>(mean_ws))
    if (ctx->wide) {
        if (m <= 2) LAUNCH_P1(uint64_t, 2);
        else if (m <= 4) LAUNCH_P1(uint64_t, 4);
        else if (m <= 8) LAUNCH_P1(uint64_t, 8);
        else LAUNCH_P1(uint64_t, 0);
    } else {
        if (m <= 2) LAUNCH_P1(uint32_t, 2);
        else if (m <= 4) LAUNCH_P1(uint32_t, 4);
        else if (m <= 8) LAUNCH_P1(uint32_t, 8);
        else LAUNCH_P1(uint32_t, 0);
    }
#undef LAUNCH_P1
    hipError_t e = hipGetLastError();
    if (mean_ws) ctx_free(ctx, mean_ws);
    if (e != hipSuccess) return set_error(e, "p1_sample_kernel");
    int rc = launch_ntt(ctx, words_ptr(out), matrix_polys(out) * L, static_cast<int>(L), false);
    if (rc) return rc;
    out->format = GPU_POLY_FORMAT_EVAL;
    return 0;
    }
}

extern "C" int gpu_matrix_sample_p1_full(const GpuMatrix *a_mat, const GpuMatrix *b_mat, const GpuMatrix *d_mat,
                                         const GpuMatrix *tp2, double sigma, double s, double dgg_stddev,
                                         GpuRngSeed seed, GpuMatrix *out) {
    ABI_GUARD_BEGIN
    if (out && ((tp2 && storage_overlaps(tp2, out)) || (a_mat && storage_overlaps(a_mat, out)) ||
                (b_mat && storage_overlaps(b_mat, out)) || (d_mat && storage_overlaps(d_mat, out))))
        return set_error("gpu_matrix_sample_p1_full: output must not alias an input");
    GpuP1CovarianceCache *cache = nullptr;
    int rc = gpu_matrix_create_p1_covariance_cache(a_mat, b_mat, d_mat, sigma, s, dgg_stddev, &cache);
    if (rc) return rc;
    rc = gpu_matrix_sample_p1_full_cached(cache, tp2, seed, out);
    gpu_matrix_destroy_p1_covariance_cache(cache);
    return rc;
    ABI_GUARD_END
}
```

mxx_amd/trapdoor.py:

```python
from __future__ import annotations

import math
import threading
import weakref

from .matrix import GpuDCRTPolyMatrix
from .sampler import DistType, GpuDCRTPolyUniformSampler, random_gpu_rng_seed, sample_gpu_matrix_with_seed

SPECTRAL_CONSTANT = 1.8


def preimage_c(base: int, sigma: float) -> float:
    return (base + 1.0) * sigma


def preimage_smoothing_parameter(base: int, sigma: float, d: int, n: int, k: int) -> float:
    return SPECTRAL_CONSTANT * (base + 1.0) * sigma * sigma * (math.sqrt(d * n * k) + math.sqrt(2 * n) + 4.7)


def p1_covariance_parameters(params, d: int, dgg_stddev: float):
    base = 1 << params.base_bits()
    n, k = params.ring_dimension(), params.modulus_digits()
    return preimage_c(base, dgg_stddev), preimage_smoothing_parameter(base, dgg_stddev, d, n, k), dgg_stddev

# ... 71 lines not shown
    def clear_public_matrix_cache(self) -> None:
        with self._p1_lock:
            self._stacked = None
            self._replicas = {}

    def replica_for(self, params, public_matrix: GpuDCRTPolyMatrix):
        key = params.ctx_raw().value
        with self._p1_lock:
            hit = self._replicas.get(key)
            if hit is not None and hit[2]() is public_matrix and hit[3] == public_matrix.content_version():
                return hit[0], hit[1]
        td, a = self.to_params(params), public_matrix.to_params(params)
        with self._p1_lock:
            self._replicas[key] = (td, a, weakref.ref(public_matrix), public_matrix.content_version())
        return td, a

    def to_params(self, params) -> "GpuDCRTTrapdoor":
        return GpuDCRTTrapdoor(self.r.to_params(params), self.e.to_params(params))

    def to_compact_bytes(self) -> bytes:
        out = b""
        for m in (self.r, self.e):
            b = m.to_compact_bytes()
            out += len(b).to_bytes(8, "little") + b
        return out

    @classmethod
    def from_compact_bytes(cls, params, data: bytes):
        mats, off = [], 0
        for _ in range(2):
            if off + 8 > len(data):
                return None
            ln = int.from_bytes(data[off : off + 8], "little")
            off += 8
            if off + ln > len(data):
                return None
            mats.append(GpuDCRTPolyMatrix.from_compact_bytes(params, data[off : off + ln]))
            off += ln
        if off != len(data):
            return None
        return cls(mats[0], mats[1])

    def __eq__(self, other):
        return isinstance(other, GpuDCRTTrapdoor) and self.r == other.r and self.e == other.e

    __hash__ = None


WORKER_DNUM = 0x5700
_worker_params_cache: dict = {}
_worker_params_lock = threading.Lock()


def preimage_workers() -> int:
    import os

    try:
        return max(1, min(8, int(os.environ.get("MXX_PREIMAGE_WORKERS", "4"))))
    except ValueError:
        return 4


def worker_params(params, k: int):
    from .params import GpuDCRTPolyParams

    key = (params.ctx_raw().value, k)
    with _worker_params_lock:
        for dead in [kk for kk, (owner, _) in _worker_params_cache.items() if owner() is None]:
            del _worker_params_cache[dead]
        hit = _worker_params_cache.get(key)
        if hit is not None and hit[0]() is params.ctx():
            return hit[1]
        pw = GpuDCRTPolyParams(params.ring_dimension(), params.moduli(), params.base_bits(), gpu_ids=params.gpu_ids(), dnum=WORKER_DNUM + k)
        _worker_params_cache[key] = (weakref.ref(params.ctx()), pw)
        return pw


TRAFFIC_BOUND_BYTES = 32 << 20


def _traffic_bound(params, polys: int) -> bool:
    word = 4 if max(params.moduli()) < (1 << 31) else 8
    return polys * params.crt_depth() * params.ring_dimension() * word >= TRAFFIC_BOUND_BYTES


class GpuDCRTPolyTrapdoorSampler:
    def __init__(self, params, sigma: float):
        self.sigma = float(sigma)
        self.base = 1 << params.base_bits()
        self.c = preimage_c(self.base, self.sigma)

    @staticmethod
    def trapdoor_to_bytes(trapdoor: "GpuDCRTTrapdoor") -> bytes:
        return trapdoor.to_compact_bytes()

    @staticmethod
    def trapdoor_from_bytes(params, data: bytes):
        return GpuDCRTTrapdoor.from_compact_bytes(params, data)

    def trapdoor(self, params, size: int):
        u = GpuDCRTPolyUniformSampler()
        td = GpuDCRTTrapdoor.new(params, size, self.sigma)
        a_bar = u.sample_uniform(params, size, size, DistType.FinRingDist())
        g = GpuDCRTPolyMatrix.gadget_matrix(params, size)
        a0 = a_bar.concat_columns([GpuDCRTPolyMatrix.identity(params, size)])
        a1 = g - (a_bar * td.r + td.e)
        return td, a0.concat_columns([a1])

    def _sample_pert(self, params, td: GpuDCRTTrapdoor, s, c, dgg_stddev, sigma_large, total_ncol):
        return self._sample_pert_parts(params, td, s, c, dgg_stddev, sigma_large, total_ncol)[:2]

    def sample_pert_square_mat_gpu_native_parts(self, params, td, s, c, dgg_stddev, sigma_large, total_ncol):
        return GpuPerturbationSamples(*self._sample_pert(params, td, s, c, dgg_stddev, sigma_large, total_ncol))

    def sample_pert_square_mat_gpu_native(self, params, td, s, c, dgg_stddev, sigma_large, total_ncol):
        p1, p2 = self._sample_pert(params, td, s, c, dgg_stddev, sigma_large, total_ncol)
        assert p1.col_size() >= total_ncol and p2.col_size() >= total_ncol, "p1 / p2 must include the target columns"
        p_hat = GpuDCRTPolyMatrix(params, p1.row_size() + p2.row_size(), total_ncol, p1.level, p1.is_ntt)
        p_hat.copy_block_from(p1, 0, 0, 0, 0, p1.row_size(), total_ncol)
        p_hat.copy_block_from(p2, p1.row_size(), 0, 0, 0, p2.row_size(), total_ncol)
        return p_hat

    @staticmethod
    def _draw_seeds():
        return random_gpu_rng_seed(), random_gpu_rng_seed(), random_gpu_rng_seed()

    def _sample_pert_parts(self, params, td: GpuDCRTTrapdoor, s, c, dgg_stddev, sigma_large, total_ncol, stacked=None, seeds=None):
        d, dk = td.r.row_size(), td.r.col_size()
        padded = -(-total_ncol // d) * d
        seed_p2 = seeds[0] if seeds is not None else random_gpu_rng_seed()
        p2 = sample_gpu_matrix_with_seed(params, dk, padded, DistType.GaussDist(sigma_large), seed_p2)
        rp2 = tp2_eval = None
        if stacked is not None and _traffic_bound(params, dk * padded):
            t = stacked * p2
            re_rows = td.re.row_size()
            tp2 = t.slice(0, re_rows, 0, padded)
            tp2_eval = t.row_view(0, re_rows)
            rp2 = t.row_view(re_rows, t.row_size())
        else:
            tp2 = td.re * p2
            if _traffic_bound(params, dk * padded):
                tp2_eval = tp2.clone()
        cache = td.p1_covariance_cache(c, s, dgg_stddev)
        p1 = GpuDCRTPolyMatrix.sample_p1_full_cached(cache, tp2, seeds[1] if seeds is not None else random_gpu_rng_seed())
        return p1, p2, tp2_eval, rp2

    def preimage(self, params, td: GpuDCRTTrapdoor, public_matrix, target, _seeds=None) -> GpuDCRTPolyMatrix:
        d = public_matrix.row_size()
        target_cols = target.col_size()
        assert target.row_size() == d, "Target matrix should have the same number of rows as the public matrix"
        n, k = params.ring_dimension(), params.modulus_digits()
        s = preimage_smoothing_parameter(self.base, self.sigma, d, n, k)
        dgg_large_std = math.sqrt(s * s - self.c * self.c)
        p1_rows, p2_rows = td.re.row_size(), td.re.col_size()
        assert public_matrix.col_size() == p1_rows + p2_rows, "public matrix columns must match perturbation rows"
        left, right, stacked = td.public_matrix_parts(public_matrix)
        p1, p2, tp2, rp2 = self._sample_pert_parts(params, td, s, self.c, self.sigma, dgg_large_std, target_cols, stacked, _seeds)
        seed_z = _seeds[2] if _seeds is not None else None
        assert (p1.row_size(), p2.row_size()) == (p1_rows, p2_rows)
        p_hat_image = (left * p1) + (rp2 if rp2 is not None else right * p2)
        if p_hat_image.col_size() != target_cols:
            p_hat_image = p_hat_image.slice_columns(0, target_cols)
        perturbed = target - p_hat_image
        out = GpuDCRTPolyMatrix(params, p1_rows + p2_rows, target_cols, p1.level, p1.is_ntt)
        if p1.col_size() == target_cols and tp2 is not None:
            z = perturbed.gauss_samp_gq_arb_base(self.c, self.sigma, seed_z if seed_z is not None else random_gpu_rng_seed(), coeff_out=True)
            out.ntt_add_rows_from(p1_rows, z, p2, consume=True)
            re_x = td.re * out.row_view(p1_rows, p1_rows + p2_rows)
            out.add_rows_from(0, p1 - tp2, re_x)
            return out
        z_hat = perturbed.gauss_samp_gq_arb_base(self.c, self.sigma, seed_z if seed_z is not None else random_gpu_rng_seed())
        re_z = td.re * z_hat
        if p1.col_size() == target_cols:
            out.add_rows_from(0, p1, re_z)
            out.add_rows_from(p1_rows, p2, z_hat)
            return out
        out.copy_block_from(p1, 0, 0, 0, 0, p1_rows, target_cols)
        out.copy_block_from(p2, p1_rows, 0, 0, 0, p2_rows, target_cols)
        out.add_block_from(re_z, 0, 0, 0, 0, re_z.row_size(), target_cols)
        out.add_block_from(z_hat, 2 * d, 0, 0, 0, z_hat.row_size(), target_cols)
        return out

    def preimage_reference_sequence(self, params, td: GpuDCRTTrapdoor, public_matrix, target) -> GpuDCRTPolyMatrix:
        d = public_matrix.row_size()
        target_cols = target.col_size()
        assert target.row_size() == d, "Target matrix should have the same number of rows as the public matrix"
        n, k = params.ring_dimension(), params.modulus_digits()
        s = preimage_smoothing_parameter(self.base, self.sigma, d, n, k)
        dgg_large_std = math.sqrt(s * s - self.c * self.c)
        u = GpuDCRTPolyUniformSampler()
        dd, dk = td.r.row_size(), td.r.col_size()
        padded = -(-target_cols // dd) * dd
        p2 = u.sample_uniform(params, dk, padded, DistType.GaussDist(dgg_large_std))
        tp2 = td.r.concat_rows([td.e]) * p2
        cache = td.p1_covariance_cache(self.c, s, self.sigma)
        p1 = GpuDCRTPolyMatrix.sample_p1_full_cached(cache, tp2, random_gpu_rng_seed())
        p1_rows, p2_rows = p1.row_size(), p2.row_size()
        assert public_matrix.col_size() == p1_rows + p2_rows, "public matrix columns must match perturbation rows"
        public_left = public_matrix.slice(0, d, 0, p1_rows)
        public_right = public_matrix.slice(0, d, p1_rows, p1_rows + p2_rows)
        p_hat_image = (public_left * p1) + (public_right * p2)
        if p_hat_image.col_size() != target_cols:
            p_hat_image = p_hat_image.slice_columns(0, target_cols)
        perturbed = target - p_hat_image
        z_hat = perturbed.gauss_samp_gq_arb_base(self.c, self.sigma, random_gpu_rng_seed())
        r_z = td.r * z_hat
        out = GpuDCRTPolyMatrix(params, p1_rows + p2_rows, target_cols, p1.level, p1.is_ntt)
        out.copy_block_from(p1, 0, 0, 0, 0, p1_rows, target_cols)
        out.copy_block_from(p2, p1_rows, 0, 0, 0, p2_rows, target_cols)
        del p1, p2
        out.add_block_from(r_z, 0, 0, 0, 0, r_z.row_size(), target_cols)
        del r_z
        e_z = td.e * z_hat
        out.add_block_from(e_z, d, 0, 0, 0, e_z.row_size(), target_cols)
        del e_z
        out.add_block_from(z_hat, 2 * d, 0, 0, 0, z_hat.row_size(), target_cols)
        return out

    def preimage_extend(self, params, td, public_matrix, ext_matrix, target) -> GpuDCRTPolyMatrix:
        d = public_matrix.row_size()
        n, k = params.ring_dimension(), params.modulus_digits()
        s = preimage_smoothing_parameter(self.base, self.sigma, d, n, k)
        u = GpuDCRTPolyUniformSampler()
        right = u.sample_uniform(params, ext_matrix.col_size(), target.col_size(), DistType.GaussDist(s))
        t = target - (ext_matrix * right)
        left = self.preimage(params, td, public_matrix, t)
        return left.concat_rows([right])

    BATCH_BYTES = 1 << 30

    @staticmethod
    def _segments_supported(params, td: GpuDCRTTrapdoor) -> bool:
        import os

        dpt = -(-params.crt_bits() // params.base_bits())
        return (params.ring_dimension() % 128 == 0 and td.r.row_size() <= 4 and dpt <= 4
                and not os.environ.get("MXX_HIP_RNG_COMPAT", "").startswith("r")
                and not os.environ.get("MXX_HIP_P1", "").startswith("s")
                and os.environ.get("MXX_PREIMAGE_BATCH", "1") != "0")
# ... 205 lines not shown
```

Baseline: 7.929 million.

## Pipeline trapdoor preimage over two column windows on main and side streams

Adds a fused native preimage entry point that splits the target columns into two windows and runs the eight-stage perturbation/gadget-sampling/matmul chain interleaved, with one window on a side stream. The aim is to overlap kernels from the two windows and to cut Python-level launches and intermediate full-size matrices, using windowed RNG segments so results match the unwindowed path. It adds a thread-local stream redirection, a second stream with fork/join events, and small windowed elementwise kernels. The cost is extra complexity and possible contention between the two streams.

```diff
diff --git a/include/gpupoly.h b/include/gpupoly.h
--- a/include/gpupoly.h
+++ b/include/gpupoly.h
@@ -204,6 +204,8 @@
                                     const GpuMatrix *const *public_matrices, size_t nkeys, uint32_t base_bits,
                                     const uint32_t *key_of, const GpuMatrix *const *targets, size_t n,
                                     const GpuRngSeed *seeds, GpuMatrix *const *outs);
+int gpupoly_trapdoor_preimage_pipelined(const GpuMatrix *stacked, const GpuMatrix *left, const GpuP1CovarianceCache *cache,
+                                        uint32_t base_bits, const GpuMatrix *target, const GpuRngSeed *seeds, GpuMatrix *out);
 int gpupoly_matrix_sample_decomposed_blocks(GpuMatrix *out, int dist_type, const GpuRngSeed *seeds, size_t nblk,
                                             uint32_t base_bits, int small, size_t src_rows, size_t full_ncol,
                                             size_t col_offset);
diff --git a/mxx_amd/_ffi.py b/mxx_amd/_ffi.py
--- a/mxx_amd/_ffi.py
+++ b/mxx_amd/_ffi.py
@@ -160,6 +160,7 @@
     "gpupoly_trapdoor_preimage_many": (C.c_int, [_vp, _vp, _vp, C.c_uint32, C.POINTER(C.c_void_p), _sz, C.POINTER(GpuRngSeed), C.POINTER(C.c_void_p)]),
     "gpupoly_trapdoor_preimage_keyed": (C.c_int, [C.POINTER(C.c_void_p), C.POINTER(C.c_void_p), C.POINTER(C.c_void_p), _sz, C.c_uint32,
                                         C.POINTER(C.c_uint32), C.POINTER(C.c_void_p), _sz, C.POINTER(GpuRngSeed), C.POINTER(C.c_void_p)]),
+    "gpupoly_trapdoor_preimage_pipelined": (C.c_int, [_vp, _vp, _vp, C.c_uint32, _vp, C.POINTER(GpuRngSeed), _vp]),
     "gpupoly_launch_count": (C.c_uint64, []),
     "gpupoly_matrix_scale_round": (C.c_int, [_vp, _vp, C.c_uint64, C.c_int]),
     "gpupoly_matrix_crt_recompose_rounded": (C.c_int, [_vp, C.POINTER(C.c_void_p), C.POINTER(C.c_int), _sz, _sz]),
diff --git a/mxx_amd/csrc/common.h b/mxx_amd/csrc/common.h
--- a/mxx_amd/csrc/common.h
+++ b/mxx_amd/csrc/common.h
@@ -56,6 +56,14 @@
     void load();
 };
 
+struct CtxStream;
+extern thread_local const CtxStream *g_side_window_of;
+extern thread_local hipStream_t g_side_window_stream;
+struct CtxStream {
+    hipStream_t main = nullptr;
+    operator hipStream_t() const { return g_side_window_of == this ? g_side_window_stream : main; }
+};
+
 struct GpuContext {
     EnvSwitches env;
     int device = 0;
@@ -69,7 +77,12 @@
     int word_bytes = 4;
     uint32_t crt_bits = 0;
     std::vector<uint64_t> moduli;
-    hipStream_t stream = nullptr;
+    CtxStream stream;
+    hipStream_t side_stream = nullptr;
+    hipEvent_t pipe_fork = nullptr, pipe_join = nullptr;
+    std::mutex pipe_mutex;
+    std::multimap<size_t, void *> side_free;
+    std::unordered_map<void *, size_t> side_live;
     LimbConst *d_limbs = nullptr;
     LimbConst *d_limbs_r = nullptr;
     void *d_tw_fwd = nullptr;
@@ -315,6 +328,8 @@
                           uint32_t src_cols, uint32_t towers, uint32_t dpt, uint32_t base_bits, size_t k, uint32_t td0 = 0);
 int launch_intt_oop_u32(GpuContext *ctx, uint32_t *out, const uint32_t *in, size_t vectors, uint32_t L);
 int launch_ntt_add_u32(GpuContext *ctx, uint32_t *out, const uint32_t *src, const uint32_t *add, size_t vectors, uint32_t L);
+int launch_ntt_add_window_u32(GpuContext *ctx, uint32_t *out, const uint32_t *src, const uint32_t *add, size_t vectors, uint32_t L,
+                              uint32_t win_cols, uint32_t out_cols);
 int launch_mul_intt_u32(GpuContext *ctx, uint32_t *out, const uint32_t *in, const uint32_t *w, size_t vectors, uint32_t L);
 int launch_matmul(GpuMatrix *out, const GpuMatrix *lhs, const GpuMatrix *rhs);
 int launch_ntt_fwd_pack24_u32(GpuContext *ctx, uint32_t *out, const uint32_t *in, size_t vectors, uint32_t L);
@@ -327,4 +342,14 @@
                       size_t src_col, size_t rows, size_t cols, bool add);
 int sample_p1_keyed_segments(const GpuP1CovarianceCache *cache, const P1KeyEntry *d_keys, const GpuMatrix *tp2,
                              const GpuRngSeed *seeds, const size_t *seg_cols, size_t nseg, GpuMatrix *out);
+int sample_p1_window(const GpuP1CovarianceCache *cache, const GpuMatrix *tp2, GpuRngSeed seed, size_t total_cols, size_t col_start,
+                     GpuMatrix *out);
+int gauss_samp_window(GpuMatrix *src, uint32_t base_bits, double c, GpuRngSeed seed, size_t total_cols, size_t col_start,
+                      GpuMatrix *out);
+struct SideWindow {
+    explicit SideWindow(GpuContext *ctx);
+    ~SideWindow();
+    SideWindow(const SideWindow &) = delete;
+    SideWindow &operator=(const SideWindow &) = delete;
+};
 int launch_scatter_i64(GpuMatrix *out, const int64_t *vals);
diff --git a/mxx_amd/csrc/ntt14.h b/mxx_amd/csrc/ntt14.h
--- a/mxx_amd/csrc/ntt14.h
+++ b/mxx_amd/csrc/ntt14.h
@@ -221,6 +221,19 @@
     fwd_body<W, TIGHT, true, LoadVector<W, true>, true, true>(out + vec * N, LoadVector<W, true>{src + vec * N}, tw_all, lc, limb, add + vec * N);
 }
 
+template <typename W, bool TIGHT = false>
+__global__ void __launch_bounds__(512, 8 / (sizeof(W) / 4))
+    fwd_add_window_kernel(W *__restrict__ out, const W *__restrict__ src, const W *__restrict__ add,
+                          const TwPair<W> *__restrict__ tw_all, const LimbConst *__restrict__ limbs, uint32_t L, uint32_t win_cols,
+                          uint32_t out_cols) {
+    const uint32_t limb = blockIdx.x;
+    const size_t poly = static_cast<size_t>(blockIdx.z) * gridDim.y + blockIdx.y;
+    const size_t row = poly / win_cols, col = poly - row * win_cols;
+    const size_t vec = poly * L + limb, ovec = (row * out_cols + col) * L + limb;
+    const LimbConst lc = limbs[limb];
+    fwd_body<W, TIGHT, true, LoadVector<W, true>, true, true>(out + ovec * N, LoadVector<W, true>{src + vec * N}, tw_all, lc, limb, add + vec * N);
+}
+
 template <typename W, bool REDUCE>
 struct LoadDigit {
     const W *src;
diff --git a/mxx_amd/csrc/ntt_lds_u32.hip b/mxx_amd/csrc/ntt_lds_u32.hip
--- a/mxx_amd/csrc/ntt_lds_u32.hip
+++ b/mxx_amd/csrc/ntt_lds_u32.hip
@@ -91,6 +91,19 @@
     });
 }
 
+int launch_ntt_add_window_u32(GpuContext *ctx, uint32_t *out, const uint32_t *src, const uint32_t *add, size_t vectors, uint32_t L,
+                              uint32_t win_cols, uint32_t out_cols) {
+    dim3 grid;
+    if (win_cols == 0 || !ntt14_grouped(ctx, vectors, L, true, true, grid)) return -1;
+    MXX_TRACE_BYTES(3.0 * vectors * ntt14::N * sizeof(W));
+    return bool_dispatch(!ctx->lazy_ok, [&](auto TIGHT) {
+        MXX_LAUNCH((ntt14::fwd_add_window_kernel<W, TIGHT()>), grid, dim3(ntt14::T), ntt14::lds_bytes(sizeof(W)), ctx->stream, out, src, add,
+                   tw_fwd<W>(ctx), ctx->d_limbs, L, win_cols, out_cols);
+        HIP_TRY(hipGetLastError());
+        return 0;
+    });
+}
+
 int launch_ntt_digits_u32(GpuContext *ctx, uint32_t *out, const uint32_t *coeff, size_t out_vectors, uint32_t L,
                           uint32_t src_cols, uint32_t towers, uint32_t dpt, uint32_t base_bits, size_t k, uint32_t td0) {
     DigitLaunch<W> d{out, coeff, L, src_cols, towers, dpt, base_bits, 0, td0};
diff --git a/mxx_amd/csrc/preimage.hip b/mxx_amd/csrc/preimage.hip
--- a/mxx_amd/csrc/preimage.hip
+++ b/mxx_amd/csrc/preimage.hip
@@ -231,7 +231,7 @@
         lhs_bytes += static_cast<double>(lhs[k]->bytes);
     }
     for (size_t k = runs; k <= kGroupMax; ++k) {
-        keys.col_start[k] = cols;
+        keys.col_start[k] = col_start[runs];
         keys.tile_start[k] = tiles;
     }
     TileGrid g = tile_grid<TR, TC, SV>(ctx, rows, cols, L, rhs->bytes);
@@ -363,6 +363,167 @@
     rc = keyed ? launch_matmul_keyed(ctx, rez.m, keyed->runs.re, keyed->runs.start, keyed->runs.count, z.m) : gpu_matrix_mul(rez.m, call.re, z.m);
     if (rc) return rc;
     return ctx->wide ? launch_scatter<uint64_t>(ctx, scatter, p.m, rez.m, z.m) : launch_scatter<uint32_t>(ctx, scatter, p.m, rez.m, z.m);
+}
+
+
+template <typename W>
+struct WinOperand {
+    const W *p;
+    size_t ld;
+};
+
+template <typename W, int VN, bool SUB_B, int E>
+__global__ void preimage_window_kernel(W *__restrict__ o, size_t o_ld, WinOperand<W> a, WinOperand<W> b, WinOperand<W> e,
+                                       const LimbConst *__restrict__ limbs, size_t rows, size_t wc, uint32_t logN,
+                                       size_t words_per_poly) {
+    typedef typename Words<W, VN>::V V;
+    const size_t entry = static_cast<size_t>(blockIdx.z) * gridDim.y + blockIdx.y;
+    if (entry >= rows * wc) return;
+    const size_t r = entry / wc, c = entry - r * wc;
+    const W *ap = a.p + (r * a.ld + c) * words_per_poly;
+    const W *bp = b.p + (r * b.ld + c) * words_per_poly;
+    const W *ep = E ? e.p + (r * e.ld + c) * words_per_poly : nullptr;
+    W *op = o + (r * o_ld + c) * words_per_poly;
+    for (size_t w0 = (static_cast<size_t>(blockIdx.x) * blockDim.x + threadIdx.x) * VN; w0 < words_per_poly;
+         w0 += static_cast<size_t>(gridDim.x) * blockDim.x * VN) {
+        const W q = static_cast<W>(limbs[w0 >> logN].q);
+        W av[VN], bv[VN], ev[VN], ov[VN];
+        *reinterpret_cast<V *>(av) = *reinterpret_cast<const V *>(ap + w0);
+        *reinterpret_cast<V *>(bv) = *reinterpret_cast<const V *>(bp + w0);
+        if (E) *reinterpret_cast<V *>(ev) = *reinterpret_cast<const V *>(ep + w0);
+#pragma unroll
+        for (int v = 0; v < VN; ++v) {
+            W x = SUB_B ? sub_mod<W>(av[v], bv[v], q) : add_mod<W>(av[v], bv[v], q);
+            if (E == 1) x = add_mod<W>(x, ev[v], q);
+            if (E == 2) x = sub_mod<W>(x, ev[v], q);
+            ov[v] = x;
+        }
+        *reinterpret_cast<V *>(op + w0) = *reinterpret_cast<const V *>(ov);
+    }
+}
+
+template <typename W, bool SUB_B, int E>
+static int launch_window(GpuContext *ctx, W *o, size_t o_ld, WinOperand<W> a, WinOperand<W> b, WinOperand<W> e, size_t rows, size_t wc,
+                         size_t L) {
+    const size_t wpp = L * static_cast<size_t>(ctx->N), entries = rows * wc;
+    const int vn = (static_cast<size_t>(ctx->N) * sizeof(W)) % 16 == 0 ? static_cast<int>(16 / sizeof(W)) : 1;
+    dim3 grid;
+    if (!poly_grid(entries, wpp, vn, grid)) return set_error("gpupoly_trapdoor_preimage_pipelined: matrix too large");
+    MXX_TRACE_BYTES((E ? 4.0 : 3.0) * entries * wpp * sizeof(W));
+    if (vn == 1)
+        MXX_LAUNCH((preimage_window_kernel<W, 1, SUB_B, E>), grid, dim3(256), 0, ctx->stream, o, o_ld, a, b, e, ctx->d_limbs, rows, wc,
+                   ctx->logN, wpp);
+    else
+        MXX_LAUNCH((preimage_window_kernel<W, 16 / sizeof(W), SUB_B, E>), grid, dim3(256), 0, ctx->stream, o, o_ld, a, b, e, ctx->d_limbs,
+                   rows, wc, ctx->logN, wpp);
+    HIP_TRY(hipGetLastError());
+    return 0;
+}
+
+struct PipeCall {
+    GpuContext *ctx;
+    const GpuMatrix *stacked, *left, *target;
+    const GpuP1CovarianceCache *cache;
+    GpuMatrix *out, *rex;
+    GpuMatrix re;
+    uint32_t base_bits;
+    double sigma_large;
+    size_t d, dk, cols;
+    GpuRngSeed seed_p2, seed_p1, seed_z;
+};
+
+struct PipeWindow {
+    size_t c0 = 0, wc = 0;
+    bool side = false;
+    TempMatrix p2, t, tp2c, p1, img, perturbed, z;
+};
+
+constexpr int kPipeStages = 8;
+
+template <typename W>
+static int pipe_stage(const PipeCall &c, PipeWindow &w, int s) {
+    GpuContext *ctx = c.ctx;
+    const int level = c.out->level;
+    const size_t top = 2 * c.d, L = matrix_limbs(c.out), wpp = L * static_cast<size_t>(ctx->N);
+    auto words = [](const GpuMatrix *m) { return static_cast<const W *>(words_ptr(m)); };
+    W *out_words = static_cast<W *>(words_ptr(c.out));
+    int rc = 0;
+    switch (s) {
+    case 0:
+        if ((rc = w.p2.make(ctx, level, c.dk, w.wc))) return rc;
+        return gpu_matrix_sample_distribution_columns(w.p2.m, GPU_MATRIX_DIST_GAUSS, c.sigma_large, c.seed_p2, c.cols, w.c0);
+    case 1: {
+        if ((rc = w.t.make(ctx, level, top + c.d, w.wc)) || (rc = gpu_matrix_mul(w.t.m, c.stacked, w.p2.m))) return rc;
+        if ((rc = w.tp2c.make(ctx, level, top, w.wc))) return rc;
+        MXX_TRACED_COPY("copy (device to device)", ctx->stream, 2.0 * w.tp2c.m->bytes,
+                        HIP_TRY(hipMemcpyAsync(words_ptr(w.tp2c.m), words_ptr(w.t.m), w.tp2c.m->bytes, hipMemcpyDeviceToDevice, ctx->stream)));
+        return gpu_matrix_intt_all(w.tp2c.m);
+    }
+    case 2:
+        if ((rc = w.p1.make(ctx, level, top, w.wc))) return rc;
+        rc = sample_p1_window(c.cache, w.tp2c.m, c.seed_p1, c.cols, w.c0, w.p1.m);
+        w.tp2c.release();
+        return rc;
+    case 3: {
+        if ((rc = w.img.make(ctx, level, c.d, w.wc)) || (rc = gpu_matrix_mul(w.img.m, c.left, w.p1.m))) return rc;
+        if ((rc = w.perturbed.make(ctx, level, c.d, w.wc))) return rc;
+        rc = launch_window<W, true, 2>(ctx, static_cast<W *>(words_ptr(w.perturbed.m)), w.wc, {words(c.target) + w.c0 * wpp, c.cols},
+                                       {words(w.img.m), w.wc}, {words(w.t.m) + top * w.wc * wpp, w.wc}, c.d, w.wc, L);
+        w.img.release();
+        return rc;
+    }
+    case 4:
+        if ((rc = w.z.make(ctx, level, c.dk, w.wc))) return rc;
+        w.z.m->format = GPU_POLY_FORMAT_COEFF;
+        rc = gauss_samp_window(w.perturbed.m, c.base_bits, c.cache->sigma, c.seed_z, c.cols, w.c0, w.z.m);
+        w.perturbed.release();
+        return rc;
+    case 5: {
+        W *dst = out_words + (top * c.cols + w.c0) * wpp;
+        if constexpr (sizeof(W) == 4) {
+            rc = launch_ntt_add_window_u32(ctx, dst, words(w.z.m), words(w.p2.m), c.dk * w.wc * L, static_cast<uint32_t>(L),
+                                           static_cast<uint32_t>(w.wc), static_cast<uint32_t>(c.cols));
+        } else {
+            rc = -1;
+        }
+        if (rc < 0) {
+            if ((rc = launch_ntt(ctx, words_ptr(w.z.m), c.dk * w.wc * L, static_cast<int>(L), false))) return rc;
+            rc = launch_window<W, false, 0>(ctx, dst, c.cols, {words(w.z.m), w.wc}, {words(w.p2.m), w.wc}, {nullptr, 0}, c.dk, w.wc, L);
+        }
+        w.z.release();
+        w.p2.release();
+        return rc;
+    }
+    case 6: {
+        GpuMatrix bottom = row_block(c.out, top, c.dk);
+        bottom.format = GPU_POLY_FORMAT_EVAL;
+        const GpuMatrix *lhs[1] = {&c.re};
+        const uint32_t run[2] = {static_cast<uint32_t>(w.c0), static_cast<uint32_t>(w.c0 + w.wc)};
+        return launch_matmul_keyed(ctx, c.rex, lhs, run, 1, &bottom);
+    }
+    default: {
+        rc = launch_window<W, true, 1>(ctx, out_words + w.c0 * wpp, c.cols, {words(w.p1.m), w.wc}, {words(w.t.m), w.wc},
+                                       {words(c.rex) + w.c0 * wpp, c.cols}, top, w.wc, L);
+        w.p1.release();
+        w.t.release();
+        return rc;
+    }
+    }
+}
+
+static int pipe_windows(const PipeCall &c, PipeWindow (&win)[2]) {
+    for (int s = 0; s < kPipeStages; ++s)
+        for (PipeWindow &w : win) {
+            int rc;
+            if (w.side) {
+                SideWindow scope(c.ctx);
+                rc = c.ctx->wide ? pipe_stage<uint64_t>(c, w, s) : pipe_stage<uint32_t>(c, w, s);
+            } else {
+                rc = c.ctx->wide ? pipe_stage<uint64_t>(c, w, s) : pipe_stage<uint32_t>(c, w, s);
+            }
+            if (rc) return rc;
+        }
+    return 0;
 }
 
 }
@@ -434,6 +595,72 @@
         if (rc) return rc;
     }
     for (size_t j = 0; j < n; ++j) outs[j]->format = GPU_POLY_FORMAT_EVAL;
+    return 0;
+    ABI_GUARD_END
+}
+
+static size_t pipe_split(size_t cols, size_t d) { return cols / d / 2 * d; }
+
+extern "C" int gpupoly_trapdoor_preimage_pipelined(const GpuMatrix *stacked, const GpuMatrix *left, const GpuP1CovarianceCache *cache,
+                                                   uint32_t base_bits, const GpuMatrix *target, const GpuRngSeed *seeds,
+                                                   GpuMatrix *out) {
+    ABI_GUARD_BEGIN
+    auto refuse = [](const std::string &what) { return set_error("gpupoly_trapdoor_preimage_pipelined: " + what); };
+    if (!stacked || !left || !cache || !target || !seeds || !out) return refuse("null argument");
+    GpuContext *ctx = stacked->ctx;
+    const int level = stacked->level;
+    if (left->ctx != ctx || cache->ctx != ctx || target->ctx != ctx || out->ctx != ctx) return refuse("context mismatch");
+    if (left->level != level || cache->level != level || target->level != level || out->level != level) return refuse("level mismatch");
+    if (base_bits == 0 || base_bits >= 63) return refuse("invalid base_bits");
+    const size_t d = target->rows, L = matrix_limbs(stacked), cols = target->cols;
+    const uint32_t dpt = (ctx->crt_bits + base_bits - 1) / base_bits;
+    const size_t top = 2 * d, dk = d * dpt * L;
+    if (d == 0 || stacked->rows != top + d || stacked->cols != dk || left->rows != d || left->cols != top || cache->d != d || cache->m != top)
+        return refuse("shape mismatch: needs [R; E; right] 3d x dk, left d x 2d and a covariance cache of dimension d");
+    if (out->rows != top + dk || out->cols != cols) return refuse("the output must be (2d + dk) x the target's columns");
+    if (stacked->format != GPU_POLY_FORMAT_EVAL || left->format != GPU_POLY_FORMAT_EVAL || target->format != GPU_POLY_FORMAT_EVAL)
+        return refuse("[R; E; right], left and the target must be in EVAL form");
+    if (cols >> 31) return refuse("target too wide");
+    if (words_overlap(out, stacked) || words_overlap(out, left) || words_overlap(out, target)) return refuse("the output aliases an input");
+    if (cols % d || cols < 2 * d) return refuse("unsupported: needs at least two blocks of d columns and no padding column");
+    if ((static_cast<size_t>(ctx->N) >> 1) % SAMPLER_THREADS) return refuse("unsupported: ring dimension not a multiple of 128 (windowed samplers)");
+    if (cache->m > 8) return refuse("unsupported: trapdoor dimension above 4 (no p1 lane kernel)");
+    if (ctx->env.p1_simple) return refuse("unsupported under MXX_HIP_P1=simple (the p1 lane kernel is switched off)");
+    if (dpt > 4) return refuse("unsupported: more than four digits per tower (G-sampler lane kernel)");
+    if (ctx->env.rng_compat) return refuse("unsupported under MXX_HIP_RNG_COMPAT=reference");
+    const double sigma_large = std::sqrt(cache->s * cache->s - cache->sigma * cache->sigma);
+    if (!(sigma_large > 0.0) || !(cache->sigma > 0.0)) return refuse("invalid Gaussian widths in the covariance cache");
+    if (ctx_activate(ctx)) return 1;
+    std::lock_guard<std::mutex> one_call(ctx->pipe_mutex);
+    (void)words_ptr(stacked);
+    (void)words_ptr(left);
+    (void)words_ptr(target);
+    (void)words_ptr(out);
+    TempMatrix rex;
+    int rc = rex.make(ctx, level, top, cols);
+    if (rc) return rc;
+    PipeCall call{ctx, stacked, left, target, cache, out, rex.m, row_block(stacked, 0, top), base_bits, sigma_large, d, dk, cols,
+                  seeds[0], seeds[1], seeds[2]};
+    call.re.format = GPU_POLY_FORMAT_EVAL;
+    PipeWindow win[2];
+    const size_t split = pipe_split(cols, d);
+    win[0].c0 = 0;
+    win[0].wc = split;
+    win[1].c0 = split;
+    win[1].wc = cols - split;
+    win[1].side = true;
+    HIP_TRY(hipEventRecord(ctx->pipe_fork, ctx->stream.main));
+    HIP_TRY(hipStreamWaitEvent(ctx->side_stream, ctx->pipe_fork, 0));
+    rc = pipe_windows(call, win);
+    const hipError_t je = hipEventRecord(ctx->pipe_join, ctx->side_stream);
+    const hipError_t we = je == hipSuccess ? hipStreamWaitEvent(ctx->stream.main, ctx->pipe_join, 0) : je;
+    if (we != hipSuccess) {
+        (void)hipGetLastError();
+        (void)hipStreamSynchronize(ctx->side_stream);
+    }
+    if (rc) return rc;
+    out->format = GPU_POLY_FORMAT_EVAL;
+    ctx->last_kernel = "preimage_pipelined (two column windows on two streams)";
     return 0;
     ABI_GUARD_END
 }
diff --git a/mxx_amd/csrc/rng.h b/mxx_amd/csrc/rng.h
--- a/mxx_amd/csrc/rng.h
+++ b/mxx_amd/csrc/rng.h
@@ -542,6 +542,7 @@
 #define RNG_MAX_SEGMENTS 64
 struct RngSegments {
     uint32_t count;
+    uint32_t win_width, win_off;
     uint32_t start[RNG_MAX_SEGMENTS + 1];
     ChaChaKey key[RNG_MAX_SEGMENTS];
 };
@@ -559,6 +560,12 @@
     }
     return lo;
 }
+__device__ __forceinline__ uint32_t rng_segment_width(const RngSegments &s, uint32_t j) {
+    return s.win_width ? s.win_width : s.start[j + 1] - s.start[j];
+}
+__device__ __forceinline__ uint32_t rng_segment_col(const RngSegments &s, uint32_t j, uint32_t col) {
+    return col - s.start[j] + s.win_off;
+}
 #endif
 
 static inline bool rng_segments_build(RngSegments &out, const GpuRngSeed *seeds, const size_t *seg_cols, size_t nseg,
@@ -566,6 +573,7 @@
     if (nseg == 0 || nseg > RNG_MAX_SEGMENTS || !seeds || !seg_cols) return false;
     size_t at = 0;
     out.count = static_cast<uint32_t>(nseg);
+    out.win_width = out.win_off = 0;
     for (size_t j = 0; j < nseg; ++j) {
         if (seg_cols[j] == 0 || at + seg_cols[j] > 0xffffffffull) return false;
         out.start[j] = static_cast<uint32_t>(at);
@@ -575,6 +583,16 @@
     for (size_t j = nseg; j <= RNG_MAX_SEGMENTS; ++j) out.start[j] = static_cast<uint32_t>(at);
     for (size_t j = nseg; j < RNG_MAX_SEGMENTS; ++j) out.key[j] = ChaChaKey{};
     return at == total_cols;
+}
+
+static inline bool rng_segments_window(RngSegments &out, GpuRngSeed seed, uint64_t domain_tag, size_t win_cols, size_t total_cols,
+                                       size_t col_start) {
+    const size_t one = win_cols;
+    if (win_cols == 0 || total_cols > 0xffffffffull || col_start > total_cols || win_cols > total_cols - col_start) return false;
+    if (!rng_segments_build(out, &seed, &one, 1, domain_tag, win_cols)) return false;
+    out.win_width = static_cast<uint32_t>(total_cols);
+    out.win_off = static_cast<uint32_t>(col_start);
+    return true;
 }
 
 struct RngBlockTable {
diff --git a/mxx_amd/csrc/runtime.hip b/mxx_amd/csrc/runtime.hip
--- a/mxx_amd/csrc/runtime.hip
+++ b/mxx_amd/csrc/runtime.hip
@@ -323,11 +323,52 @@
     }
 }
 
+thread_local const CtxStream *g_side_window_of = nullptr;
+thread_local hipStream_t g_side_window_stream = nullptr;
+
+SideWindow::SideWindow(GpuContext *ctx) {
+    g_side_window_stream = ctx->side_stream;
+    g_side_window_of = &ctx->stream;
+}
+SideWindow::~SideWindow() {
+    g_side_window_of = nullptr;
+    g_side_window_stream = nullptr;
+}
+
+static void side_cache_drop(GpuContext *ctx) {
+    for (auto &kv : ctx->side_free) (void)hipFree(kv.second);
+    ctx->side_free.clear();
+}
+
+static int side_alloc(GpuContext *ctx, size_t want, void **out) {
+    auto it = ctx->side_free.lower_bound(want);
+    if (it != ctx->side_free.end() && it->first <= want + want / 4) {
+        *out = it->second;
+        ctx->side_live[*out] = it->first;
+        ctx->side_free.erase(it);
+        return 0;
+    }
+    hipError_t e = hipMalloc(out, want);
+    if (e != hipSuccess) {
+        (void)hipGetLastError();
+        cache_trim(ctx, 0);
+        side_cache_drop(ctx);
+        e = hipMalloc(out, want);
+    }
+    if (e != hipSuccess) {
+        *out = nullptr;
+        return set_error(e, "hipMalloc");
+    }
+    ctx->side_live[*out] = want;
+    return 0;
+}
+
 int ctx_alloc(GpuContext *ctx, size_t bytes, void **out) {
     *out = nullptr;
     if (bytes == 0) return 0;
     const size_t want = round_block(bytes);
     std::lock_guard<std::mutex> lk(ctx->alloc_mutex);
+    if (g_side_window_of == &ctx->stream) return side_alloc(ctx, want, out);
     auto it = ctx->free_blocks.lower_bound(want);
     if (it != ctx->free_blocks.end() && it->first <= want + want / 4) {
         *out = it->second;
@@ -340,6 +381,7 @@
     if (e != hipSuccess) {
         (void)hipGetLastError();
         cache_trim(ctx, 0);
+        side_cache_drop(ctx);
         e = hipMalloc(out, want);
     }
     if (e != hipSuccess) {
@@ -366,6 +408,13 @@
 void ctx_free(GpuContext *ctx, void *ptr) {
     if (!ptr) return;
     std::lock_guard<std::mutex> lk(ctx->alloc_mutex);
+    auto side = ctx->side_live.find(ptr);
+    if (side != ctx->side_live.end()) {
+        if (ctx->pool_ok) ctx->side_free.emplace(side->second, ptr);
+        else (void)hipFree(ptr);
+        ctx->side_live.erase(side);
+        return;
+    }
     auto it = ctx->live_blocks.find(ptr);
     if (it == ctx->live_blocks.end()) {
         (void)hipFree(ptr);
@@ -464,9 +513,15 @@
         g_contexts.erase(std::remove(g_contexts.begin(), g_contexts.end(), ctx), g_contexts.end());
     }
     (void)hipSetDevice(ctx->device);
-    if (ctx->stream) (void)hipStreamSynchronize(ctx->stream);
+    if (ctx->side_stream) (void)hipStreamSynchronize(ctx->side_stream);
+    if (ctx->stream.main) (void)hipStreamSynchronize(ctx->stream.main);
     for (auto &kv : ctx->free_blocks) (void)hipFree(kv.second);
     for (auto &kv : ctx->live_blocks) (void)hipFree(kv.first);
+    for (auto &kv : ctx->side_free) (void)hipFree(kv.second);
+    for (auto &kv : ctx->side_live) (void)hipFree(kv.first);
+    if (ctx->pipe_fork) (void)hipEventDestroy(ctx->pipe_fork);
+    if (ctx->pipe_join) (void)hipEventDestroy(ctx->pipe_join);
+    if (ctx->side_stream) (void)hipStreamDestroy(ctx->side_stream);
     if (ctx->d_limbs) (void)hipFree(ctx->d_limbs);
     if (ctx->d_limbs_r) (void)hipFree(ctx->d_limbs_r);
     if (ctx->d_twf_fwd) (void)hipFree(ctx->d_twf_fwd);
@@ -486,7 +541,7 @@
     if (ctx->timer_stop) (void)hipEventDestroy(ctx->timer_stop);
     for (hipEvent_t ev : ctx->marks)
         if (ev) (void)hipEventDestroy(ev);
-    if (ctx->stream) (void)hipStreamDestroy(ctx->stream);
+    if (ctx->stream.main) (void)hipStreamDestroy(ctx->stream.main);
     delete ctx;
 }
 
@@ -533,8 +588,18 @@
 
     hipError_t e = hipSetDevice(ctx->device);
     if (e != hipSuccess) { delete ctx; return set_error(e, "hipSetDevice"); }
-    e = hipStreamCreateWithFlags(&ctx->stream, hipStreamNonBlocking);
+    e = hipStreamCreateWithFlags(&ctx->stream.main, hipStreamNonBlocking);
     if (e != hipSuccess) { delete ctx; return set_error(e, "hipStreamCreate"); }
+    e = hipStreamCreateWithFlags(&ctx->side_stream, hipStreamNonBlocking);
+    if (e == hipSuccess) e = hipEventCreateWithFlags(&ctx->pipe_fork, hipEventDisableTiming);
+    if (e == hipSuccess) e = hipEventCreateWithFlags(&ctx->pipe_join, hipEventDisableTiming);
+    if (e != hipSuccess) {
+        if (ctx->pipe_fork) (void)hipEventDestroy(ctx->pipe_fork);
+        if (ctx->side_stream) (void)hipStreamDestroy(ctx->side_stream);
+        (void)hipStreamDestroy(ctx->stream.main);
+        delete ctx;
+        return set_error(e, "hipStreamCreate (side stream)");
+    }
 
     ctx->env.load();
     {
@@ -657,7 +722,7 @@
 
 extern "C" int gpupoly_context_stream(const GpuContext *ctx, void **out_stream) {
     if (!ctx || !out_stream) return set_error("gpupoly_context_stream: null argument");
-    *out_stream = static_cast<void *>(ctx->stream);
+    *out_stream = static_cast<void *>(ctx->stream.main);
     return 0;
 }
 
diff --git a/mxx_amd/csrc/trapdoor.hip b/mxx_amd/csrc/trapdoor.hip
--- a/mxx_amd/csrc/trapdoor.hip
+++ b/mxx_amd/csrc/trapdoor.hip
@@ -186,7 +186,7 @@
         const uint32_t row = p_u / src_cols, col = p_u - row * src_cols;
         const uint32_t j = rng_segment_of(segs, col);
         key = segs.key[j];
-        p = row * (segs.start[j + 1] - segs.start[j]) + (col - segs.start[j]);
+        p = row * rng_segment_width(segs, j) + rng_segment_col(segs, j, col);
     }
     const uint64_t qt = limbs[t].q;
     uint64_t value = static_cast<uint64_t>(src[idx]);
@@ -243,7 +243,7 @@
         const uint32_t row = p_u / src_cols, col = p_u - row * src_cols;
         const uint32_t j = rng_segment_of(segs, col);
         key = segs.key[j];
-        p_u = row * (segs.start[j + 1] - segs.start[j]) + (col - segs.start[j]);
+        p_u = row * rng_segment_width(segs, j) + rng_segment_col(segs, j, col);
     }
 
     ChaChaRng rng;
@@ -555,6 +555,17 @@
     }
 }
 
+int gauss_samp_window(GpuMatrix *src, uint32_t base_bits, double c, GpuRngSeed seed, size_t total_cols, size_t col_start,
+                      GpuMatrix *out) {
+    if (!src || !out) return set_error("invalid gauss_samp_window arguments");
+    if (static_cast<size_t>(src->ctx->N) % SAMPLER_THREADS)
+        return set_error("gauss_samp_window: unsupported: ring too small for a wave per polynomial chunk");
+    RngSegments segs;
+    if (!rng_segments_window(segs, seed, kTagGadget, src->cols, total_cols, col_start))
+        return set_error("gauss_samp_window: the window must be non-empty and lie inside the request");
+    return gauss_samp_impl(src, base_bits, c, GpuRngSeed{}, out, &segs);
+}
+
 struct P1KeyedSegments {
     RngSegments segs;
     const P1KeyEntry *keys;
@@ -692,7 +703,7 @@
         const uint32_t col_u = static_cast<uint32_t>(__builtin_amdgcn_readfirstlane(static_cast<uint32_t>(chunk.base >> logN)));
         const uint32_t j = rng_segment_of(segs, col_u < cols ? col_u : cols - 1);
         key = segs.key[j];
-        seg_col0 = segs.start[j];
+        seg_col0 = segs.start[j] - segs.win_off;
     }
     ChaChaRng rng;
     rng_init_keyed(rng, ring, key, 0, 0, SAMPLER_THREADS);
@@ -1026,6 +1037,19 @@
     }
 }
 
+int sample_p1_window(const GpuP1CovarianceCache *cache, const GpuMatrix *tp2, GpuRngSeed seed, size_t total_cols, size_t col_start,
+                     GpuMatrix *out) {
+    if (!cache || !tp2 || !out) return set_error("invalid sample_p1_window arguments");
+    if (cache->m > 8) return set_error("sample_p1_window: unsupported: trapdoor dimension above 4 (no lane kernel)");
+    if (cache->ctx->env.p1_simple) return set_error("sample_p1_window: unsupported under MXX_HIP_P1=simple (the lane kernel is switched off)");
+    if (static_cast<size_t>(cache->ctx->N) % SAMPLER_THREADS)
+        return set_error("sample_p1_window: unsupported: ring too small for a wave per column chunk");
+    RngSegments segs;
+    if (!rng_segments_window(segs, seed, kTagP1, tp2->cols, total_cols, col_start))
+        return set_error("sample_p1_window: the window must be non-empty and lie inside the request");
+    return sample_p1_impl(cache, tp2, GpuRngSeed{}, out, &segs);
+}
+
 extern "C" int gpu_matrix_sample_p1_full(const GpuMatrix *a_mat, const GpuMatrix *b_mat, const GpuMatrix *d_mat,
                                          const GpuMatrix *tp2, double sigma, double s, double dgg_stddev,
                                          GpuRngSeed seed, GpuMatrix *out) {
diff --git a/mxx_amd/trapdoor.py b/mxx_amd/trapdoor.py
--- a/mxx_amd/trapdoor.py
+++ b/mxx_amd/trapdoor.py
@@ -177,6 +177,24 @@
 def _traffic_bound(params, polys: int) -> bool:
     word = 4 if max(params.moduli()) < (1 << 31) else 8
     return polys * params.crt_depth() * params.ring_dimension() * word >= TRAFFIC_BOUND_BYTES
+
+
+PIPE_MIN_COLS = 8
+
+
+def preimage_pipe_mode() -> str:
+    import os
+
+    v = os.environ.get("MXX_HIP_PREIMAGE_PIPE", "auto")
+    return v if v in ("0", "force") else "auto"
+
+
+def pipe_split(cols: int, d: int) -> int:
+    return cols // d // 2 * d
+
+
+def pipe_key_index(row: int, local_col: int, total_cols: int, col_start: int) -> int:
+    return row * total_cols + col_start + local_col
 
 
 class GpuDCRTPolyTrapdoorSampler:
@@ -240,6 +258,22 @@
         p1 = GpuDCRTPolyMatrix.sample_p1_full_cached(cache, tp2, seeds[1] if seeds is not None else random_gpu_rng_seed())
         return p1, p2, tp2_eval, rp2
 
+    pipelined_calls = 0
+
+    def _pipe_eligible(self, params, td: GpuDCRTTrapdoor, target) -> bool:
+        import os
+
+        mode = preimage_pipe_mode()
+        if mode == "0":
+            return False
+        d, dk, cols = td.r.row_size(), td.r.col_size(), target.col_size()
+        dpt = -(-params.crt_bits() // params.base_bits())
+        if not (params.ring_dimension() % 128 == 0 and d <= 4 and dpt <= 4 and cols % d == 0 and cols >= 2 * d and target.is_ntt
+                and not os.environ.get("MXX_HIP_RNG_COMPAT", "").startswith("r")
+                and not os.environ.get("MXX_HIP_P1", "").startswith("s")):
+            return False
+        return mode == "force" or (cols >= PIPE_MIN_COLS and _traffic_bound(params, dk * cols))
+
     def preimage(self, params, td: GpuDCRTTrapdoor, public_matrix, target, _seeds=None) -> GpuDCRTPolyMatrix:
         d = public_matrix.row_size()
         target_cols = target.col_size()
@@ -250,6 +284,18 @@
         p1_rows, p2_rows = td.re.row_size(), td.re.col_size()
         assert public_matrix.col_size() == p1_rows + p2_rows, "public matrix columns must match perturbation rows"
         left, right, stacked = td.public_matrix_parts(public_matrix)
+        if self._pipe_eligible(params, td, target):
+            from . import _ffi
+
+            seeds = _seeds if _seeds is not None else self._draw_seeds()
+            cache = td.p1_covariance_cache(self.c, s, self.sigma)
+            out = GpuDCRTPolyMatrix(params, p1_rows + p2_rows, target_cols, public_matrix.level, True)
+            st = _ffi.lib().gpupoly_trapdoor_preimage_pipelined(stacked.raw, left.raw, cache.raw, params.base_bits(), target.raw,
+                                                                (_ffi.GpuRngSeed * 3)(*seeds), out.raw)
+            if st != 0:
+                raise _ffi.GpuPolyError(f"gpupoly_trapdoor_preimage_pipelined failed: {_ffi.last_error_string()}")
+            type(self).pipelined_calls += 1
+            return out
         p1, p2, tp2, rp2 = self._sample_pert_parts(params, td, s, self.c, self.sigma, dgg_large_std, target_cols, stacked, _seeds)
         seed_z = _seeds[2] if _seeds is not None else None
         assert (p1.row_size(), p2.row_size()) == (p1_rows, p2_rows)
```

Result: no change. 7.962 million (median of 3 runs) (+0.4%).
